# worm-privacy/proof-of-burn

Hardware: AMD Instinct MI355X
Metric: proof_of_burn witnesses/sec (higher is better)
Workload: dtype u64 bit-sliced lanes + BN254 Fr (8x32-bit Montgomery)

## Files before the change

### proof_of_burn_amd/csrc/circuits.hpp

```cpp
#pragma once
#include <string.h>
#include "gadgets.hpp"
#include "poseidon_consts.h"

#define KECCAKF_ROUND_WIRES 102656u
#define KECCAKF_WIRES (43200u + 24u * KECCAKF_ROUND_WIRES)
#define ABSORB_OWN 5888u
#define ABSORB_WIRES (ABSORB_OWN + 17u * 384u + KECCAKF_WIRES)
#define KR_STORED 76u
#define KR_BITS (KR_STORED * 64u)
#define AB_DIRECT (ABSORB_OWN + 17u * 384u + 43200u)
#define ABSORB_BITS (AB_DIRECT + 24u * KR_BITS)
#define ABSORB_ALIAS (ABSORB_WIRES - ABSORB_BITS)

enum UnitKind : uint32_t {
    U_POB_INPUT = 1, U_POB_RANGE, U_POB_LAYER_ASSERT, U_POB_HDR_ASSERT, U_POB_POSEIDONS, U_BAH_PRE, U_BAH_POST,
    U_KB_HEAD, U_KB_RANGE, U_KB_SELROW, U_KB_POST, U_POB_N2B, U_PC_PRE, U_PC_POST, U_POB_LASTLAYER, U_POB_LASTLAYER_RANGE,
    U_POB_LASTLEN, U_POB_LEAF, U_POB_LAYER_POST, U_SC_M, U_SC_RANGE, U_SC_SUMS, U_POB_LASTLEAF,
    U_RL_A, U_RL_SLROW, U_RL_ACC, U_RL_B, U_POW_PRE, U_POW_POST, U_POB_FINAL, U_ABS_RANGE, U_LD_HEAD, U_LD_SELR, U_LD_TAIL, U_POB_INPUT_FR, U_RL_ACC_B, U_RL_ACC_C,
    U_SP_INPUT, U_SP_HEAD,
    U_SC_MI,
    CK_POS_SEG,
    CK_SR_COLS,
    CK_SL_ROWS,
    CK_N2BE,
    CK_CAT,
    CK_RL_B2, CK_RL_B3,
    U_POS_WIDE,
    U_GM, U_GM_INPUT,
    U_PC_COPY,
    U_LD_COPY,
    U_KIND_COUNT
};
enum : uint32_t { UNIT_GEN = 1, UNIT_CHECK = 2, UNIT_EMIT = 4 };
enum Fam : uint32_t { F_MISC = 0, F_RANGE, F_SELROW, F_LD, F_RL, F_SC, F_POS, F_N2B, F_GM, F_COUNT };
#define FAM_BIT(f) (1u << (f))
#define FAM_LIGHT (FAM_BIT(F_MISC) | FAM_BIT(F_RANGE) | FAM_BIT(F_SELROW) | FAM_BIT(F_LD) | FAM_BIT(F_RL))
#define FAM_HEAVY (FAM_BIT(F_POS) | FAM_BIT(F_N2B))
#define FAM_ALL ((1u << F_COUNT) - 1)
HD constexpr uint32_t fam_of(uint32_t k) {
    return (k == U_KB_RANGE || k == U_ABS_RANGE) ? F_RANGE
         : k == U_KB_SELROW ? F_SELROW
         : (k == U_LD_HEAD || k == U_LD_SELR || k == U_LD_TAIL || k == U_LD_COPY || k == U_POB_LASTLAYER_RANGE || k == U_SC_SUMS) ? F_LD
         : (k == U_RL_A || k == U_RL_SLROW || k == U_RL_ACC_B || k == U_RL_ACC_C || k == U_RL_B || k == CK_SR_COLS || k == CK_SL_ROWS || k == CK_RL_B2 || k == CK_RL_B3 || k == CK_CAT) ? F_RL
         : (k == U_POB_LAYER_POST || k == U_SC_M || k == U_SC_RANGE) ? F_SC
         : (k == U_POB_POSEIDONS || k == U_BAH_PRE || k == U_SP_HEAD || k == CK_POS_SEG || k == U_POS_WIDE) ? F_POS
         : (k == U_GM || k == U_GM_INPUT) ? F_GM
         : (k == U_POB_INPUT_FR || k == U_POB_RANGE || k == U_POB_N2B || k == U_PC_POST || k == U_RL_ACC || k == U_POW_PRE || k == U_SP_INPUT || k == CK_N2BE) ? F_N2B
         : F_MISC;
}
HD constexpr uint32_t gen_fam_of(uint32_t k) { return k == U_PC_PRE ? (uint32_t)F_N2B : fam_of(k); }
HD constexpr bool ride_keeps_evaluation(uint32_t kind) { return fam_of(kind) == F_RL; }
#define UCASE(K) case K: if constexpr ((((MASK) >> (P::is_gen ? gen_fam_of(K) : fam_of(K))) & 1u) && !(P::ride && ride_keeps_evaluation(K)))

struct PobParams { int L, NB, HB, minNib, amountBytes, powZero; Fr maxIntended, maxActual; };
struct SpendParams { int maxAmountBytes; };

#define FP_ISEQ_S (Cur{6, 2, 0, 0, 4})
#define FP_ISEQ_F (Cur{6, 2, 0, 0, 4})
#define FP_N2B8 (Cur{9, 0, 0, 0, 9})
#define FP_ISEQ_D (Cur{6, 0, 0, 0, 6})

struct PobMain {
    FrRef commitment, burnKey, actualBalance, intendedBalance, revealAmount, burnExtraCommitment;
    SmRef numLeafAddressNibbles, layers, layerLens, numLayers, blockHeader, blockHeaderLen, byteSecurityRelax;
    FrRef proofExtraCommitment, remainingCoin, nullifier;
    SmRef addressHashNibbles, blockRoot, stateRoot, nullifierBytes, remainingCoinBytes, revealAmountBytes, burnExtraCommitmentBytes,
        extraCommitmentBytes, lastLayer, lastLayerLen;
    BitRef layerExists, substringCheckers;
    SmRef layerKeccaks, reducedLayerKeccaks;
    BitRef isLeaf, isLastLayerLeaf;
    SmRef leaf, leafLen;
};
struct SpendMain {
    FrRef commitment, burnKey, balance, withdrawnBalance, extraCommitment, coin, remainingCoin;
    SmRef coinBytes, withdrawnBalanceBytes, remainingCoinBytes, extraCommitmentBytes;
};
struct KBRefs {
    SmRef out, in, inLen, numBlocks; BitRef inBitsArray, inBits, inBlocks, outBits, outBytes;
    uint32_t padded_w, pad_o_w, pad_in_w;
    SmRef pad_nb, pad_il, pad_dv, pad_rm; BitRef pad_flt, pad_isEq, pad_isLast;
    Cur c_loop;
    Cur c_div;
    BitRef k_out, k_in; SmRef k_blocks; BitRef k_finalState, f_out, f_in; SmRef f_blocks; BitRef f_s;
    uint32_t abs_w, abs_b;
    BitRef sel_out, sel_arrays; SmRef sel_select; BitRef sel_T;
    Cur c_post;
    SmRef dst; uint32_t has_dst;
    uint32_t mb, index;
};
struct ScRefs {
    BitRef out; uint32_t mi_w; SmRef ml, si; FrRef num; uint32_t M_w; BitRef ex, isl, alw; SmRef sums; BitRef dne;
    Cur c_abs_sub, c_abs_main, c_after_abs, c_loop, c_tail;
    SmRef abs_main_in;
};
struct RlRefs {
    SmRef o, ol, in, inl; FrRef bal; SmRef key, keyLen, acc, accLen, pk, pkLen, val, valLen;
    SmRef t_o, t_ol, t_in, t_il, t_dv, t_rm, t_shf, t_on, t_tmp;
    SmRef s_o, s_in, s_cn; BitRef s_isEq; SmRef s_temp;
    Cur c_sl_iseq, c_mux, c_age, c_acc, c_concat;
};
struct LdRefs {
    BitRef isLeaf; SmRef layer, ll;
    BitRef leafPrefixIsF8; SmRef totalLength; BitRef isConsistentWithLayerLen; SmRef keyPrefix; BitRef keyPrefixIsValid, keyIsMultiByte;
    SmRef keyExtraLen, keyLen, valueWrapperPrefix; BitRef valueWrapperPrefixIsB8; SmRef valueWrapperLen, valuePrefix; BitRef valuePrefixIsF8;
    SmRef valueLen; BitRef isValueWrapperLenConsistent, isKeyValueLenEqualWithLayerLen;
    Cur c_sel[4], c_eq[4], c_mand, c_end;
    SmRef src, len_src; BitRef dst;
};
struct RaRefs {
    SmRef ea_o, ea_ol; FrRef ea_ib; SmRef pn, pnl, br, brl, nbl, sc;
    SmRef ri_o, ri_ol; FrRef ri_i; SmRef by, len, be; BitRef isb, isz; SmRef frb;
    Cur c_cb, c_sl, c_lt, c_concat, c_end;
};
struct SpongeDesc { uint32_t n, stage, src_b, kin_b, fin_b, fs_b, abs_b, kin_w, fin_w, fs_w, abs_w, src_w; };
struct UnitDesc { uint32_t kind, stage; Cur cur; uint32_t a[8]; uint32_t cost, flags; };

#define SC_RANGE_POS 32
#define MAX_KB 72
#define MAX_SC 64
struct CircuitLayout {
    int circuit;
    struct { uint32_t tid, nfr_in, nsm_in, nout; } gm;
    uint32_t decl_order;
    PobParams pob; SpendParams spend;
    PobMain pm; SpendMain sm;
    Fr prefix[3];
    struct { SmRef nibbles; FrRef in; SmRef addressBytes, block, hash; uint32_t kb; } bah;
    struct { FrRef out; SmRef in, flat, block, hash, reduced; uint32_t kb; int N, nb; SmRef fl_o, fl_i, fit_o, fit_i; Cur c_abs; } pc;
    struct { FrRef in; SmRef mzb, keyBytes, raBytes, becBytes, eip, hin, block, keccak; BitRef sbz; uint32_t kb; } pw;
    struct { SmRef out; uint32_t arr_w, sel_w, T_w; Cur c_sel0; } ll;
    RlRefs rl;
    RaRefs ra;
    uint32_t kb_hdr, kb_layer0, nkb, nsc;
    Cur fp_n2be32, fp_n2beN;
    KBRefs kbs[MAX_KB];
    ScRefs scs[MAX_SC];
    LdRefs lds[MAX_SC + 1];
};

HD PosOff pos_off(int t) {
    PosOff k;
    if (t == 3) { k.C = POS_OFF_C_3; k.S = POS_OFF_S_3; k.M = POS_OFF_M_3; k.Pm = POS_OFF_P_3; k.rp = POS_RP_3; }
    else if (t == 4) { k.C = POS_OFF_C_4; k.S = POS_OFF_S_4; k.M = POS_OFF_M_4; k.Pm = POS_OFF_P_4; k.rp = POS_RP_4; }
    else { k.C = POS_OFF_C_5; k.S = POS_OFF_S_5; k.M = POS_OFF_M_5; k.Pm = POS_OFF_P_5; k.rp = POS_RP_5; }
    return k;
}

#define NO_RANK 0xFFFFFFFFu
template <class P> HD BitRef dbits(P& p, uint32_t n) { BitRef r = {p.dvs(n), NO_RANK}; return r; }
template <class P> GD void kb_head(P& p, int mb, S inLen, KBRefs& r) {
    const uint32_t m = 136 * mb;
    r.mb = mb;
    r.out = p.sms(32); r.in = p.sms(m); r.inLen = p.sms(1); r.padded_w = p.dvs(m); r.numBlocks = p.sms(1);
    r.inBitsArray = dbits(p, 8 * m); r.inBits = dbits(p, 8 * m); r.inBlocks = p.bits(8 * m); r.outBits = dbits(p, 256); r.outBytes = dbits(p, 256);
    inLen = p.put(r.inLen, inLen);
    gAssertLessThanS(p, 16, inLen, (S)m);
    r.pad_o_w = p.dvs(m); r.pad_nb = p.sms(1); r.pad_in_w = p.dvs(m); r.pad_il = p.sms(1); r.pad_dv = p.sms(1); r.pad_rm = p.sms(1);
    r.pad_flt = p.bits(m + 1); r.pad_isEq = p.bits(m); r.pad_isLast = p.bits(m);
    inLen = p.put(r.pad_il, inLen);
    S q, rem;
    r.c_div = p.cur;
    gDivide(p, 16, inLen, (S)136, q, rem);
    q = p.put(r.pad_dv, q); p.put(r.pad_rm, rem);
    S nb = p.put(r.pad_nb, q + 1);
    gAssertLessEqThanS(p, 16, nb, (S)mb);
    p.put(r.numBlocks, nb);
    p.put(r.pad_flt, ~(B)0);
    r.c_loop = p.cur;
    p.cur = cur_add(cur_add(cur_add(p.cur, FP_ISEQ_D, 2 * m), FP_N2B8, m), Cur{16u * m, 0, 0, 0, 16u * m}, 1);
}
template <class P> HD void iseq_derived(P& p, Cur c, S a, S b) {
    p.derived(c.w + 1, a); p.derived(c.w + 2, b);
    const S x = (S)((uint32_t)b - (uint32_t)a);
    p.derived(c.w + 4, x); p.derived_inv(c.w + 5, x, true);
}
template <class P> GD void kb_range(P& p, const KBRefs& r, SmRef src, uint32_t lo, uint32_t hi, bool assert_src = false, SmRef also = SmRef{0, 0}) {
    const uint32_t m = 136 * r.mb, cnt = hi - lo, ln = p.lane_id();
    const S inLen = p.get(r.inLen), nb = p.get(r.numBlocks);
    const S last = (S)((uint32_t)nb * 136u - 1u);
    const Cur cE = r.c_loop, cL = cur_add(cE, FP_ISEQ_D, m), cN = cur_add(cL, FP_ISEQ_D, m), cF = cur_add(cN, FP_N2B8, m);
    const uint32_t flat_o_w = cF.w, flat_i_w = cF.w + 8 * m;
    bool fl = P::is_gen ? ((uint32_t)inLen >= lo) : p.bit(p.get(r.pad_flt + lo));
    uint32_t wE = 0, wL = 0, wF = 0, wPE = 0, wPL = 0;
    B wb0 = 0, wb1 = 0;
    S vs[16];
    if constexpr (P::is_count) { for (uint32_t t = 0; t < cnt; t++) p.put(r.in + (lo + t), (S)0); for (int q = 0; q < 16; q++) vs[q] = 0; }
    else {
        SmRef rr[16]; S sv[16];
#pragma unroll
        for (int q = 0; q < 16; q++) rr[q] = r.in + (lo + ((uint32_t)q < cnt ? (uint32_t)q : cnt - 1));
        const SmLoaded<16> h = sm_load(p, rr);
#pragma unroll
        for (int q = 0; q < 16; q++) sv[q] = p.get(src + (lo + ((uint32_t)q < cnt ? (uint32_t)q : cnt - 1)));
        sm_commit(p, rr, h, sv);
#pragma unroll
        for (int q = 0; q < 16; q++) vs[q] = P::is_check ? h.s[q] : sv[q];
        if (assert_src) {
#pragma unroll
            for (int q = 0; q < 16; q++) p.require_lane((uint32_t)sv[q] < 256u, FAILCODE(T_NUM2BITS, 38));
        }
        if (also.w) {
            SmRef ar[16];
#pragma unroll
            for (int q = 0; q < 16; q++) ar[q] = also + (lo + ((uint32_t)q < cnt ? (uint32_t)q : cnt - 1));
            const SmLoaded<16> ha = sm_load(p, ar);
            sm_commit(p, ar, ha, sv);
        }
    }
#pragma unroll
    for (uint32_t t = 0; t < 16; t++) if (t < cnt) {
        const uint32_t i = lo + t;
        const Cur ce = cur_add(cE, FP_ISEQ_D, i), cl = cur_add(cL, FP_ISEQ_D, i);
        const S v = vs[t];
        iseq_derived(p, ce, (S)i, inLen); iseq_derived(p, cl, (S)i, last);
        const bool e = (uint32_t)inLen == i, l = (uint32_t)last == i;
        fl = fl && !e;
        const S pv = (fl ? v : 0) + (S)e + (l ? 0x80 : 0);
        p.derived(r.pad_in_w + i, v); p.derived(r.pad_o_w + i, pv); p.derived(r.padded_w + i, pv); p.derived(cN.w + 9 * i + 8, pv);
        p.require_lane((uint32_t)pv < 256u, FAILCODE(T_NUM2BITS, 38));
        wE |= (uint32_t)e << t; wL |= (uint32_t)l << t; wF |= (uint32_t)fl << t;
        wPE |= (e ? 3u : 0u) << (2 * t); wPL |= (l ? 3u : 0u) << (2 * t);
        if (t < 8) wb0 |= (B)((uint32_t)pv & 0xffu) << (8 * t); else wb1 |= (B)((uint32_t)pv & 0xffu) << (8 * (t - 8));
    }
    const B runE = p.xpose64(wE, 0, cnt), runL = p.xpose64(wL, 0, cnt), runF = p.xpose64(wF, 0, cnt);
    const B runPairE = p.xpose64(wPE, 0, 2 * cnt), runPairL = p.xpose64(wPL, 0, 2 * cnt);
    const B bits0 = p.xpose(wb0, 64), bits1 = cnt > 8 ? p.xpose(wb1, 64) : 0;
    p.run_put(cnt, r.pad_isEq.w + lo + ln, r.pad_isEq.i + lo + ln, runE);
    p.run_put(cnt, r.pad_flt.w + lo + 1 + ln, r.pad_flt.i + lo + 1 + ln, runF);
    p.run_put(cnt, r.pad_isLast.w + lo + ln, r.pad_isLast.i + lo + ln, runL);
    {
        const uint32_t i = lo + (ln >> 1), wh = ln & 1;
        p.run_derived(2 * cnt, cE.w + 6 * i + 3 * wh, runPairE);
        p.run_derived(2 * cnt, cL.w + 6 * i + 3 * wh, runPairL);
        if constexpr (P::is_emit) { if (ln < 2 * cnt) { p.site_c(cE.w + 6 * i + 3 * wh, r.pad_isEq.w + i); p.site_c(cL.w + 6 * i + 3 * wh, r.pad_isLast.w + i); } }
    }
    for (uint32_t h2 = 0; h2 < 2 && 8 * h2 < cnt; h2++) {
        const uint32_t n = (cnt - 8 * h2 < 8 ? cnt - 8 * h2 : 8) * 8;
        const B x = h2 ? bits1 : bits0;
        const uint32_t j = 8 * (lo + 8 * h2) + ln, i = lo + 8 * h2 + (ln >> 3);
        p.run_put(n, r.inBlocks.w + j, r.inBlocks.i + j, x);
        p.run_derived(n, cN.w + 9 * i + (ln & 7), x);
        p.run_derived(n, r.inBitsArray.w + j, x);
        p.run_derived(n, flat_i_w + j, x);
        p.run_derived(n, flat_o_w + j, x);
        p.run_derived(n, r.inBits.w + j, x);
    }
}
template <class P> GD void kb_declare_keccak(P& p, KBRefs& r) {
    const uint32_t n = r.mb;
    r.k_out = dbits(p, 256); r.k_in = p.bits(n * 1088); r.k_blocks = p.sms(1); r.k_finalState = dbits(p, 1600);
    r.f_out = dbits(p, 1600); r.f_in = p.bits(n * 1088); r.f_blocks = p.sms(1); r.f_s = p.bits((n + 1) * 1600);
    r.abs_w = p.cur.w; r.abs_b = p.cur.b;
    p.skip_alias(n * ABSORB_WIRES, n * ABSORB_BITS);
    r.sel_out = dbits(p, 1600); r.sel_arrays = dbits(p, (n + 1) * 1600); r.sel_select = p.sms(1); r.sel_T = dbits(p, 1600 * (n + 1));
}
template <class P, int N1> GD void kb_selrow_n(P& p, const KBRefs& r, uint32_t row, uint32_t j0, uint32_t j1) {
    const uint32_t n1 = N1 ? (uint32_t)N1 : r.mb + 1, n = j1 - j0, ln = p.lane_id();
    const uint32_t fw = 9 * n1 + 3, fb = 1, fq = 9 * n1 + 2;
    const Cur c0 = p.cur;
    const uint32_t idx = row * 64 + j0 + ln;
    const S blocks = p.get(r.numBlocks);
    p.require(p.ballot((uint32_t)blocks < n1), FAILCODE(T_SELECTOR, 43));
    const uint32_t bw = c0.w + ln * fw, bb = c0.b + ln * fb;
    B acc = 0;
    p.run_derived(n, bw + 2 * n1 + 2, 0);
#pragma unroll
    for (uint32_t k = 0; k < n1; k++) {
        const B v = p.run_get(n, r.f_s.i + k * 1600 + idx);
        const B e = p.ballot((uint32_t)blocks == k);
        acc |= e & v;
        if constexpr (P::is_emit) {
            p.run_derived(n, r.sel_arrays.w + k * 1600 + idx, v);
            p.run_derived(n, r.sel_T.w + idx * n1 + k, v);
            p.run_derived(n, bw + 1 + k, v);
            p.run_derived(n, bw + n1 + 2 + k, e);
            p.run_derived(n, bw + 2 * n1 + 3 + k, acc);
            const uint32_t cw = bw + 3 * n1 + 3 + 6 * k;
            p.run_derived(n, cw, e);
            p.run_derived(n, cw + 3, e);
        }
    }
    p.run_put(n, bw, bb, acc);
    p.run_derived(n, r.sel_out.w + idx, acc);
    p.run_derived(n, r.f_out.w + idx, acc);
    p.run_derived(n, r.k_finalState.w + idx, acc);
    if (row < 4) {
        const uint32_t pw = r.c_post.w;
        p.run_derived(n, r.k_out.w + idx, acc);
        p.run_derived(n, r.outBits.w + idx, acc);
        p.run_derived(n, pw + 256 + idx, acc);
        p.run_derived(n, pw + idx, acc);
        p.run_derived(n, r.outBytes.w + idx, acc);
        p.run_derived(n, pw + 512 + 9 * (idx >> 3) + 1 + (idx & 7), acc);
        for (uint32_t jj = 0; jj < n; jj += 8) {
            S by = 0;
#pragma unroll
            for (uint32_t b = 0; b < 8; b++) by |= (S)p.bit(p.run_bcast(acc, jj + b)) << b;
            const uint32_t i = (row * 64 + j0 + jj) >> 3;
            const SmRef b2n_o = {pw + 512 + 9 * i, r.c_post.s + i};
            const S o = p.put(r.out + i, p.put(b2n_o, by));
            if (r.has_dst) p.put(r.dst + i, o);
        }
    }
    derived_rows_same(p, c0.w + n1 + 1, fw, n, blocks);
    for (uint32_t k = 0; k < n1; k++) {
        const uint32_t cw = c0.w + 3 * n1 + 3 + 6 * k;
        const S x = (S)(k - (uint32_t)blocks);
        derived_rows_same(p, cw + 1, fw, n, blocks);
        derived_rows_same(p, cw + 2, fw, n, (S)k);
        derived_rows_same(p, cw + 4, fw, n, x);
        derived_rows_same(p, cw + 5, fw, n, x, true);
    }
    p.cur = cur_add(c0, Cur{fw, fb, 0, 0, fq}, n);
}
template <class P> GD void kb_selrow(P& p, const KBRefs& r, uint32_t row, uint32_t j0, uint32_t j1) { kb_selrow_n<P, 0>(p, r, row, j0, j1); }
template <class P> GD void kb_post(P& p, const KBRefs& r) {
    S nb = p.get(r.numBlocks);
    p.put(r.k_blocks, nb); p.put(r.f_blocks, nb); p.put(r.sel_select, nb);
    p.cur = cur_add(r.c_post, Cur{512 + 32 * 9, 0, 32, 0, 512 + 32 * 8}, 1);
}

#include "gadget_mains.hpp"

template <class P> GD void rl_b_prefixes(P& p, const RlRefs& R, const PobParams& prm, S kl, S& pl, S& vl) {
    const int ab = 32, bb = prm.amountBytes, maxAcc = 4 + bb + 66, maxKey = 1 + ab;
    const S al = p.get(R.accLen);
    p.put(R.val, 0xb8); p.put(R.val + 1, al);
    copy_n(p, R.val + 2, R.acc, maxAcc);
    vl = p.put(R.valLen, 2 + al);
    p.put(R.pk, 0xf8); p.put(R.pk + 1, (kl + 1) + vl); p.put(R.pk + 2, 0x80 + kl);
    copy_n(p, R.pk + 3, R.key, maxKey);
    pl = p.put(R.pkLen, 3 + kl);
}
template <class P, class MR> GD void rl_b_concat(P& p, const RlRefs& R, const MR& M, const PobParams& prm, S pl, S vl) {
    const int ab = 32, bb = prm.amountBytes, maxAcc = 4 + bb + 66, maxVal = 2 + maxAcc, maxKey = 1 + ab, maxPK = 2 + 1 + maxKey, maxOut = maxPK + maxVal;
    p.cur = R.c_concat;
    S cl;
    SmRef c;
    if constexpr (P::is_check) c = gConcatHead(p, maxPK, maxVal, R.pk, pl, R.val, vl, cl);
    else c = gConcat(p, maxPK, maxVal, R.pk, pl, R.val, vl, cl, true);
    { copy_n(p, R.o, c, (int)(maxOut)); copy_n(p, M.leaf, c, (int)(maxOut)); }
    p.put(M.leafLen, p.put(R.ol, cl));
}

template <class P> GD void L_pc_declare(P& p, CircuitLayout& L, int N) {
    const Cur c_abs = p.cur;
    for (int j = 0; j < N; j++) { p.dvs(32); p.cur = cur_add(p.cur, FP_ABITS8, 32); }
    const SmRef fl_o = p.sms(32 * N), fl_i = p.sms(32 * N);
    const SmRef fit_o = p.sms(136 * L.pc.nb), fit_i = p.sms(32 * N);
    if (P::is_count) { L.pc.c_abs = c_abs; L.pc.fl_o = fl_o; L.pc.fl_i = fl_i; L.pc.fit_o = fit_o; L.pc.fit_i = fit_i; }
}

HD bool unit_is_heavy(uint32_t k) { return fam_of(k) >= F_SC; }
HD bool unit_gen_is_heavy(uint32_t k) { return gen_fam_of(k) >= F_SC; }

template <class P, uint32_t MASK> GD void unit_run(P& p, const UnitDesc& d, CircuitLayout& L);
#ifdef __HIPCC__
template <uint32_t MASK, bool FAULT> GD void unit_run_ride(GenPT<true, FAULT>& p, const UnitDesc& d, CircuitLayout& L) {
    if constexpr ((MASK >> F_RL) & 1u) { if (ride_keeps_evaluation(d.kind)) { GenPT<false> q = plain_of(p); unit_run<GenPT<false>, FAM_BIT(F_RL)>(q, d, L); p.status = q.status; return; } }
    unit_run<GenPT<true, FAULT>, MASK>(p, d, L);
}
#endif
template <class P, uint32_t MASK> GD void unit_run(P& p, const UnitDesc& d, CircuitLayout& L) {

    const PobMain& M = L.pm;
    const PobParams& prm = L.pob;
    const int LB = 136 * prm.NB, HBy = 136 * prm.HB;
    (void)M; (void)LB; (void)HBy;
    p.cur = d.cur;
    switch (d.kind) {
    UCASE(U_GM) { gm_run(p, d, L); } break;
    UCASE(U_GM_INPUT) { gm_input(p, d); } break;
    UCASE(U_POB_INPUT) {
        for (uint32_t k = d.a[0]; k < d.a[1]; k++) { SmRef r = {M.numLeafAddressNibbles.w + k, M.numLeafAddressNibbles.i + k}; p.put(r, p.input_sm(k)); }
    } break;
    UCASE(U_POB_LAYER_ASSERT) {
        gAssertLessThanS(p, 16, p.get(M.layerLens + d.a[0]), (S)(LB * 8));
    } break;
    UCASE(U_POB_HDR_ASSERT) {
        gAssertLessThanS(p, 16, p.get(M.blockHeaderLen), (S)(HBy * 8));
        for (int i = 0; i < 32; i++) p.put(M.stateRoot + i, p.get(M.blockHeader + 91 + i));
    } break;
    UCASE(U_ABS_RANGE) {
        SmRef src = {d.a[2], d.a[3]};
        abs_range(p, d.cur, d.a[0], src, d.a[4], d.a[5]);
    } break;
    UCASE(U_BAH_POST) {
        SmRef nb = gBytes2Nibbles(p, 32, L.bah.hash);
        { copy_n(p, L.bah.nibbles, nb, (int)(64)); copy_n(p, M.addressHashNibbles, nb, (int)(64)); }
    } break;
    UCASE(U_KB_HEAD) {
        SmRef len = {d.a[1], d.a[2]};
        KBRefs r = L.kbs[d.a[0]];
        const S inLen = (P::is_gen && d.a[3]) ? p.input_sm(d.a[3] - 1) : p.get(len);
        kb_head(p, r.mb, inLen, r);
        if (P::is_count) L.kbs[d.a[0]] = r;
    } break;
    UCASE(U_KB_RANGE) {
        SmRef src = {d.a[1], d.a[2]};
        kb_range(p, L.kbs[d.a[0]], src, d.a[3], d.a[4], d.a[5] != 0, SmRef{d.a[6], d.a[7]});
    } break;
    UCASE(U_KB_SELROW) { kb_selrow(p, L.kbs[d.a[0]], d.a[1], d.a[2], d.a[3]); } break;
    UCASE(U_KB_POST) { kb_post(p, L.kbs[d.a[0]]); } break;
    UCASE(U_PC_PRE) {
        const int N = L.pc.N;
        L_pc_declare(p, L, N);
        KBRefs r = L.kbs[L.pc.kb];
        kb_head(p, L.pc.nb, (S)(32 * N), r);
        if (P::is_count) L.kbs[L.pc.kb] = r;
    } break;
    UCASE(U_PC_COPY) {
        const uint32_t N = (uint32_t)L.pc.N, j = d.a[0], nblk = 136u * (uint32_t)L.pc.nb;
        if (j < N) {
            SmRef src;
            if (L.circuit == 2) src = L.pc.in + 32 * j;
            else if (L.circuit == 0) src = j == 0 ? M.blockRoot : j == 1 ? M.nullifierBytes : j == 2 ? M.remainingCoinBytes : j == 3 ? M.revealAmountBytes : j == 4 ? M.burnExtraCommitmentBytes : M.extraCommitmentBytes;
            else src = j == 0 ? L.sm.coinBytes : j == 1 ? L.sm.withdrawnBalanceBytes : j == 2 ? L.sm.remainingCoinBytes : L.sm.extraCommitmentBytes;
            auto dst_of = [&](uint32_t a) -> SmRef {
                const SmRef b = a == 0 ? L.pc.in : a == 1 ? L.pc.fl_i : a == 2 ? L.pc.fl_o : a == 3 ? L.pc.flat : a == 4 ? L.pc.fit_i : a == 5 ? L.pc.fit_o : L.pc.block;
                return b + 32 * j;
            };
// ... 448 lines not shown
        }
        if (lo == 0) p.derived_fr(sc.M_w, fr_zero());
        for (uint32_t k = lo; k < hi; k++) {
            Fr b1 = {{(uint32_t)p.get(src + k), 0, 0, 0, 0, 0, 0, 0}};
            acc = fr_add(fr_mul(b1, p.k256r(k)), acc);
            p.derived_fr(sc.M_w + k + 1, acc);
            p.site_m(sc.M_w + k + 1, sc.mi_w + k, k);
        }
    } break;
    UCASE(U_SC_RANGE) {
        const ScRefs& sc = L.scs[d.a[0]];
        const uint32_t lo = d.a[1], hi = d.a[2], sl = 31;
        const S mainLen = p.get(sc.ml);
        const F subNum = p.get(sc.num);
        const Fr subC = fr_from_mont(subNum);
        const SmRef src = M.layers + ((d.a[0] - 1) * LB);
        const uint32_t lastIdx = (uint32_t)(mainLen - (S)sl + 1);
        const uint32_t ln = p.lane_id(), cnt = hi - lo;
        bool allowed = P::is_gen ? (lastIdx >= lo) : p.bit(p.get(sc.alw + lo));
        uint32_t wIsl = 0, wAlw = 0, wEx = 0;
        B wC0 = 0, wC1 = 0;
        F ddL = fr_zero();
        Fr win = sc_window(p, src, lo, sl);
        for (uint32_t t = 0; t < cnt; t++) {
            const uint32_t i = lo + t;
            const S nxt = i + sl < (uint32_t)LB ? p.get(src + (i + sl)) : 0;
            const bool e = fr_eq(win, subC), last = i == lastIdx;
            allowed = allowed && !last;
            wIsl |= (uint32_t)last << t; wAlw |= (uint32_t)allowed << t; wEx |= (uint32_t)e << t;
            const B four = (B)((last ? 3u : 0u) | (e ? 12u : 0u)) << (4 * (t & 15));
            if (t < 16) wC0 |= four; else wC1 |= four;
            if constexpr (P::is_emit) {
                const Cur c = cur_add(cur_add(sc.c_loop, FP_ISEQ_S, i), FP_ISEQ_F, i);
                iseq_derived(p, c, (S)i, (S)lastIdx);
                const F t1 = fr_mul(subNum, p.k256(i)), t2 = fr_mul(fr_to_mont(win), p.k256(i)), dd = fr_sub(t2, t1);
                p.derived_fr(c.w + 7, t1); p.derived_fr(c.w + 8, t2); p.derived_fr(c.w + 10, dd);
                const F ds = p.bcast_sel(dd);
                if (ln == t) ddL = ds;
            }
            sc_window_step(win, sl, (uint32_t)nxt);
        }
        if constexpr (P::is_emit) {
            const F inv = fr_is_zero(ddL) ? fr_zero() : fr_inv(ddL);
            if (ln < cnt) p.w32(cur_add(cur_add(sc.c_loop, FP_ISEQ_S, lo + ln), FP_ISEQ_F, lo + ln).w + 11, fr_from_mont(inv), (fr_is_zero(ddL) ? 3 : 2) | 4);
        }
        const B runIsl = p.xpose64(wIsl, 0, cnt), runAlw = p.xpose64(wAlw, 0, cnt), runEx = p.xpose64(wEx, 0, cnt);
        const B runC0 = p.xpose(wC0, 64), runC1 = cnt > 16 ? p.xpose(wC1, 64) : 0;
        p.run_put(cnt, sc.isl.w + lo + ln, sc.isl.i + lo + ln, runIsl);
        p.run_put(cnt, sc.alw.w + lo + 1 + ln, sc.alw.i + lo + 1 + ln, runAlw);
        p.run_put(cnt, sc.ex.w + lo + ln, sc.ex.i + lo + ln, runEx);
        for (uint32_t h2 = 0; h2 < 2 && 16 * h2 < cnt; h2++) {
            const uint32_t n = (cnt - 16 * h2 < 16 ? cnt - 16 * h2 : 16) * 4, i = lo + 16 * h2 + (ln >> 2), wh = ln & 3;
            p.run_put(n, sc.c_loop.w + 12 * i + 3 * wh, sc.c_loop.b + 4 * i + wh, h2 ? runC1 : runC0);
        }
    } break;
    UCASE(CK_POS_SEG) {
        if constexpr (!(P::is_check || P::is_count)) { (void)d; }
        else if (d.a[0] == 3) gPoseidonSegStored<P, 3>(p, pos_off(3), d.cur, d.a[1]);
        else if (d.a[0] == 4) gPoseidonSegStored<P, 4>(p, pos_off(4), d.cur, d.a[1]);
        else gPoseidonSegStored<P, 5>(p, pos_off(5), d.cur, d.a[1]);
    } break;
    UCASE(CK_SL_ROWS) {
        if constexpr (P::is_check || P::is_count) gShiftLeftRows(p, (int)d.a[0], d.cur, Cur{d.a[3], d.a[4], d.a[5], d.cur.f, d.cur.q}, d.a[1], d.a[2]);
    } break;
    UCASE(CK_N2BE) {
        if constexpr (P::is_check || P::is_count || P::is_gen) {
            const FrRef src = P::is_gen ? FrRef{d.a[6], d.a[7]} : FrRef{d.a[1], d.a[2]}; const SmRef also = {d.a[3], d.a[4]};
            gNum2BigEndianBytesFv(p, (int)d.a[0], p.get(src), also, d.a[5] != 0);
        }
    } break;
    default: break;
    }
}
template <class P> GD void unit_run_all(P& p, const UnitDesc& d, CircuitLayout& L) { unit_run<P, FAM_ALL>(p, d, L); }

#include <stdlib.h>
#include <algorithm>
#include <stdexcept>
#include <string>
#include <vector>
struct Plan {
    CircuitLayout L;
    std::vector<UnitDesc> units;
    std::vector<SpongeDesc> sponges;
    Cur total;
    uint32_t nfr_in, nsm_in, max_stage;
    enum { TRACK_STRIDE = 32, MAX_TRACKS = 7 };
    uint32_t ntracks, track_fork[MAX_TRACKS], track_join[MAX_TRACKS];
    uint32_t wide_tracks = 0;
    CountP p;

    static bool same(Cur a, Cur b) { return a.w == b.w && a.b == b.b && a.s == b.s && a.f == b.f && a.q == b.q; }
    void expect_cursor(const char* what, Cur got, Cur want) {
        if (!same(got, want)) throw std::runtime_error(std::string("layout planner: split units disagree with the monolithic template: ") + what);
    }
    void record(uint32_t kind, uint32_t stage, Cur cur, uint32_t a0 = 0, uint32_t a1 = 0, uint32_t a2 = 0, uint32_t a3 = 0, uint32_t a4 = 0, uint32_t a5 = 0, uint32_t a6 = 0, uint32_t a7 = 0) {
        UnitDesc d; d.kind = kind; d.stage = stage; d.cur = cur; d.cost = 0; d.a[0] = a0; d.a[1] = a1; d.a[2] = a2; d.a[3] = a3; d.a[4] = a4; d.a[5] = a5; d.a[6] = a6; d.a[7] = a7;
        d.flags = (kind == CK_POS_SEG || kind == CK_SR_COLS || kind == CK_SL_ROWS || kind == CK_RL_B2 || kind == CK_RL_B3 || kind == CK_CAT) ? UNIT_CHECK
                : kind == CK_N2BE ? (UNIT_GEN | UNIT_CHECK)
                : kind == U_POS_WIDE ? UNIT_GEN
                : kind == U_SC_M ? UNIT_EMIT
                : kind == U_POB_POSEIDONS ? (UNIT_CHECK | UNIT_EMIT)
                : kind == U_GM_INPUT ? (UNIT_GEN | UNIT_CHECK)
                : kind == U_POB_INPUT ? UNIT_EMIT
                : (UNIT_GEN | UNIT_CHECK | UNIT_EMIT);
        units.push_back(d);
        if (stage > max_stage) max_stage = stage;
    }
    void unit(uint32_t kind, uint32_t stage, uint32_t a0 = 0, uint32_t a1 = 0, uint32_t a2 = 0, uint32_t a3 = 0, uint32_t a4 = 0) {
        record(kind, stage, p.cur, a0, a1, a2, a3, a4);
        const UnitDesc d = units.back();
        p.nnotes = 0;
        unit_run_all(p, d, L);
        take_notes(p, stage);
    }
    void take_notes(CountP& q, uint32_t stage) {
        if (q.notes_overflow) throw std::runtime_error("layout planner: a composite unit has more split sub-blocks than PLAN_MAX_NOTES");
        for (uint32_t k = 0; k < q.nnotes; k++) {
            const PlanNote& nt = q.notes[k];
            if (nt.what == NOTE_POSEIDON) {
                const uint32_t ns = pos_nseg(pos_off((int)nt.n).rp);
                for (uint32_t seg = 1; seg < ns; seg++) record(CK_POS_SEG, stage, nt.cur, nt.n, seg);
                if (stage % TRACK_STRIDE == 0) throw std::runtime_error("layout planner: a Poseidon composite needs a stage before it");
                record(U_POS_WIDE, stage - 1, nt.cur, nt.n, nt.a[0], nt.a[1], nt.a[2], nt.a[3], nt.a[4], nt.a[5]);
            } else if (nt.what == NOTE_N2BE) record(CK_N2BE, stage, nt.cur, nt.n, nt.a[0], nt.a[1], nt.a[2], nt.a[3], nt.a[4], nt.a[5], nt.a[6]);
            else if (nt.what == NOTE_SHIFTLEFT) { for (uint32_t i = 0; i < nt.n; i += 2) record(CK_SL_ROWS, stage, nt.cur, nt.n, i, std::min(i + 2, nt.n), nt.a[0], nt.a[1], nt.a[2]); }
        }
        q.nnotes = 0;
    }
    void record_composite(uint32_t kind, uint32_t stage, Cur cur) {
        record(kind, stage, cur);
        const UnitDesc d = units.back();
        CountP q; q.nnotes = 0;
        unit_run_all(q, d, L);
        take_notes(q, stage);
    }
    void cat_units(uint32_t stage, Cur c0, int La, int Lb) {
        Cur cc[3]; concat_cursors(p, c0, La, Lb, cc);
        for (uint32_t part = 0; part < 4; part++) record(CK_CAT, stage, cc[part < 3 ? part : 2], part, (uint32_t)La, (uint32_t)Lb, c0.w, c0.s);
    }
    void abs_units(uint32_t stage, uint32_t N, SmRef src, uint32_t chunk = 32, bool emit_only = false) {
        CountP chk; chk.cur = p.cur; gAssertByteString(chk, (int)N, src);
        const uint32_t own_w = p.dvs(N);
        const Cur c0 = p.cur;
        for (uint32_t lo = 0; lo < N; lo += chunk) { record(U_ABS_RANGE, stage, c0, own_w, 0, src.w, src.i, lo, std::min(lo + chunk, N)); if (emit_only) units.back().flags = UNIT_EMIT; }
        p.cur = cur_add(c0, FP_ABITS8, N);
        expect_cursor("AssertByteString", p.cur, chk.cur);
    }
    void keccak_tail(uint32_t kb, uint32_t range_stage, SmRef dst, bool has_dst) {
        KBRefs& r = L.kbs[kb];
        r.index = kb;
        kb_declare_keccak(p, r);
        SpongeDesc s; s.n = r.mb; s.stage = range_stage + 1; s.src_b = r.inBlocks.i; s.src_w = r.inBlocks.w;
        s.kin_b = r.k_in.i; s.kin_w = r.k_in.w; s.fin_b = r.f_in.i; s.fin_w = r.f_in.w; s.fs_b = r.f_s.i; s.fs_w = r.f_s.w; s.abs_b = r.abs_b; s.abs_w = r.abs_w;
        sponges.push_back(s);
        r.dst = dst; r.has_dst = has_dst ? 1 : 0;
        {
            CountP q; q.cur = p.cur; r.c_post = Cur{0, 0, 0, 0}; r.has_dst = 0; kb_selrow(q, r, 24, 0, 1);
            const Cur fp1 = {q.cur.w - p.cur.w, q.cur.b - p.cur.b, q.cur.s - p.cur.s, 0, q.cur.q - p.cur.q};
            r.c_post = cur_add(p.cur, fp1, 1600); r.has_dst = has_dst ? 1 : 0;
        }
        const uint32_t split = r.mb >= 8 ? 4 : r.mb >= 3 ? 2 : 1;
        for (uint32_t row = 0; row < 25; row++) {
            const Cur c0 = p.cur;
            CountP q; q.cur = c0; kb_selrow(q, r, row, 0, 64);
            const Cur fp = {(q.cur.w - c0.w) / 64, (q.cur.b - c0.b) / 64, (q.cur.s - c0.s) / 64, 0, (q.cur.q - c0.q) / 64};
            for (uint32_t k = 0; k < split; k++) record(U_KB_SELROW, range_stage + 2, cur_add(c0, fp, k * (64 / split)), kb, row, k * (64 / split), (k + 1) * (64 / split));
            p.cur = q.cur;
        }
        if (!same(p.cur, r.c_post)) throw std::runtime_error("layout planner: selector footprint");
        unit(U_KB_POST, range_stage + 2, kb);
        if (range_stage + 1 > max_stage) max_stage = range_stage + 1;
    }
    void keccak_bytes(uint32_t kb, int mb, uint32_t stage, SmRef src, SmRef len, SmRef dst, uint32_t len_input = 0, bool has_dst = true, bool assert_src = false, SmRef also = SmRef{0, 0}) {
        L.kbs[kb].mb = mb;
        const Cur start = p.cur;
        unit(U_KB_HEAD, stage, kb, len.w, len.i, len_input);
        const uint32_t m = 136 * mb;
        for (uint32_t lo = 0; lo < m; lo += 16) record(U_KB_RANGE, stage + 1, start, kb, src.w, src.i, lo, std::min(lo + 16, m), assert_src ? 1u : 0u, also.w, also.i);
        keccak_tail(kb, stage + 1, dst, has_dst);
    }
    void kb_ranges(uint32_t kb, uint32_t stage, SmRef src) {
        const uint32_t m = 136 * L.kbs[kb].mb;
        for (uint32_t lo = 0; lo < m; lo += 16) record(U_KB_RANGE, stage, p.cur, kb, src.w, src.i, lo, std::min(lo + 16, m));
    }
    void leaf_detector(uint32_t inst, uint32_t stage, SmRef src, SmRef len, BitRef dst, bool copy_units = true) {
        const uint32_t N = 136 * L.pob.NB;
        CountP chk; chk.cur = p.cur; gLeafDetector(chk, (int)N, src, 0);
        L.lds[inst].src = src; L.lds[inst].len_src = len; L.lds[inst].dst = dst;
        unit(U_LD_HEAD, stage, inst);
        expect_cursor("LeafDetector", p.cur, chk.cur);
        if (copy_units) for (uint32_t lo = 0; lo < N; lo += 32) record(U_LD_COPY, stage, p.cur, inst, lo, std::min(lo + 32, N));
        for (uint32_t k = 0; k < 4; k++) for (uint32_t lo = 0; lo < N; lo += 34) record(U_LD_SELR, stage + 1, p.cur, inst, k, lo, std::min(lo + 34, N));
        record(U_LD_TAIL, stage + 2, p.cur, inst);
    }
    void burn_address_hash(uint32_t pre_stage) {
        L.bah.nibbles = p.sms(64); L.bah.in = p.frs(3); L.bah.addressBytes = p.sms(20); L.bah.block = p.sms(136); L.bah.hash = p.sms(32);
        L.bah.kb = L.nkb++;
        if (L.circuit == 2) { L.pm.burnKey = L.bah.in; L.pm.revealAmount = L.bah.in + 1; L.pm.burnExtraCommitment = L.bah.in + 2; L.pm.addressHashNibbles = L.bah.nibbles; }
        unit(U_BAH_PRE, pre_stage);
        kb_ranges(L.bah.kb, pre_stage + 1, L.bah.block);
        keccak_tail(L.bah.kb, pre_stage + 1, L.bah.hash, true);
        unit(U_BAH_POST, pre_stage + 4);
    }
    void proof_of_work_checker(uint32_t pre_stage) {
        L.pw.in = p.frs(3); L.pw.mzb = p.sms(1); L.pw.keyBytes = p.sms(32); L.pw.raBytes = p.sms(32); L.pw.becBytes = p.sms(32); L.pw.eip = p.sms(8);
        L.pw.hin = p.sms(104); L.pw.block = p.sms(136); L.pw.keccak = p.sms(32); L.pw.sbz = p.bits(32);
        L.pw.kb = L.nkb++;
        if (L.circuit == 2) { L.pm.burnKey = L.pw.in; L.pm.revealAmount = L.pw.in + 1; L.pm.burnExtraCommitment = L.pw.in + 2; L.pm.byteSecurityRelax = L.pw.mzb; }
        unit(U_POW_PRE, pre_stage);
        kb_ranges(L.pw.kb, pre_stage + 1, L.pw.block);
        keccak_tail(L.pw.kb, pre_stage + 1, L.pw.keccak, true);
        unit(U_POW_POST, pre_stage + 4);
    }
    void public_commitment(int N, uint32_t pre_stage) {
        L.pc.N = N; L.pc.nb = N * 32 / 136 + ((N * 32) % 136 != 0);
        L.pc.out = p.frs(1); L.pc.in = p.sms(32 * N); L.pc.flat = p.sms(32 * N); L.pc.block = p.sms(136 * L.pc.nb); L.pc.hash = p.sms(32); L.pc.reduced = p.sms(31);
        L.pc.kb = L.nkb++; L.kbs[L.pc.kb].mb = L.pc.nb;
        {
            CountP chk; chk.cur = p.cur; chk.decl_order = p.decl_order;
            for (int j = 0; j < N; j++) gAssertByteString(chk, 32, L.pc.in + 32 * j);
            gFlattenS(chk, 32 * N, L.pc.in); gFitS(chk, 32 * N, 136 * L.pc.nb, L.pc.flat);
            unit(U_PC_PRE, pre_stage);
            for (int j = 0; j <= N; j++) record(U_PC_COPY, pre_stage, p.cur, (uint32_t)j);
            KBRefs r2 = L.kbs[L.pc.kb]; kb_head(chk, L.pc.nb, (S)(32 * N), r2);
            expect_cursor("PublicCommitment", p.cur, chk.cur);
        }
        kb_ranges(L.pc.kb, pre_stage + 1, L.pc.block);
        keccak_tail(L.pc.kb, pre_stage + 1, L.pc.hash, true);
        unit(U_PC_POST, pre_stage + 4);
    }

    void estimate_costs() {
        for (UnitDesc& d : units) {
            if (d.kind == U_POS_WIDE) { d.cost = 8 * pos_wires((int)d.a[0], pos_off((int)d.a[0]).rp); continue; }
            CountP q; const UnitDesc dd = d; unit_run_all(q, dd, L); d.cost = q.nput * (unit_is_heavy(d.kind) ? 4 : 1);
        }
    }
    void plan_pob(const PobParams& prm) {
        memset(&L, 0, sizeof L);
        L.circuit = 0; L.pob = prm; L.nkb = 0; max_stage = 0; L.decl_order = p.decl_order;
        L.fp_n2be32 = n2be_footprint(32); L.fp_n2beN = n2be_footprint(prm.amountBytes);
        const uint32_t TB = TRACK_STRIDE, TR = 2 * TRACK_STRIDE, TC = 3 * TRACK_STRIDE, TN = 4 * TRACK_STRIDE;
        ntracks = 6; track_fork[1] = 0; track_join[1] = 5; track_fork[2] = TB + 6; track_join[2] = 10; track_fork[3] = 0; track_join[3] = TR + 2;
        track_fork[4] = TB + 1; track_join[4] = 4;
        const uint32_t TP = 5 * TRACK_STRIDE;
        track_fork[5] = 0; track_join[5] = 5; wide_tracks = 1u << 5;
        const uint32_t TQ = 6 * TRACK_STRIDE;
        ntracks = 7; track_fork[6] = 4; track_join[6] = 10;
        PobMain& M = L.pm;
        const int Ln = prm.L, LB = 136 * prm.NB, HBy = 136 * prm.HB;
        p.cur = Cur{1, 0, 0, 0};
        M.commitment = p.frs(1);
        M.burnKey = p.frs(1); M.actualBalance = p.frs(1); M.intendedBalance = p.frs(1); M.revealAmount = p.frs(1); M.burnExtraCommitment = p.frs(1);
        M.numLeafAddressNibbles = p.sms(1); M.layers = p.sms(Ln * LB); M.layerLens = p.sms(Ln); M.numLayers = p.sms(1);
        M.blockHeader = p.sms(HBy); M.blockHeaderLen = p.sms(1); M.byteSecurityRelax = p.sms(1); M.proofExtraCommitment = p.frs(1);
        M.remainingCoin = p.frs(1); M.nullifier = p.frs(1); M.addressHashNibbles = p.sms(64); M.blockRoot = p.sms(32); M.stateRoot = p.sms(32);
        M.nullifierBytes = p.sms(32); M.remainingCoinBytes = p.sms(32); M.revealAmountBytes = p.sms(32); M.burnExtraCommitmentBytes = p.sms(32);
        M.extraCommitmentBytes = p.sms(32); M.lastLayer = p.sms(LB); M.lastLayerLen = p.sms(1); M.layerExists = p.bits(Ln);
        M.substringCheckers = p.bits(Ln - 1); M.layerKeccaks = p.sms(32 * Ln); M.reducedLayerKeccaks = p.sms(31 * Ln); M.isLeaf = p.bits(Ln);
        M.isLastLayerLeaf = p.bits(1); M.leaf = p.sms(139); M.leafLen = p.sms(1);
        nfr_in = 6; nsm_in = 1 + Ln * LB + Ln + 1 + HBy + 2;

        unit(U_POB_INPUT_FR, 0);
        for (uint32_t k = 0; k < nsm_in; k += 256) unit(U_POB_INPUT, 0, k, std::min(k + 256, nsm_in));
        for (int k = 0; k < 5; k++) unit(U_POB_RANGE, TB + 1, k);
        for (int i = 0; i < Ln; i++) { unit(U_POB_LAYER_ASSERT, TP + 1, i); abs_units(TP + 1, LB, M.layers + i * LB, 32, true); }
        unit(U_POB_HDR_ASSERT, TP + 1); abs_units(TP + 1, HBy, M.blockHeader, 32, true);
        unit(U_POB_POSEIDONS, TB + 2, 0);
        unit(U_POB_POSEIDONS, TB + 2, 1);
        burn_address_hash(TB + 2);
        L.kb_hdr = L.nkb++;
        keccak_bytes(L.kb_hdr, prm.HB, 0, M.blockHeader, M.blockHeaderLen, M.blockRoot, 0, true, true);
        for (int j = 0; j < 5; j++) unit(U_POB_N2B, TN + 1, j);
        public_commitment(6, TQ + 1);
        {
            CountP chk; chk.cur = p.cur; gSelectorArray1D(chk, Ln, LB, M.layers, 0);
            L.ll.out = p.sms(LB); L.ll.arr_w = p.dvs(Ln * LB); L.ll.sel_w = p.dvs(1); L.ll.T_w = p.dvs(LB * Ln);
            unit(U_POB_LASTLAYER, TP + 1);
            L.ll.c_sel0 = p.cur;
            const Cur fp = sel_fp((uint32_t)Ln);
            for (uint32_t j = 0; j < (uint32_t)LB; j += 4) record(U_POB_LASTLAYER_RANGE, TP + 1, p.cur, j, std::min<uint32_t>(j + 4, LB));
            p.cur = cur_add(p.cur, fp, LB);
            expect_cursor("SelectorArray1D", p.cur, chk.cur);
        }
        unit(U_POB_LASTLEN, TP + 1);
        L.kb_layer0 = L.nkb; L.nkb += Ln;
        L.nsc = Ln;
        for (int i = 0; i < Ln; i++) {
            leaf_detector(i, TP + 1, M.layers + i * LB, M.layerLens + i, M.isLeaf + i, false);
            keccak_bytes(L.kb_layer0 + i, prm.NB, 0, M.layers + i * LB, M.layerLens + i, M.layerKeccaks + 32 * i, 0, true, true, L.lds[i].layer);
            const Cur start = p.cur;
            unit(U_POB_LAYER_POST, 5, i);
            if (i > 0) {
                const ScRefs sc = L.scs[i];
                CountP chk; chk.cur = start; { gFitS(chk, 32, 31, M.layerKeccaks); gSubstringCheck(chk, LB, 31, M.layers, 0, M.reducedLayerKeccaks); }
                expect_cursor("SubstringCheck", p.cur, chk.cur);
                const SmRef src = M.layers + (i - 1) * LB;
                for (uint32_t lo = 0; lo < (uint32_t)LB; lo += 32) {
                    record(U_ABS_RANGE, TP + 1, sc.c_abs_main, sc.abs_main_in.w, sc.abs_main_in.i, src.w, src.i, lo, std::min<uint32_t>(lo + 32, LB));
                    units.back().flags = UNIT_EMIT;
                }
                for (uint32_t lo = 0; lo < (uint32_t)LB; lo += 32) record(U_SC_M, TP + 1, start, i, lo, std::min<uint32_t>(lo + 32, LB));
                const uint32_t kk = LB - 31 + 1;
                record(U_SC_MI, TP + 1, start, i);
                for (uint32_t lo = 0; lo < kk; lo += SC_RANGE_POS) record(U_SC_RANGE, 6, sc.c_loop, i, lo, std::min<uint32_t>(lo + SC_RANGE_POS, kk));
                const uint32_t sums_step = 64;
// ... 129 lines not shown
```

### proof_of_burn_amd/csrc/k_keccak.hip

```cpp
#include <stdlib.h>
#define POB_KECCAK_TU
#include "keccak_kernels.hpp"
void launch_k_chain(const KArgs& K, bool check, uint32_t nsponges, uint32_t ngroups, hipStream_t st) {
    if (check) hipLaunchKernelGGL(k_chain_check, dim3(nsponges, ngroups), dim3(64), 0, st, K);
    else hipLaunchKernelGGL(k_chain, dim3(nsponges, ngroups), dim3(64), 0, st, K);
}
int pob_kchk_rounds() { return POB_KCHK_ROUNDS; }
void launch_k_rounds(const KArgs& K, bool check, uint32_t nperms, uint32_t ngroups, hipStream_t st) {
    if (check) hipLaunchKernelGGL((k_rounds_check<true, POB_KCHK_ROUNDS, 4, 12>), dim3(nperms * (24 / POB_KCHK_ROUNDS), ngroups), dim3(64), 0, st, K);
    else hipLaunchKernelGGL(k_rounds_gen<POB_KGEN_ROUNDS>, dim3(nperms * (24 / POB_KGEN_ROUNDS), ngroups), dim3(64), 0, st, K);
}
#ifndef POB_KGC_ROUNDS
#define POB_KGC_ROUNDS 8
#endif
#ifndef POB_KGC_WAVES
#define POB_KGC_WAVES 4
#endif
#ifndef POB_KGC_DP
#define POB_KGC_DP 4
#endif
#ifndef POB_KGC_NTM
#define POB_KGC_NTM false
#endif
int pob_kgc_rounds() { return POB_KGC_ROUNDS; }
void launch_k_rounds_gc(const KArgs& K, uint32_t nperms, uint32_t ngroups, bool fault, hipStream_t st) {
    if (fault) hipLaunchKernelGGL((k_rounds_gc<POB_KGC_ROUNDS, POB_KGC_DP, POB_KGC_WAVES, true, POB_KGC_NTM>), dim3(nperms * (24 / POB_KGC_ROUNDS), ngroups), dim3(64), 0, st, K);
    else hipLaunchKernelGGL((k_rounds_gc<POB_KGC_ROUNDS, POB_KGC_DP, POB_KGC_WAVES, false, POB_KGC_NTM>), dim3(nperms * (24 / POB_KGC_ROUNDS), ngroups), dim3(64), 0, st, K);
}
void launch_k_emit_bits(const u64* G, uint8_t* out, uint32_t wire_base, uint32_t bit_base, uint32_t count, uint32_t sel, hipStream_t st) {
    uint32_t blocks = (count + 255) / 256; if (blocks > 8192) blocks = 8192;
    hipLaunchKernelGGL(k_emit_bits, dim3(blocks), dim3(256), 0, st, G, out, wire_base, bit_base, count, sel);
}
void launch_k_emit_bits_red(const u64* G, uint8_t* out, uint32_t wire0, uint32_t bit_base, uint32_t count, uint32_t sel, const unsigned long long* rbits, const uint32_t* rpre,
                            uint32_t k0, uint32_t kn, hipStream_t st) {
    uint32_t blocks = (count + 255) / 256; if (blocks > 16384) blocks = 16384;
    hipLaunchKernelGGL(k_emit_bits_red, dim3(blocks), dim3(256), 0, st, G, out, wire0, bit_base, count, sel, rbits, rpre, k0, kn);
}
void launch_k_emit_absorb(const u64* G, uint8_t* out, uint32_t ab, uint32_t o0, uint32_t count, uint32_t sel, const uint16_t* tab, hipStream_t st) {
    uint32_t blocks = (count + 255) / 256; if (blocks > 8192) blocks = 8192;
    hipLaunchKernelGGL(k_emit_absorb, dim3(blocks), dim3(256), 0, st, G, out, ab, o0, count, sel, tab);
}
void launch_k_emit_absorb_red(const u64* G, uint8_t* out, uint32_t wire0, uint32_t ab, uint32_t o0, uint32_t count, uint32_t sel, const uint16_t* tab, const unsigned long long* rbits,
                              const uint32_t* rpre, uint32_t k0, uint32_t kn, hipStream_t st) {
    uint32_t blocks = (count + 255) / 256; if (blocks > 16384) blocks = 16384;
    hipLaunchKernelGGL(k_emit_absorb_red, dim3(blocks), dim3(256), 0, st, G, out, wire0, ab, o0, count, sel, tab, rbits, rpre, k0, kn);
}
bool keccak_alias_table_host(uint16_t* tab) { return keccak_round_alias_table(tab); }
```

### proof_of_burn_amd/csrc/keccak_kernels.hpp

```cpp
#pragma once
#include <hip/hip_runtime.h>
#include <stdint.h>
#include "kernels_common.hpp"
#ifdef POB_HOSTSIM
#define POB_WAVES_PER_SIMD(n)
#else
#define POB_WAVES_PER_SIMD(n) __attribute__((amdgpu_waves_per_eu(n, n)))
#endif

static __device__ __constant__ u64 KECCAK_RC_DEV[24] = {
    0x0000000000000001ULL, 0x0000000000008082ULL, 0x800000000000808AULL, 0x8000000080008000ULL, 0x000000000000808BULL,
    0x0000000080000001ULL, 0x8000000080008081ULL, 0x8000000000008009ULL, 0x000000000000008AULL, 0x0000000000000088ULL,
    0x0000000080008009ULL, 0x000000008000000AULL, 0x000000008000808BULL, 0x800000000000008BULL, 0x8000000000008089ULL,
    0x8000000000008003ULL, 0x8000000000008002ULL, 0x8000000000000080ULL, 0x000000000000800AULL, 0x800000008000000AULL,
    0x8000000080008081ULL, 0x8000000000008080ULL, 0x0000000080000001ULL, 0x8000000080008008ULL};

__host__ __device__ constexpr int krot_(int i) {
    constexpr int t[25] = {1, 10, 7, 11, 17, 18, 3, 5, 16, 8, 21, 24, 4, 15, 23, 19, 13, 12, 2, 20, 14, 22, 9, 6, 1};
    return t[i];
}
#define KROT(i) krot_(i)

enum : uint32_t { KS_IN = 0, KS_ST = 25, KS_OUT = 101, KS_ZERO = 126, KS_RC = 127 };
#define KSL_X5(x, k) (4u * (x) + (k))
// ... 107 lines not shown
    void arr(uint32_t off, const V& v) { for (uint32_t k = 0; k < 64; k++) set(off + k, v.e[k]); }
    void gate(uint32_t off, const V& o, const V& a, const V& b) { for (uint32_t k = 0; k < 64; k++) { set(off + 3 * k, o.e[k]); set(off + 3 * k + 1, a.e[k]); set(off + 3 * k + 2, b.e[k]); } }
    void out(int, const V&) {}
    void set(uint32_t w, uint16_t e) { if (w >= KECCAKF_ROUND_WIRES || tab[w] != 0xFFFFu) ok = false; else tab[w] = e; }
};

template <class IO> HD void garr(IO& io, uint32_t off, const typename IO::V& o, const typename IO::V& a, const typename IO::V& b) {
    io.arr(off, o); io.arr(off + 64, a); io.arr(off + 128, b); io.gate(off + 192, o, a, b);
}

template <class W> __device__ __forceinline__ void round_native(W* a, int r, uint32_t lane) {
    W c[5], d[5], b[25];
#pragma unroll
    for (int x = 0; x < 5; x++) c[x] = a[x] ^ a[x + 5] ^ a[x + 10] ^ a[x + 15] ^ a[x + 20];
#pragma unroll
    for (int x = 0; x < 5; x++) d[x] = c[(x + 4) % 5] ^ lane_rotl(c[(x + 1) % 5], 1, lane);
#pragma unroll
    for (int i = 0; i < 25; i++) a[i] ^= d[i % 5];
    b[0] = a[0];
#pragma unroll
    for (int i = 0; i < 24; i++) b[KROT(i + 1)] = lane_rotl(a[KROT(i)], ((i + 1) * (i + 2) / 2) % 64, lane);
#pragma unroll
    for (int i = 0; i < 25; i++) { const int y = i / 5 * 5; a[i] = b[i] ^ (~b[y + (i + 1) % 5] & b[y + (i + 2) % 5]); }
    a[0] ^= ((KECCAK_RC_DEV[r] >> lane) & 1) ? ~(W)0 : (W)0;
}

template <class IO> HD void round_walk(IO& io, int r) {
    typedef typename IO::V V;
    V in[25], th[25], rp[25], ch[25], out[25];
#pragma unroll
    for (int i = 0; i < 25; i++) in[i] = io.in(i);
#pragma unroll
    for (int i = 0; i < 25; i++) io.arr(1600 + 64 * i, in[i]);
    {
        const uint32_t T = 8000;
        V C[5], Dv[5];
#pragma unroll
        for (int i = 0; i < 25; i++) io.arr(T + 1600 + 64 * i, in[i]);
#pragma unroll
        for (int x = 0; x < 5; x++) {
            const uint32_t X = T + 3840 + 2112 * x;
            const V a = in[x], b = in[5 + x], c = in[10 + x], d = in[15 + x], e = in[20 + x];
            const V ab = io.gx(KSL_X5(x, 0), a, b), abc = io.gx(KSL_X5(x, 1), ab, c), abcd = io.gx(KSL_X5(x, 2), abc, d), o = io.gx(KSL_X5(x, 3), abcd, e);
            io.arr(X, o); io.arr(X + 64, a); io.arr(X + 128, b); io.arr(X + 192, c); io.arr(X + 256, d); io.arr(X + 320, e);
            io.arr(X + 384, ab); io.arr(X + 448, abc); io.arr(X + 512, abcd);
            garr(io, X + 576, ab, a, b); garr(io, X + 960, abc, ab, c); garr(io, X + 1344, abcd, abc, d); garr(io, X + 1728, o, abcd, e);
            C[x] = o; io.arr(T + 3200 + 64 * x, o);
        }
#pragma unroll
        for (int x = 0; x < 5; x++) {
            const uint32_t Dd = T + 14400 + 1408 * x;
            const V a = C[(x + 1) % 5], b = C[(x + 4) % 5];
            const V rot = io.rotl(a, 1);
            const V aux0 = io.keep_ge(rot, 1), aux1 = io.keep_lt(rot, 1), aux2 = io.or_disjoint(aux0, aux1, rot);
            const V o = io.gx(KSL_D(x), b, aux2);
            io.arr(Dd, o); io.arr(Dd + 64, a); io.arr(Dd + 128, b); io.arr(Dd + 192, aux0); io.arr(Dd + 256, aux1); io.arr(Dd + 320, aux2);
            io.arr(Dd + 384, aux0); io.arr(Dd + 448, a);
            io.arr(Dd + 512, aux1); io.arr(Dd + 576, a);
            garr(io, Dd + 640, aux2, aux0, aux1); garr(io, Dd + 1024, o, b, aux2);
            Dv[x] = o; io.arr(T + 3520 + 64 * x, o);
        }
#pragma unroll
        for (int i = 0; i < 5; i++) {
#pragma unroll
            for (int j = 0; j < 5; j++) {
                const int idx = i + 5 * j;
                const V o = io.gx(KSL_TH(idx), in[idx], Dv[i]);
                garr(io, T + 21440 + 384 * (i * 5 + j), o, in[idx], Dv[i]);
                th[idx] = o; io.arr(T + 64 * idx, o);
            }
        }
    }
#pragma unroll
    for (int i = 0; i < 25; i++) io.arr(3200 + 64 * i, th[i]);
    {
        const uint32_t Rb = 39040;
#pragma unroll
        for (int i = 0; i < 25; i++) io.arr(Rb + 1600 + 64 * i, th[i]);
        rp[0] = th[0]; io.arr(Rb, th[0]);
#pragma unroll
        for (int i = 0; i < 24; i++) {
            const uint32_t S_ = Rb + 3200 + 896 * i;
            const int shl = ((i + 1) * (i + 2) / 2) % 64;
            const V a = th[KROT(i)];
            const V rot = io.rotl(a, shl);
            const V aux0 = io.keep_lt(rot, shl);
            const V aux1 = io.keep_ge(rot, shl);
            const V o = io.or_disjoint(aux0, aux1, rot);
            io.arr(S_, o); io.arr(S_ + 64, a); io.arr(S_ + 128, aux0); io.arr(S_ + 192, aux1);
            io.arr(S_ + 256, aux0); io.arr(S_ + 320, a);
            io.arr(S_ + 384, aux1); io.arr(S_ + 448, a);
            garr(io, S_ + 512, o, aux0, aux1);
            rp[KROT(i + 1)] = o; io.arr(Rb + 64 * KROT(i + 1), o);
        }
    }
#pragma unroll
    for (int i = 0; i < 25; i++) io.arr(4800 + 64 * i, rp[i]);
    {
        const uint32_t Cb = 63744;
#pragma unroll
        for (int i = 0; i < 25; i++) io.arr(Cb + 1600 + 64 * i, rp[i]);
#pragma unroll
        for (int i = 0; i < 25; i++) {
            const uint32_t C_ = Cb + 3200 + 1280 * i;
            const int y = i / 5 * 5;
            const V a = rp[i], b = rp[y + (i + 1) % 5], c = rp[y + (i + 2) % 5];
            const V bx = io.not_(b), bc = io.ga(KSL_AND(i), bx, c);
            const V o = i == 0 ? io.gx(KSL_CHI0, a, bc) : io.gxo(i, a, bc);
            io.arr(C_, o); io.arr(C_ + 64, a); io.arr(C_ + 128, b); io.arr(C_ + 192, c); io.arr(C_ + 256, bx); io.arr(C_ + 320, bc);
            io.arr(C_ + 384, bx); io.arr(C_ + 448, b);
            garr(io, C_ + 512, bc, bx, c); garr(io, C_ + 896, o, a, bc);
            ch[i] = o; io.arr(Cb + 64 * i, o);
        }
    }
#pragma unroll
    for (int i = 0; i < 25; i++) io.arr(6400 + 64 * i, ch[i]);
    {
        const uint32_t Ib = 98944;
        const V rc = io.rc(r);
#pragma unroll
        for (int i = 0; i < 25; i++) io.arr(Ib + 1600 + 64 * i, ch[i]);
        io.arr(Ib + 3200, rc); io.arr(Ib + 3264, rc);
        const V o = io.gxo(0, ch[0], rc);
        garr(io, Ib + 3328, o, ch[0], rc);
        out[0] = o;
#pragma unroll
        for (int i = 1; i < 25; i++) out[i] = ch[i];
#pragma unroll
        for (int i = 0; i < 25; i++) io.arr(Ib + 64 * i, out[i]);
    }
#pragma unroll
    for (int i = 0; i < 25; i++) { io.arr(64 * i, out[i]); io.out(i, out[i]); }
}
static inline bool keccak_round_alias_table(uint16_t* tab) {
    for (uint32_t i = 0; i < KECCAKF_ROUND_WIRES; i++) tab[i] = 0xFFFFu;
    SymIO io; io.tab = tab; io.ok = true;
    round_walk(io, 0);
    for (uint32_t i = 0; i < KECCAKF_ROUND_WIRES; i++) if (tab[i] == 0xFFFFu) io.ok = false;
    return io.ok;
}

#define KF_MID 3200u
#define KF_ROUNDS 43200u
#define AB_KECCAKF (ABSORB_OWN + 17u * 384u)


__device__ __forceinline__ void chain_body(const KArgs A, uint32_t bx, uint32_t by) {
    const uint32_t lane = threadIdx.x & 63u;
    const SpongeDesc sp = A.sponges[A.first + bx];
    u64* G = A.bits + (uint64_t)by * A.group_stride;
    u64 st[25];
#pragma unroll
    for (int i = 0; i < 25; i++) st[i] = 0;
    auto put = [&](uint32_t idx, u64 v) { G[idx + lane] = v; };
    for (uint32_t b = 0; b < sp.n; b++) {
        const uint32_t Ab = sp.abs_b + b * ABSORB_BITS;
        u64 blk[17], aux[25];
#pragma unroll
        for (int i = 0; i < 17; i++) blk[i] = G[sp.src_b + b * 1088 + 64 * i + lane];
#pragma unroll
        for (int i = 0; i < 25; i++) { put(sp.fs_b + b * 1600 + 64 * i, st[i]); put(Ab + 1600 + 64 * i, st[i]); }
#pragma unroll
        for (int i = 0; i < 17; i++) {
            put(sp.kin_b + b * 1088 + 64 * i, blk[i]); put(sp.fin_b + b * 1088 + 64 * i, blk[i]); put(Ab + 3200 + 64 * i, blk[i]);
            const u64 o = st[i] ^ blk[i];
            const uint32_t X = Ab + ABSORB_OWN + 384 * i;
            put(X, o); put(X + 64, st[i]); put(X + 128, blk[i]);
            { u64* q = G + X + 192 + 3 * lane; q[0] = o; q[1] = st[i]; q[2] = blk[i]; }
            aux[i] = o;
        }
#pragma unroll
        for (int i = 17; i < 25; i++) aux[i] = st[i];
        const uint32_t Kf = Ab + AB_KECCAKF;
#pragma unroll
        for (int i = 0; i < 25; i++) { put(Ab + 4288 + 64 * i, aux[i]); put(Kf + 1600 + 64 * i, aux[i]); put(Kf + KF_MID + 64 * i, aux[i]); st[i] = aux[i]; }
        for (int r = 0; r < 24; r++) {
            round_native(st, r, lane);
#pragma unroll
            for (int i = 0; i < 25; i++) put(Kf + KF_MID + 1600 * (r + 1) + 64 * i, st[i]);
        }
#pragma unroll
        for (int i = 0; i < 25; i++) { put(Kf + 64 * i, st[i]); put(Ab + 64 * i, st[i]); }
    }
#pragma unroll
    for (int i = 0; i < 25; i++) put(sp.fs_b + sp.n * 1600 + 64 * i, st[i]);
}
#ifdef POB_KECCAK_TU
__global__ void __launch_bounds__(64, 3) k_chain(KArgs A) { chain_body(A, blockIdx.x, blockIdx.y); }
#endif

__device__ __forceinline__ void chain_check_body(const KArgs A, uint32_t bx, uint32_t by) {
    const uint32_t lane = threadIdx.x;
    const uint32_t pi = A.first + bx;
    const SpongeDesc sp = A.sponges[A.perm_sponge[pi]];
    const uint32_t b = A.perm_block[pi];
    const u64* G = A.bits + (uint64_t)by * A.group_stride;
    const uint32_t Ab = sp.abs_b + b * ABSORB_BITS, Kf = Ab + AB_KECCAKF;
    u64 bad = 0;
#pragma unroll 1
    for (int i = 0; i < 25; i++) {
        const u64 st = G[sp.fs_b + b * 1600 + 64 * i + lane];
        if (b == 0) bad |= st;
        bad |= G[Ab + 1600 + 64 * i + lane] ^ st;
        u64 aux = st;
        if (i < 17) {
            const u64 blk = G[sp.src_b + b * 1088 + 64 * i + lane];
            bad |= (G[sp.kin_b + b * 1088 + 64 * i + lane] ^ blk) | (G[sp.fin_b + b * 1088 + 64 * i + lane] ^ blk) | (G[Ab + 3200 + 64 * i + lane] ^ blk);
            const u64 o = st ^ blk;
            const uint32_t X = Ab + ABSORB_OWN + 384 * i;
            const u64* q = G + X + 192 + 3 * lane;
            bad |= (G[X + lane] ^ o) | (G[X + 64 + lane] ^ st) | (G[X + 128 + lane] ^ blk) | (q[0] ^ o) | (q[1] ^ st) | (q[2] ^ blk);
            aux = o;
        }
        bad |= (G[Ab + 4288 + 64 * i + lane] ^ aux) | (G[Kf + 1600 + 64 * i + lane] ^ aux) | (G[Kf + KF_MID + 64 * i + lane] ^ aux);
        const u64 last = G[Kf + KF_MID + 1600 * 24 + 64 * i + lane];
        bad |= (G[Kf + 64 * i + lane] ^ last) | (G[Ab + 64 * i + lane] ^ last) | (G[sp.fs_b + (b + 1) * 1600 + 64 * i + lane] ^ last);
    }
#pragma unroll
    for (int o = 32; o > 0; o >>= 1) { bad |= ((u64)__shfl_xor((uint32_t)(bad >> 32), o, 64) << 32) | __shfl_xor((uint32_t)bad, o, 64); }
    if ((bad >> lane) & 1) atomicMin(&A.bad_wire[by * 64 + lane], sp.abs_w + b * ABSORB_WIRES);
}
#ifdef POB_KECCAK_TU
__global__ void __launch_bounds__(64) POB_WAVES_PER_SIMD(4) k_chain_check(KArgs A) { chain_check_body(A, blockIdx.x, blockIdx.y); }
#endif

template <int KR> __device__ __forceinline__ void rounds_gen_body(const KArgs A, uint32_t x, uint32_t y) {
    static_assert(24 % KR == 0, "a chunk does not straddle two permutations");
    const uint32_t lane = threadIdx.x;
    const uint32_t pi = A.first + x / (24 / KR), r0 = x % (24 / KR) * KR;
    const SpongeDesc sp = A.sponges[A.perm_sponge[pi]];
    const uint32_t Ab = sp.abs_b + A.perm_block[pi] * ABSORB_BITS;
    u64* G = A.bits + (uint64_t)y * A.group_stride;
    GenIO io; io.lane = lane;
    const u64* mid = G + Ab + AB_KECCAKF + KF_MID + 1600 * r0;
#pragma unroll
    for (int i = 0; i < 25; i++) io.s[i] = mid[64 * i + lane];
    io.st = G + Ab + AB_DIRECT + r0 * KR_BITS;
#pragma unroll 1
    for (uint32_t r = r0; r < r0 + KR; r++) {
        io.refresh();
        round_walk(io, (int)r);
        io.st += KR_BITS;
    }
}
template <int KR> __global__ void __launch_bounds__(64) k_rounds_gen(KArgs A) { rounds_gen_body<KR>(A, blockIdx.x, blockIdx.y); }

#define KR_CHECK_ARRAYS(kr) (101u * (kr) + 25u)
#define POB_KCHK_ROUNDS 4
#define POB_KGEN_ROUNDS 8
#define POB_ROUNDS_CHECK_BODY(A, X_, Y_, NT, KR, DP) do { \
    static_assert(24 % (KR) == 0, "a chunk does not straddle two permutations"); \
    __builtin_amdgcn_s_setprio(3);        \
    const uint32_t lane = threadIdx.x; \
    const uint32_t pi = (A).first + (X_) / (24 / (KR)), r0 = (X_) % (24 / (KR)) * (KR); \
    const SpongeDesc sp = (A).sponges[(A).perm_sponge[pi]]; \
    const uint32_t Ab = sp.abs_b + (A).perm_block[pi] * ABSORB_BITS; \
    const u64* G = (A).bits + (uint64_t)(Y_) * (A).group_stride; \
    CheckIOT<NT, DP> io; io.lane = lane; io.bad = 0; \
    const u64* mid = G + Ab + AB_KECCAKF + KF_MID + 1600 * r0; \
    _Pragma("unroll") \
    for (int i = 0; i < 25; i++) io.s[i] = io.ldw(mid + 64 * i + lane); \
    io.st = G + Ab + AB_DIRECT + r0 * KR_BITS; \
    _Pragma("unroll 1") \
    for (uint32_t r = r0; r < r0 + (KR); r++) { \
        mid += 1600; io.out_ = mid; \
        io.begin_round(); \
        round_walk(io, (int)r); \
        io.st += KR_BITS; \
        if (__any(io.bad != 0)) {        \
            u64 bad = io.bad; \
            _Pragma("unroll") \
            for (int o = 32; o > 0; o >>= 1) { bad |= ((u64)__shfl_xor((uint32_t)(bad >> 32), o, 64) << 32) | __shfl_xor((uint32_t)bad, o, 64); } \
            if ((bad >> lane) & 1) atomicMin(&(A).bad_wire[(Y_) * 64 + lane], sp.abs_w + (A).perm_block[pi] * ABSORB_WIRES + AB_KECCAKF + KF_ROUNDS + r * KECCAKF_ROUND_WIRES); \
            io.bad = 0; \
        } \
    } } while (0)
template <bool NT, int KR, int WAVES, int DP> __global__ void __launch_bounds__(64) POB_WAVES_PER_SIMD(WAVES) k_rounds_check(KArgs A) { POB_ROUNDS_CHECK_BODY(A, blockIdx.x, blockIdx.y, NT, KR, DP); }

template <int DP, bool FAULT, bool NTM> struct GcIOT : DevIOBase {
    u64* st; const u64* ld; const u64* out_; u64 bad; V s[25];
    V ring[DP], pend[DP];
    const u64* fault; u64 fault_mask;
    __device__ __forceinline__ V in(int i) const { return s[i]; }
    template <bool STORE> __device__ __forceinline__ V twin(int want, V v) {
        const int q = kchk_pos(want), k = q % DP;
        if (q >= DP) bad |= ring[k] ^ pend[k];
        if constexpr (STORE) {
            u64* p = st + want + lane;
            V w = v;
            if constexpr (FAULT) { if (p == fault) w ^= fault_mask; }
            *p = w;
            ring[k] = ld[want + lane];
        } else ring[k] = NTM ? __builtin_nontemporal_load(out_ + (-want - 1) + lane) : out_[(-want - 1) + lane];
        pend[k] = v;
        __builtin_amdgcn_sched_barrier(0);
        return v;
    }
    __device__ __forceinline__ V gx(uint32_t sl, V a, V b) { return twin<true>(64 * (int)sl, a ^ b); }
    __device__ __forceinline__ V ga(uint32_t sl, V a, V b) { return twin<true>(64 * (int)sl, a & b); }
    __device__ __forceinline__ V gxo(int i, V a, V b) { return twin<false>(-(64 * i) - 1, a ^ b); }
    __device__ __forceinline__ void out(int i, V v) { s[i] = v; }
    __device__ __forceinline__ void end_round() {
#pragma unroll
        for (int k = 0; k < DP; k++) bad |= ring[k] ^ pend[k];
    }
};
template <int KR, int DP, int WAVES, bool FAULT, bool NTM> __global__ void __launch_bounds__(64) POB_WAVES_PER_SIMD(WAVES) k_rounds_gc(KArgs A) {
    static_assert(24 % KR == 0, "a chunk does not straddle two permutations");
    static_assert(DP >= 1 && DP <= KCHK_LOADS, "loads in flight");
    const uint32_t lane = threadIdx.x;
    const uint32_t pi = A.first + blockIdx.x / (24 / KR), r0 = blockIdx.x % (24 / KR) * KR;
    const SpongeDesc sp = A.sponges[A.perm_sponge[pi]];
    const uint32_t Ab = sp.abs_b + A.perm_block[pi] * ABSORB_BITS;
    u64* G = A.bits + (uint64_t)blockIdx.y * A.group_stride;
    const u64* mid = G + Ab + AB_KECCAKF + KF_MID + 1600 * r0;
    GcIOT<DP, FAULT, NTM> io; io.lane = lane; io.bad = 0;
    if constexpr (FAULT) { io.fault = blockIdx.y == A.fault_group ? G + A.fault_word : nullptr; io.fault_mask = A.fault_mask; }
#pragma unroll
    for (int i = 0; i < 25; i++) io.s[i] = mid[64 * i + lane];
    io.st = G + Ab + AB_DIRECT + r0 * KR_BITS;
#pragma unroll 1
    for (uint32_t r = r0; r < r0 + KR; r++) {
        uint32_t zero = 0;
        POB_OPAQUE_S(zero);
        io.ld = io.st + zero; mid += 1600; io.out_ = mid;
        io.refresh();
        round_walk(io, (int)r);
        io.end_round();
        io.st += KR_BITS;
        if (__any(io.bad != 0)) {
            u64 bad = io.bad;
#pragma unroll
            for (int o = 32; o > 0; o >>= 1) { bad |= ((u64)__shfl_xor((uint32_t)(bad >> 32), o, 64) << 32) | __shfl_xor((uint32_t)bad, o, 64); }
            if ((bad >> lane) & 1) atomicMin(&A.bad_wire[blockIdx.y * 64 + lane], sp.abs_w + A.perm_block[pi] * ABSORB_WIRES + AB_KECCAKF + KF_ROUNDS + r * KECCAKF_ROUND_WIRES);
            io.bad = 0;
        }
    }
}

__device__ __forceinline__ u64 absorb_wire_word(const u64* A, uint32_t ab, uint32_t o, const uint16_t* tab, uint32_t* neg) {
    *neg = 0;
    if (o < AB_DIRECT) return A[ab + o];
    const uint32_t q = o - AB_DIRECT, r = q / KECCAKF_ROUND_WIRES, e = tab[q - r * KECCAKF_ROUND_WIRES];
    const uint32_t slot = e >> 7, k = (e >> 1) & 63u;
    *neg = e & 1u;
    if (slot < KS_ST) return A[ab + AB_KECCAKF + KF_MID + 1600 * r + 64 * slot + k];
    if (slot < KS_OUT) return A[ab + AB_DIRECT + r * KR_BITS + 64 * (slot - KS_ST) + k];
    if (slot < KS_ZERO) return A[ab + AB_KECCAKF + KF_MID + 1600 * (r + 1) + 64 * (slot - KS_OUT) + k];
    if (slot == KS_ZERO) return 0;
    return ((KECCAK_RC_DEV[r] >> k) & 1) ? ~0ULL : 0ULL;
}
#ifdef POB_KECCAK_TU
__global__ void __launch_bounds__(256) k_emit_absorb(const u64* G, uint8_t* out, uint32_t ab, uint32_t o0, uint32_t count, uint32_t sel, const uint16_t* tab) {
    for (uint32_t t = blockIdx.x * blockDim.x + threadIdx.x; t < count; t += gridDim.x * blockDim.x) {
        uint32_t neg;
        const u64 word = absorb_wire_word(G, ab, o0 + t, tab, &neg);
        const uint32_t v = (uint32_t)((word >> sel) & 1) ^ neg;
        uint4* q = (uint4*)(out + (uint64_t)t * 32);
        q[0] = make_uint4(v, 0, 0, 0); q[1] = make_uint4(0, 0, 0, 0);
    }
}
__global__ void __launch_bounds__(256) k_emit_absorb_red(const u64* G, uint8_t* out, uint32_t wire0, uint32_t ab, uint32_t o0, uint32_t count, uint32_t sel, const uint16_t* tab,
                                                         const unsigned long long* rbits, const uint32_t* rpre, uint32_t k0, uint32_t kn) {
    for (uint32_t t = blockIdx.x * blockDim.x + threadIdx.x; t < count; t += gridDim.x * blockDim.x) {
        const uint32_t w = wire0 + t;
        const unsigned long long word_k = rbits[w >> 6];
        if (!((word_k >> (w & 63)) & 1)) continue;
        const uint32_t p = rpre[w >> 6] + (uint32_t)__popcll(word_k & ((1ull << (w & 63)) - 1)) - k0;
        if (p >= kn) continue;
        uint32_t neg;
        const u64 word = absorb_wire_word(G, ab, o0 + t, tab, &neg);
        const uint32_t v = (uint32_t)((word >> sel) & 1) ^ neg;
        uint4* q = (uint4*)(out + (uint64_t)p * 32);
        q[0] = make_uint4(v, 0, 0, 0); q[1] = make_uint4(0, 0, 0, 0);
    }
}

__global__ void __launch_bounds__(256) k_emit_bits(const u64* G, uint8_t* out, uint32_t wire_base, uint32_t bit_base, uint32_t count, uint32_t sel) {
    for (uint32_t t = blockIdx.x * blockDim.x + threadIdx.x; t < count; t += gridDim.x * blockDim.x) {
        const uint32_t v = (uint32_t)((G[bit_base + t] >> sel) & 1);
        uint4* q = (uint4*)(out + (uint64_t)(wire_base + t) * 32);
        q[0] = make_uint4(v, 0, 0, 0); q[1] = make_uint4(0, 0, 0, 0);
    }
}
__global__ void __launch_bounds__(256) k_emit_bits_red(const u64* G, uint8_t* out, uint32_t wire0, uint32_t bit_base, uint32_t count, uint32_t sel,
                                                       const unsigned long long* rbits, const uint32_t* rpre, uint32_t k0, uint32_t kn) {
    for (uint32_t t = blockIdx.x * blockDim.x + threadIdx.x; t < count; t += gridDim.x * blockDim.x) {
        const uint32_t w = wire0 + t;
        const unsigned long long word = rbits[w >> 6];
        if (!((word >> (w & 63)) & 1)) continue;
        const uint32_t p = rpre[w >> 6] + (uint32_t)__popcll(word & ((1ull << (w & 63)) - 1)) - k0;
        if (p >= kn) continue;
        const uint32_t v = (uint32_t)((G[bit_base + t] >> sel) & 1);
        uint4* q = (uint4*)(out + (uint64_t)p * 32);
        q[0] = make_uint4(v, 0, 0, 0); q[1] = make_uint4(0, 0, 0, 0);
    }
}
#endif
```

### proof_of_burn_amd/csrc/kernels_common.hpp

```cpp
#pragma once
#include <hip/hip_runtime.h>
#include <stdint.h>
#include "circuits.hpp"

typedef unsigned long long u64;

struct GArgs {
    const UnitDesc* units; const uint32_t* order; uint32_t first;
    CircuitLayout* L;
    uint64_t* bits; int32_t* sm; uint32_t* fr;
    uint64_t bits_stride, sm_stride, fr_stride;
    const uint32_t* pos_tab; const uint32_t* inv_lut; const uint32_t* pow256; uint32_t npow256;
    const uint8_t* in_fr; const int32_t* in_sm; uint32_t nfr_in, nsm_in;
    uint32_t* status; uint32_t* chk_status; uint32_t* bad_wire;
    uint8_t* emit_out; uint32_t emit_sel, emit_group;
    uint32_t emit_w0, emit_wn;
    unsigned long long* emit_probe;
    const unsigned long long* emit_rbits; const uint32_t* emit_rpre;
    uint32_t* emit_sites; uint32_t emit_sites_cap;
    uint32_t* emit_counters;
    uint32_t fault_cls, fault_group, fault_idx; uint64_t fault_lanes;
};
struct KArgs {
    u64* bits;
    uint64_t group_stride;
    const SpongeDesc* sponges;
    const uint32_t* perm_sponge;
    const uint32_t* perm_block;
    uint32_t* bad_wire;
    uint32_t first, count;
    uint32_t fault_group; uint64_t fault_word, fault_mask;
};

void launch_g_gen_light(const GArgs& A, uint32_t nunits, uint32_t ngroups, hipStream_t st);
void launch_g_gen_sc(const GArgs& A, uint32_t nunits, uint32_t ngroups, hipStream_t st);
void launch_pos_wide(const GArgs& A, uint32_t nunits, uint32_t ngroups, hipStream_t st, bool ride = false, bool fault = false);
void launch_g_gen_n2b(const GArgs& A, uint32_t nunits, uint32_t ngroups, hipStream_t st);
void launch_g_gen_all(const GArgs& A, uint32_t nunits, uint32_t ngroups, hipStream_t st);
void launch_g_gen_all_ride(const GArgs& A, uint32_t nunits, uint32_t ngroups, hipStream_t st);
void launch_g_gen_all_ride_fault(const GArgs& A, uint32_t nunits, uint32_t ngroups, hipStream_t st);
void launch_g_check_narrow(const GArgs& A, uint32_t nunits, uint32_t ngroups, hipStream_t st);
void launch_g_check_misc(const GArgs& A, uint32_t nunits, uint32_t ngroups, hipStream_t st);
void launch_g_check_range(const GArgs& A, uint32_t nunits, uint32_t ngroups, hipStream_t st);
void launch_g_check_selrow(const GArgs& A, uint32_t nunits, uint32_t ngroups, hipStream_t st);
void launch_g_check_ld(const GArgs& A, uint32_t nunits, uint32_t ngroups, hipStream_t st);
void launch_g_check_rl(const GArgs& A, uint32_t nunits, uint32_t ngroups, hipStream_t st);
void launch_g_check_sc(const GArgs& A, uint32_t nunits, uint32_t ngroups, hipStream_t st);
void launch_g_check_pos(const GArgs& A, uint32_t nunits, uint32_t ngroups, hipStream_t st);
void launch_g_check_n2b(const GArgs& A, uint32_t nunits, uint32_t ngroups, hipStream_t st);
void launch_g_emit_light(const GArgs& A, uint32_t nunits, uint32_t ngroups, hipStream_t st);
void launch_g_emit_heavy(const GArgs& A, uint32_t nunits, uint32_t ngroups, hipStream_t st);
void launch_g_emit_sc(const GArgs& A, uint32_t nunits, uint32_t ngroups, hipStream_t st);
void launch_g_gen_gm(const GArgs& A, uint32_t nunits, uint32_t ngroups, hipStream_t st);
void launch_g_check_gm(const GArgs& A, uint32_t nunits, uint32_t ngroups, hipStream_t st);
void launch_g_emit_gm(const GArgs& A, uint32_t nunits, uint32_t ngroups, hipStream_t st);
void launch_pos_chain(const GArgs& A, const KArgs& K, uint32_t npos, uint32_t nsponges, uint32_t ngroups, hipStream_t st, bool ride = false, bool fault = false);
void launch_k_chain(const KArgs& K, bool check, uint32_t nsponges, uint32_t ngroups, hipStream_t st);
void launch_k_rounds(const KArgs& K, bool check, uint32_t nperms, uint32_t ngroups, hipStream_t st);
void launch_k_rounds_gc(const KArgs& K, uint32_t nperms, uint32_t ngroups, bool fault, hipStream_t st);
int pob_kchk_rounds();
int pob_kgc_rounds();
void launch_k_emit_bits(const u64* G, uint8_t* out, uint32_t wire_base, uint32_t bit_base, uint32_t count, uint32_t sel, hipStream_t st);
void launch_k_emit_bits_red(const u64* G, uint8_t* out, uint32_t wire0, uint32_t bit_base, uint32_t count, uint32_t sel, const unsigned long long* rbits, const uint32_t* rpre, uint32_t k0, uint32_t kn, hipStream_t st);
void launch_k_emit_absorb(const u64* G, uint8_t* out, uint32_t ab, uint32_t o0, uint32_t count, uint32_t sel, const uint16_t* tab, hipStream_t st);
void launch_k_emit_absorb_red(const u64* G, uint8_t* out, uint32_t wire0, uint32_t ab, uint32_t o0, uint32_t count, uint32_t sel, const uint16_t* tab, const unsigned long long* rbits,
                              const uint32_t* rpre, uint32_t k0, uint32_t kn, hipStream_t st);
bool keccak_alias_table_host(uint16_t* tab);
```

### proof_of_burn_amd/csrc/pob_host.hip

```cpp
#include <hip/hip_runtime.h>
#include <stdint.h>
#include <stdio.h>
#include <stdlib.h>
#include <string.h>
#include <time.h>
#include <algorithm>
#include <array>
#include <functional>
#include <string>
#include <mutex>
#include <vector>

#include "../../include/pob_hip.h"
#include "kernels_common.hpp"
#include "pack_window.hpp"


__global__ void k_init_invlut(uint32_t* lut) {
    int t = blockIdx.x * blockDim.x + threadIdx.x;
    if (t > 8192) return;
    Fr c = fr_from_mont(fr_inv(fr_from_i64((int64_t)t - 4096)));
    for (int j = 0; j < 8; j++) lut[t * 8 + j] = c.l[j];
}
__global__ void k_collect(const uint32_t* fr, uint64_t fr_stride, uint32_t out_idx, uint32_t* status_raw, uint32_t* status, uint8_t* outputs, uint32_t* records,
// ... 124 lines not shown
    if (!((word >> (w & 63)) & 1)) return false;
    *pos = W.rpre[w >> 6] + (uint32_t)__popcll(word & ((1ull << (w & 63)) - 1)) - W.w0;
    return *pos < W.wn;
}
__device__ __forceinline__ Fr sc_load(const ScWin& W, uint32_t pos) {
    const uint32_t* q = (const uint32_t*)(W.win + (size_t)pos * 32);
    Fr c; for (int j = 0; j < 8; j++) c.l[j] = q[j];
    return fr_to_mont(c);
}
__global__ void __launch_bounds__(64) k_selfcheck_z(ScWin W, const uint32_t* sites, uint32_t n, uint32_t* res) {
    const uint32_t t = blockIdx.x * blockDim.x + threadIdx.x;
    if (t >= n) return;
    const uint32_t s = sites[t], w = s & 0x7FFFFFFFu;
    uint32_t po, pi, pv, pe = 0, pa = 0, pb = 0;
    bool have = sc_pos(W, w, &po) && sc_pos(W, w + 1, &pi) && sc_pos(W, w + 2, &pv);
    if (have && (s >> 31)) have = sc_pos(W, w - 3, &pe) && sc_pos(W, w - 2, &pa) && sc_pos(W, w - 1, &pb);
    if (!have) { atomicAdd(res + 1, 1u); return; }
    const Fr out = sc_load(W, po), in = sc_load(W, pi), inv = sc_load(W, pv);
    bool ok = fr_eq(fr_mul(in, inv), fr_sub(fr_one_mont(), out)) && fr_is_zero(fr_mul(in, out));
    if (s >> 31) {
        const Fr eo = sc_load(W, pe), a = sc_load(W, pa), b = sc_load(W, pb);
        ok = ok && fr_eq(in, fr_sub(b, a)) && fr_eq(eo, out);
    }
    if (!ok) atomicMin(res, w);
}
__global__ void __launch_bounds__(64) k_selfcheck_c(ScWin W, const uint32_t* sites, uint32_t n, uint32_t* res) {
    const uint32_t t = blockIdx.x * blockDim.x + threadIdx.x;
    if (t >= n) return;
    const uint32_t a = sites[2 * t], b = sites[2 * t + 1];
    uint32_t pa, pb;
    if (!sc_pos(W, a, &pa) || !sc_pos(W, b, &pb)) { atomicAdd(res + 1, 1u); return; }
    const uint4* p = (const uint4*)(W.win + (size_t)pa * 32); const uint4* q = (const uint4*)(W.win + (size_t)pb * 32);
    const uint4 x0 = p[0], x1 = p[1], y0 = q[0], y1 = q[1];
    if (x0.x != y0.x || x0.y != y0.y || x0.z != y0.z || x0.w != y0.w || x1.x != y1.x || x1.y != y1.y || x1.z != y1.z || x1.w != y1.w) atomicMin(res, a);
}
__global__ void __launch_bounds__(64) k_selfcheck_m(ScWin W, const uint32_t* sites, uint32_t n, const uint32_t* pow256, uint32_t* res) {
    const uint32_t t = blockIdx.x * blockDim.x + threadIdx.x;
    if (t >= n) return;
    const uint32_t wn1 = sites[3 * t], wb = sites[3 * t + 1], k = sites[3 * t + 2];
    uint32_t pn, pp, pby;
    if (!sc_pos(W, wn1, &pn) || !sc_pos(W, wn1 - 1, &pp) || !sc_pos(W, wb, &pby)) { atomicAdd(res + 1, 1u); return; }
    Fr pw; for (int j = 0; j < 8; j++) pw.l[j] = pow256[(size_t)k * 8 + j];
    const Fr next = sc_load(W, pn), prev = sc_load(W, pp), by = sc_load(W, pby);
    if (!fr_eq(next, fr_add(prev, fr_mul(by, pw)))) atomicMin(res, wn1);
}
__global__ void __launch_bounds__(64) k_selfcheck_zr(ScWin W, const uint32_t* zw, uint32_t n, uint32_t* res) {
    const uint32_t t = blockIdx.x * blockDim.x + threadIdx.x;
    if (t >= n) return;
    const uint32_t* w6 = zw + 6 * (size_t)t;
    uint32_t p[6];
    if (!sc_pos(W, w6[0], &p[0])) return;
    const bool iseq = w6[3] != 0xFFFFFFFFu;
    auto pos = [&](int j) { if (w6[j] >> 31) { p[j] = w6[j]; return true; } return sc_pos(W, w6[j], &p[j]); };
    bool have = pos(1) && pos(2);
    if (have && iseq) have = pos(3) && pos(4) && pos(5);
    if (!have) { atomicAdd(res + 1, 1u); return; }
    atomicAdd(res + 2, 1u);
    auto val = [&](int j) { if (p[j] >> 31) { Fr c = fr_zero(); c.l[0] = p[j] & 0x7FFFFFFFu; return fr_to_mont(c); } return sc_load(W, p[j]); };
    const Fr out = val(0), in = val(1), inv = val(2);
    bool ok = fr_eq(fr_mul(in, inv), fr_sub(fr_one_mont(), out)) && fr_is_zero(fr_mul(in, out));
    if (iseq) { const Fr eo = val(3), a = val(4), b = val(5); ok = ok && fr_eq(in, fr_sub(b, a)) && fr_eq(eo, out); }
    if (!ok) atomicMin(res, w6[0]);
}
__global__ void __launch_bounds__(64) k_selfcheck_mr(ScWin W, const uint32_t* mw, uint32_t n, const uint32_t* pow256, uint32_t* res) {
    const uint32_t t = blockIdx.x * blockDim.x + threadIdx.x;
    if (t >= n) return;
    const uint32_t* w4 = mw + 4 * (size_t)t;
    uint32_t pn, pp, pby;
    if (!sc_pos(W, w4[0], &pn)) return;
    if (!sc_pos(W, w4[1], &pp) || !sc_pos(W, w4[2], &pby)) { atomicAdd(res + 1, 1u); return; }
    atomicAdd(res + 2, 1u);
    Fr pw; for (int j = 0; j < 8; j++) pw.l[j] = pow256[(size_t)w4[3] * 8 + j];
    const Fr next = sc_load(W, pn), prev = sc_load(W, pp), by = sc_load(W, pby);
    if (!fr_eq(next, fr_add(prev, fr_mul(by, pw)))) atomicMin(res, w4[0]);
}
__global__ void k_xor_word(uint64_t* p, uint64_t mask) { *p ^= mask; }
__global__ void k_xor_u32(uint32_t* p, uint32_t mask) { *p ^= mask; }
__global__ void __launch_bounds__(256) k_fill_ee(uint4* p, uint64_t n16) {
    const uint4 v = make_uint4(0xEEEEEEEEu, 0xEEEEEEEEu, 0xEEEEEEEEu, 0xEEEEEEEEu);
    for (uint64_t i = (uint64_t)blockIdx.x * blockDim.x + threadIdx.x; i < n16; i += (uint64_t)gridDim.x * blockDim.x) p[i] = v;
}

__device__ __forceinline__ uint64_t pow_rotl(uint64_t x, int n) { return n ? (x << n) | (x >> (64 - n)) : x; }
__global__ void __launch_bounds__(256) k_pow_search(uint64_t k0, uint64_t k1, uint64_t k2, uint64_t k3,
                                                     const uint64_t* __restrict__ tail,
                                                     uint64_t base, uint64_t count, uint64_t mask, unsigned long long* found) {
    const uint64_t t = (uint64_t)blockIdx.x * blockDim.x + threadIdx.x;
    if (t >= count) return;
    const uint64_t off = base + t;
    uint64_t w3 = k3 + off, c = w3 < k3, w2 = k2 + c; c = w2 < c; uint64_t w1 = k1 + c; c = w1 < c; const uint64_t w0 = k0 + c;
    uint64_t a[25];
    a[0] = __builtin_bswap64(w0); a[1] = __builtin_bswap64(w1); a[2] = __builtin_bswap64(w2); a[3] = __builtin_bswap64(w3);
#pragma unroll
    for (int i = 4; i < 17; i++) a[i] = tail[i - 4];
#pragma unroll
    for (int i = 17; i < 25; i++) a[i] = 0;
    const uint64_t RC[24] = {0x0000000000000001ULL, 0x0000000000008082ULL, 0x800000000000808AULL, 0x8000000080008000ULL, 0x000000000000808BULL,
                             0x0000000080000001ULL, 0x8000000080008081ULL, 0x8000000000008009ULL, 0x000000000000008AULL, 0x0000000000000088ULL,
                             0x0000000080008009ULL, 0x000000008000000AULL, 0x000000008000808BULL, 0x800000000000008BULL, 0x8000000000008089ULL,
                             0x8000000000008003ULL, 0x8000000000008002ULL, 0x8000000000000080ULL, 0x000000000000800AULL, 0x800000008000000AULL,
                             0x8000000080008081ULL, 0x8000000000008080ULL, 0x0000000080000001ULL, 0x8000000080008008ULL};
    const int ROT[25] = {0, 1, 62, 28, 27, 36, 44, 6, 55, 20, 3, 10, 43, 25, 39, 41, 45, 15, 21, 8, 18, 2, 61, 56, 14};
#pragma unroll 1
    for (int r = 0; r < 24; r++) {
        uint64_t cc[5], b[25];
#pragma unroll
        for (int x = 0; x < 5; x++) cc[x] = a[x] ^ a[x + 5] ^ a[x + 10] ^ a[x + 15] ^ a[x + 20];
#pragma unroll
        for (int x = 0; x < 5; x++) {
            const uint64_t d = cc[(x + 4) % 5] ^ pow_rotl(cc[(x + 1) % 5], 1);
#pragma unroll
            for (int y = 0; y < 25; y += 5) a[y + x] ^= d;
        }
#pragma unroll
        for (int x = 0; x < 5; x++)
#pragma unroll
            for (int y = 0; y < 5; y++) b[y + 5 * ((2 * x + 3 * y) % 5)] = pow_rotl(a[x + 5 * y], ROT[x + 5 * y]);
#pragma unroll
        for (int y = 0; y < 25; y += 5)
#pragma unroll
            for (int x = 0; x < 5; x++) a[y + x] = b[y + x] ^ (~b[y + (x + 1) % 5] & b[y + (x + 2) % 5]);
        a[0] ^= RC[r];
    }
    if ((a[0] & mask) == 0) atomicMin(found, (unsigned long long)off);
}

struct pob_ctx {
    int device = 0, circuit = 0;
    Plan plan;
    uint32_t max_batch = 0, groups = 0, n = 0;
    std::string err;
    hipStream_t stream = nullptr;
    uint64_t* d_bits = nullptr; int32_t* d_sm = nullptr; uint32_t* d_fr = nullptr;
    UnitDesc* d_units = nullptr; uint32_t* d_order = nullptr; CircuitLayout* d_L = nullptr;
    SpongeDesc* d_sponges = nullptr; uint32_t *d_perm_sponge = nullptr, *d_perm_block = nullptr;
    uint32_t *d_pos = nullptr, *d_inv = nullptr, *d_pow256 = nullptr; uint32_t npow256 = 0;
    uint32_t* d_emit_ctr = nullptr;
    uint16_t* d_ktab = nullptr;
    uint8_t* d_in_fr[2] = {nullptr, nullptr}; int32_t* d_in_sm[2] = {nullptr, nullptr}; int in_cur = 0, in_next = 0; uint32_t n_next = 0;
    hipEvent_t ev_in_done[2] = {nullptr, nullptr}; bool in_done_rec[2] = {false, false};
    uint8_t* d_in_sm8[2] = {nullptr, nullptr}; pob_sm_exc_t* d_in_exc[2] = {nullptr, nullptr};
    bool in_bytes[2] = {false, false};
    uint32_t *d_status_raw = nullptr, *d_status = nullptr, *d_chk = nullptr, *d_bad = nullptr, *d_records = nullptr; uint8_t* d_outputs = nullptr;
    struct Emit {
        enum { NSLOT = 3 };
        uint8_t* d_win[NSLOT] = {nullptr, nullptr, nullptr}; uint8_t* h_pin[NSLOT] = {nullptr, nullptr, nullptr};
        hipStream_t s_copy = nullptr; hipEvent_t ev_made[NSLOT] = {nullptr, nullptr, nullptr}, ev_copied[NSLOT] = {nullptr, nullptr, nullptr}, ev_free[NSLOT] = {nullptr, nullptr, nullptr};
        uint64_t win_wires = 0, alloc_wires = 0, next_make = 0, next_take = 0, nwin = 0; uint32_t idx = 0; bool active = false;
        uint32_t first_slot = 0;
        int64_t queued_idx = -1; bool pre_made = false;
        uint64_t pre_made_gen = 0;
        std::vector<uint32_t> status_host; uint64_t status_gen = 0;
        const uint32_t* pin_ptr = nullptr; uint64_t pin_n = 0, pin_id = 0;
        struct Run { uint32_t w, b, n, absorb; };
        std::vector<Run> runs;
        uint64_t probe_win = 0, probe_map = 0; uint32_t* d_order = nullptr; unsigned long long* d_probe = nullptr;
        struct WSeg { uint32_t cls, first, count; };
        std::vector<std::vector<WSeg>> wsegs;
        bool sc_on = false, sc_built = false; std::vector<uint32_t> sc_z, sc_m_next, sc_c_hi; uint32_t *d_sc_z = nullptr, *d_sc_m = nullptr, *d_sc_c = nullptr, *d_sc_res = nullptr;
        uint64_t sc_checked = 0, sc_skipped = 0;
        std::vector<std::array<uint32_t, 3>> sc_ms; std::vector<std::array<uint32_t, 2>> sc_cs;
        const int32_t* sc_alias = nullptr; uint64_t sc_alias_n = 0, sc_red_map = 0, sc_red_host_skipped = 0; uint32_t sc_red_nz = 0, sc_red_nm = 0;
        uint32_t *d_sc_zr = nullptr, *d_sc_mr = nullptr;
        bool red = false; uint64_t map_id = 0, total = 0; std::vector<uint32_t> keep; unsigned long long* d_rbits = nullptr; uint32_t* d_rpre = nullptr;
        bool packed = false, pre_made_packed = false; uint8_t* d_pk[NSLOT] = {nullptr, nullptr, nullptr}; uint32_t *d_pk_blk = nullptr, *d_pk_tot = nullptr; uint64_t pk_alloc_wires = 0, pk_d2h = 0;
        hipStream_t s_val = nullptr;
    } em;
    std::vector<uint32_t> order;
    struct Seg { uint32_t stage, lds, first, count; };
    std::vector<Seg> segs, emit_segs, chk_segs;
    hipStream_t stream2 = nullptr, stream3 = nullptr; hipEvent_t ev_fork = nullptr, ev_join = nullptr, ev_join3 = nullptr;
    struct KSeg { uint32_t stage, sp_first, sp_count, perm_first, perm_count; hipEvent_t ev_done; };
    std::vector<KSeg> ksegs;
    hipStream_t stream_k = nullptr;
    hipEvent_t ev_rounds_fork = nullptr, ev_g_done = nullptr, ev_k_done = nullptr;
    struct Track { hipStream_t s_main = nullptr, s_heavy = nullptr; hipEvent_t ev_fork = nullptr, ev_join = nullptr, ev_start = nullptr, ev_end = nullptr; };
    Track tracks[Plan::MAX_TRACKS];
    uint32_t nperms = 0;
    bool inorder = false;
    bool fused = false;
    bool gc = false, rode = false;
    bool rode_g = false;
    bool fault_armed = false, fault_g = false; int fault_cls = 0; uint32_t fault_group = 0; uint64_t fault_word = 0, fault_mask = 0;
    struct GenLaunch { uint32_t kind, cls, first, count, k_first, k_count; };
    enum { GL_UNITS = 0, GL_CHAIN = 1, GL_POS_CHAIN = 2, GL_ROUNDS = 4 };
    std::vector<GenLaunch> gen_plan[2];
    Seg chk_narrow{0, 0, 0, 0};
    Seg chk_ride_kept{0, F_RL, 0, 0};
    uint32_t nlevels = 0;
    bool generated = false; uint64_t gen_count = 0;
    pob_ctx* partner = nullptr; struct StreamPool* pool = nullptr;
    hipEvent_t ev_gen_done = nullptr, ev_check_done = nullptr; bool gen_done_rec = false, check_done_rec = false, evaluated = false;
    hipStream_t gen_stream = nullptr, chk_stream = nullptr; bool gen_ordered = false, chk_ordered = false;
    hipStream_t s_upload = nullptr;
    hipEvent_t ev_upload = nullptr, ev_rec[2] = {nullptr, nullptr};
    bool kchk_rec[2] = {false, false}; hipEvent_t ev_kchk[2][2] = {{nullptr, nullptr}, {nullptr, nullptr}};
    uint8_t* h_records[2] = {nullptr, nullptr}; int rec_slot = 0, fetch_slot = 0; uint32_t rec_n[2] = {0, 0}; bool upload_pending = false, have_next = false, fetch_pending = false;
};

static hipStream_t own_stream(pob_ctx* h) {
    if (!h->stream) {
        int lo = 0, hi = 0;
        hipSetDevice(h->device);
        if (hipDeviceGetStreamPriorityRange(&lo, &hi) != hipSuccess) hi = 0;
        if (hipStreamCreateWithPriority(&h->stream, hipStreamNonBlocking, hi) != hipSuccess) h->stream = nullptr;
    }
    return h->stream;
}

struct StreamPool { int device = 0, refs = 0; hipStream_t stream2 = nullptr, stream_k = nullptr, track1 = nullptr, track2 = nullptr, chk1 = nullptr, chk2 = nullptr, s_in = nullptr; };
static std::mutex g_pool_mu;
static std::vector<StreamPool*> g_pools;

#define POB_PIPELINE_HW_QUEUES 12
static int hw_queues_env() { const char* e = getenv("GPU_MAX_HW_QUEUES"); return e ? atoi(e) : 4; }
__attribute__((constructor)) static void pob_default_hw_queues() { setenv("GPU_MAX_HW_QUEUES", "16", 0); }

struct pob_ctx;
static hipStream_t own_stream(pob_ctx* h);

#define HIPC(call) do { hipError_t e_ = (call); if (e_ != hipSuccess) { h->err = std::string(#call) + ": " + hipGetErrorString(e_); return POB_E_HIP; } } while (0)

#define N_GEN_CLASSES 6
#define CLS_ALL 6
static uint32_t unit_class(uint32_t kind, bool gen = false) { return fam_of(kind) == F_GM ? 5 : kind == U_POS_WIDE ? 4 : fam_of(kind) == F_SC ? 3 : (gen ? unit_gen_is_heavy(kind) : unit_is_heavy(kind)) ? 1 : 0; }
static void launch_g_gen(const GArgs& A, uint32_t cls, uint32_t nunits, uint32_t ngroups, hipStream_t st, bool ride = false, bool fault = false) {
    if (cls == 5) launch_g_gen_gm(A, nunits, ngroups, st);
    else if (cls == 4) launch_pos_wide(A, nunits, ngroups, st, ride, fault);
    else if (cls == CLS_ALL && ride && fault) launch_g_gen_all_ride_fault(A, nunits, ngroups, st);
    else if (cls == CLS_ALL && ride) launch_g_gen_all_ride(A, nunits, ngroups, st);
    else if (cls == 3) launch_g_gen_sc(A, nunits, ngroups, st);
    else if (cls == 1) launch_g_gen_n2b(A, nunits, ngroups, st);
    else if (cls == CLS_ALL) launch_g_gen_all(A, nunits, ngroups, st);
    else launch_g_gen_light(A, nunits, ngroups, st);
}
static void launch_g_check(const GArgs& A, uint32_t fam, uint32_t nunits, uint32_t ngroups, hipStream_t st) {
    switch (fam) {
    case F_MISC: launch_g_check_misc(A, nunits, ngroups, st); break;
    case F_RANGE: launch_g_check_range(A, nunits, ngroups, st); break;
    case F_SELROW: launch_g_check_selrow(A, nunits, ngroups, st); break;
    case F_LD: launch_g_check_ld(A, nunits, ngroups, st); break;
    case F_RL: launch_g_check_rl(A, nunits, ngroups, st); break;
    case F_SC: launch_g_check_sc(A, nunits, ngroups, st); break;
    case F_POS: launch_g_check_pos(A, nunits, ngroups, st); break;
    case F_GM: launch_g_check_gm(A, nunits, ngroups, st); break;
    default: launch_g_check_n2b(A, nunits, ngroups, st); break;
    }
}
static void launch_g_emit(const GArgs& A, uint32_t cls, uint32_t nunits, hipStream_t st) {
    if (cls == 5) launch_g_emit_gm(A, nunits, 1, st); else if (cls == 3) launch_g_emit_sc(A, nunits, 1, st); else if (cls) launch_g_emit_heavy(A, nunits, 1, st); else launch_g_emit_light(A, nunits, 1, st);
}

static void launch_inputs(pob_ctx* h, int mode, uint32_t G, hipStream_t st) {
    if (h->circuit != POB_CIRCUIT_PROOF_OF_BURN || !h->plan.nsm_in) return;
    const SmRef r0 = h->plan.L.pm.numLeafAddressNibbles;
    const uint32_t fk = (mode == 2 && h->fault_armed && !h->fault_g && h->fault_cls == POB_CLASS_SM) ? (uint32_t)h->fault_word - r0.i : 0xFFFFFFFFu;
    if (h->in_bytes[h->in_cur]) {
        const dim3 grid8((h->plan.nsm_in + IN8_K - 1) / IN8_K, G);
        const size_t lds = 64 * (IN8_K + 1) * 4;
        auto go = [&](auto kern) { hipLaunchKernelGGL(kern, grid8, dim3(256), lds, st, h->d_in_sm8[h->in_cur], h->d_in_exc[h->in_cur], h->plan.nsm_in, h->n, h->d_sm, (uint64_t)h->plan.total.s * 64, r0.i, r0.w, h->d_bad, fk, h->fault_group, h->fault_mask); };
        if (mode == 1) go(k_inputs8<1>); else if (mode == 2) go(k_inputs8<2>); else go(k_inputs8<0>);
        return;
    }
    const dim3 grid((h->plan.nsm_in + 63) / 64, G);
    auto go = [&](auto kern) { hipLaunchKernelGGL(kern, grid, dim3(64), 64 * 65 * 4, st, h->d_in_sm[h->in_cur], h->plan.nsm_in, h->d_sm, (uint64_t)h->plan.total.s * 64, r0.i, r0.w, h->d_bad, fk, h->fault_group, h->fault_mask); };
    if (mode == 1) go(k_inputs<1>); else if (mode == 2) go(k_inputs<2>); else go(k_inputs<0>);
}
static Fr limbs_to_mont(const uint64_t* l) {
    Fr c; for (int i = 0; i < 4; i++) { c.l[2 * i] = (uint32_t)l[i]; c.l[2 * i + 1] = (uint32_t)(l[i] >> 32); }
    return fr_to_mont(c);
}

static GArgs gargs(pob_ctx* h) {
    GArgs A; memset(&A, 0, sizeof A);
    A.units = h->d_units; A.order = h->d_order; A.L = h->d_L;
    A.bits = h->d_bits; A.sm = h->d_sm; A.fr = h->d_fr;
    A.bits_stride = h->plan.total.b; A.sm_stride = (uint64_t)h->plan.total.s * 64; A.fr_stride = (uint64_t)h->plan.total.f * 512;
    A.pos_tab = h->d_pos; A.inv_lut = h->d_inv; A.pow256 = h->d_pow256; A.npow256 = h->npow256; A.in_fr = h->d_in_fr[h->in_cur]; A.in_sm = h->d_in_sm[h->in_cur];
    A.nfr_in = h->plan.nfr_in; A.nsm_in = h->plan.nsm_in;
    A.status = h->d_status_raw; A.chk_status = h->d_chk; A.bad_wire = h->d_bad; A.emit_counters = h->d_emit_ctr;
    A.fault_cls = 0xFFFFFFFFu;
    return A;
}
static KArgs kargs(pob_ctx* h) {
    KArgs K; memset(&K, 0, sizeof K);
    K.bits = (u64*)h->d_bits; K.group_stride = h->plan.total.b; K.sponges = h->d_sponges;
    K.perm_sponge = h->d_perm_sponge; K.perm_block = h->d_perm_block; K.bad_wire = h->d_bad;
    return K;
}

static bool small_param(const uint64_t* l, uint64_t lo, uint64_t hi, int* out) {
    if (l[1] | l[2] | l[3]) return false;
    if (l[0] < lo || l[0] > hi) return false;
    *out = (int)l[0];
    return true;
}
static Fr field_param(const uint64_t* l) {
    Fr c; for (int i = 0; i < 4; i++) { c.l[2 * i] = (uint32_t)l[i]; c.l[2 * i + 1] = (uint32_t)(l[i] >> 32); }
    for (int k = 0; k < 6 && fr_geq_p(c); k++) c = fr_sub_p(c);
    return fr_to_mont(c);
}
static int make_plan(Plan& plan, std::string& err, int circuit, const uint64_t* params, int nparams) {
    if (circuit == POB_CIRCUIT_PROOF_OF_BURN) {
        if (nparams != 8) { err = "ProofOfBurn takes 8 template parameters"; return POB_E_ARG; }
        PobParams prm;
        if (!small_param(params + 0, 2, 64, &prm.L) || !small_param(params + 4, 1, 16, &prm.NB) || !small_param(params + 8, 1, 32, &prm.HB) ||
            !small_param(params + 12, 0, 64, &prm.minNib) || !small_param(params + 16, 1, 31, &prm.amountBytes) || !small_param(params + 20, 0, 32, &prm.powZero) ||
// ... 566 lines not shown
        return POB_OK;
    }
    static const uint32_t side_plan[2][5] = {{F_N2B, F_SC, F_LD, F_RANGE, F_GM}, {F_RL, F_POS, F_MISC, F_SELROW, F_COUNT}};
    hipStream_t side[2] = {h->partner ? h->pool->chk1 : h->stream2, h->partner ? h->pool->chk2 : h->stream3};
    HIPC(hipEventRecord(h->ev_fork, st));
    for (int k = 0; k < 2; k++) {
        HIPC(hipStreamWaitEvent(side[k], h->ev_fork, 0));
        if (k == 1) launch_inputs(h, 1, G, side[k]);
        for (uint32_t fam : side_plan[k])
            for (const pob_ctx::Seg& sg : h->chk_segs) if (sg.lds == fam) { A.first = sg.first; launch_g_check(A, fam, sg.count, G, side[k]); }
    }
    if (!h->plan.sponges.empty()) {
        KArgs K = kargs(h);
        K.first = 0;
        hipStream_t sk = h->partner ? h->stream_k : st;
        if (sk != st) HIPC(hipStreamWaitEvent(sk, h->ev_g_done, 0));
        if (h->ev_kchk[h->rec_slot][0]) { HIPC(hipEventRecord(h->ev_kchk[h->rec_slot][0], sk)); h->kchk_rec[h->rec_slot] = true; }
        launch_k_rounds(K, true, h->nperms, G, sk);
        if (h->ev_kchk[h->rec_slot][1]) HIPC(hipEventRecord(h->ev_kchk[h->rec_slot][1], sk));
        launch_k_chain(K, true, h->nperms, G, h->partner ? side[1] : sk);
        if (sk != st) { HIPC(hipEventRecord(h->ev_k_done, sk)); HIPC(hipStreamWaitEvent(st, h->ev_k_done, 0)); }
    }
    HIPC(hipEventRecord(h->ev_join, side[0])); HIPC(hipEventRecord(h->ev_join3, side[1]));
    HIPC(hipStreamWaitEvent(st, h->ev_join, 0)); HIPC(hipStreamWaitEvent(st, h->ev_join3, 0));
    { int rc = enqueue_collect(h, st, true); if (rc) return rc; }
    HIPC(hipEventRecord(h->ev_check_done, st)); h->check_done_rec = true; h->evaluated = true; h->chk_stream = st; h->chk_ordered = true;
    HIPC(hipEventRecord(h->ev_in_done[h->in_cur], st));
    HIPC(hipGetLastError());
    return POB_OK;
}

int pob_set_partner(pob_handle h, pob_handle partner) {
    if (!h || h == partner || (partner && partner->device != h->device)) return POB_E_ARG;
    if (partner && (h->inorder || partner->inorder)) { h->err = "the two-calculator pipeline links calculators with the track schedule, not in-order ones"; return POB_E_STATE; }
    if (partner && hw_queues_env() < POB_PIPELINE_HW_QUEUES) {
        h->err = "the two-calculator pipeline needs GPU_MAX_HW_QUEUES >= " + std::to_string(POB_PIPELINE_HW_QUEUES) + " in the environment BEFORE the HIP runtime "
                 "initialises (it is " + std::to_string(hw_queues_env()) + "); libpob_hip.so sets it when it is loaded first and the variable is unset";
        return POB_E_STATE;
    }
    for (pob_handle q : {h, partner}) if (q && q->partner) { q->partner->partner = nullptr; q->partner = nullptr; }
    h->partner = partner; h->gen_done_rec = h->check_done_rec = false;
    if (partner) { partner->partner = h; partner->gen_done_rec = partner->check_done_rec = false; }
    return POB_OK;
}

int pob_set_inorder(pob_handle h, int on) {
    if (!h) return POB_E_ARG;
    if (on && h->partner) { h->err = "an in-order calculator has no partner: unlink first (pob_set_partner(h, NULL))"; return POB_E_STATE; }
    h->inorder = on != 0; h->fused = (on & 2) != 0; h->gc = (on & 4) != 0;
    return POB_OK;
}

int pob_sync(pob_handle h) {
    if (!h) return POB_E_ARG;
    HIPC(hipSetDevice(h->device));
    if (h->gen_done_rec) HIPC(hipEventSynchronize(h->ev_gen_done));
    if (h->check_done_rec && h->evaluated) HIPC(hipEventSynchronize(h->ev_check_done));
    HIPC(hipStreamSynchronize(own_stream(h)));
    return POB_OK;
}

int pob_results_fetch(pob_handle h) {
    if (!h || !h->generated) return POB_E_STATE;
    h->fetch_slot = h->rec_slot; h->fetch_pending = true;
    return POB_OK;
}

int pob_results_wait(pob_handle h, const uint8_t** records, uint32_t* n) {
    if (!h || !records) return POB_E_ARG;
    if (!h->fetch_pending) { h->err = "pob_results_wait without pob_results_fetch"; return POB_E_STATE; }
    HIPC(hipSetDevice(h->device));
    HIPC(hipEventSynchronize(h->ev_rec[h->fetch_slot]));
    *records = h->h_records[h->fetch_slot];
    if (n) *n = h->rec_n[h->fetch_slot];
    return POB_OK;
}

int pob_results(pob_handle h, uint32_t* status, uint8_t* outputs, uint32_t* check_status, uint32_t* bad_wire) {
    if (!h || !h->generated) return POB_E_STATE;
    int rc = pob_results_fetch(h); if (rc) return rc;
    const uint8_t* rec = nullptr; uint32_t n = 0;
    rc = pob_results_wait(h, &rec, &n); if (rc) return rc;
    for (uint32_t i = 0; i < n; i++) {
        const uint32_t* r = (const uint32_t*)(rec + (uint64_t)i * POB_RECORD_BYTES);
        if (status) status[i] = r[0];
        if (check_status) check_status[i] = r[1];
        if (bad_wire) bad_wire[i] = r[2];
        if (outputs) memcpy(outputs + (uint64_t)i * 32, r + 3, 32);
    }
    return POB_OK;
}

int pob_results_device(pob_handle h, void** d_status, void** d_outputs) {
    if (!h) return POB_E_ARG;
    if (d_status) *d_status = h->d_status;
    if (d_outputs) *d_outputs = h->d_outputs;
    return POB_OK;
}

#include <dlfcn.h>
typedef int (*pob_nccl_allgather_t)(const void*, void*, size_t, int, void*, hipStream_t);
typedef const char* (*pob_nccl_errstr_t)(int);
static pob_nccl_allgather_t g_nccl_allgather = nullptr; static pob_nccl_errstr_t g_nccl_errstr = nullptr; static bool g_nccl_tried = false;
int pob_gather_records(pob_handle h, void* comm, void* stream_, void* d_out, uint32_t n_per_rank) {
    if (!h || !comm || !d_out || n_per_rank == 0 || n_per_rank > h->groups * 64) return POB_E_ARG;
    if (!h->generated) return POB_E_STATE;
    {
        std::lock_guard<std::mutex> lk(g_pool_mu);
        if (!g_nccl_tried) {
            g_nccl_tried = true;
            void* lib = dlopen("librccl.so.1", RTLD_NOW | RTLD_GLOBAL);
            if (!lib) lib = dlopen("librccl.so", RTLD_NOW | RTLD_GLOBAL);
            if (lib) { g_nccl_allgather = (pob_nccl_allgather_t)dlsym(lib, "ncclAllGather"); g_nccl_errstr = (pob_nccl_errstr_t)dlsym(lib, "ncclGetErrorString"); }
        }
    }
    if (!g_nccl_allgather) { h->err = "librccl.so could not be loaded (pob_gather_records)"; return POB_E_STATE; }
    HIPC(hipSetDevice(h->device));
    hipStream_t st = stream_ ? (hipStream_t)stream_ : own_stream(h);
    if (h->evaluated && h->check_done_rec) { if (h->chk_stream != st) HIPC(hipStreamWaitEvent(st, h->ev_check_done, 0)); }
    else if (h->gen_done_rec && h->gen_stream != st) HIPC(hipStreamWaitEvent(st, h->ev_gen_done, 0));
    const int rc = g_nccl_allgather(h->d_records, d_out, (size_t)n_per_rank * POB_RECORD_BYTES,  1, comm, st);
    if (rc != 0) { h->err = std::string("ncclAllGather: ") + (g_nccl_errstr ? g_nccl_errstr(rc) : "error"); return POB_E_HIP; }
    return POB_OK;
}

int pob_results_records_device(pob_handle h, void** d_records) {
    if (!h || !d_records) return POB_E_ARG;
    *d_records = h->d_records;
    return POB_OK;
}

static int emit_make_window(pob_ctx* h, uint32_t idx, uint64_t k, int slot) {
    pob_ctx::Emit& E = h->em;
    const uint64_t w0 = k * E.win_wires, wn = std::min(E.win_wires, E.total - w0);
    hipStream_t st = own_stream(h);
    HIPC(hipStreamWaitEvent(st, E.ev_free[slot], 0));
    hipLaunchKernelGGL(k_fill_ee, dim3(2048), dim3(256), 0, st, (uint4*)E.d_win[slot], wn * 2);
    if (w0 == 0) { const uint32_t one[8] = {1, 0, 0, 0, 0, 0, 0, 0}; HIPC(hipMemcpyAsync(E.d_win[slot], one, 32, hipMemcpyHostToDevice, st)); }
    GArgs A = gargs(h);
    A.emit_out = E.d_win[slot]; A.emit_sel = idx % 64; A.emit_group = idx / 64; A.emit_w0 = (uint32_t)w0; A.emit_wn = (uint32_t)wn;
    if (E.red) { A.emit_rbits = E.d_rbits; A.emit_rpre = E.d_rpre; }
    if (E.probe_win == E.win_wires && E.probe_map == E.map_id && k < E.wsegs.size()) {
        A.order = E.d_order;
        for (const pob_ctx::Emit::WSeg& sg : E.wsegs[k]) { A.first = sg.first; launch_g_emit(A, sg.cls, sg.count, st); }
    } else {
        for (const pob_ctx::Seg& sg : h->emit_segs) { A.first = sg.first; launch_g_emit(A, sg.lds, sg.count, st); }
    }
    const u64* Gp = (const u64*)h->d_bits + (uint64_t)(idx / 64) * h->plan.total.b;
    const uint64_t wire_lo = E.red ? E.keep[w0] : w0, wire_hi = E.red ? (uint64_t)E.keep[w0 + wn - 1] + 1 : w0 + wn;
    for (const pob_ctx::Emit::Run& r : E.runs) {
        const uint64_t lo = std::max<uint64_t>(r.w, wire_lo), hi = std::min<uint64_t>((uint64_t)r.w + r.n, wire_hi);
        if (lo >= hi) continue;
        if (!E.red) {
            if (r.absorb) launch_k_emit_absorb(Gp, E.d_win[slot] + (lo - w0) * 32, r.b, (uint32_t)(lo - r.w), (uint32_t)(hi - lo), idx % 64, h->d_ktab, st);
            else launch_k_emit_bits(Gp, E.d_win[slot] + (lo - w0) * 32, 0, (uint32_t)(r.b + (lo - r.w)), (uint32_t)(hi - lo), idx % 64, st);
        } else {
            const auto a = std::lower_bound(E.keep.begin() + w0, E.keep.begin() + w0 + wn, (uint32_t)lo), b = std::lower_bound(a, E.keep.begin() + w0 + wn, (uint32_t)hi);
            if (a == b) continue;
            const uint64_t lo2 = *a, hi2 = (uint64_t)*(b - 1) + 1;
            if (r.absorb) launch_k_emit_absorb_red(Gp, E.d_win[slot], (uint32_t)lo2, r.b, (uint32_t)(lo2 - r.w), (uint32_t)(hi2 - lo2), idx % 64, h->d_ktab, E.d_rbits, E.d_rpre, (uint32_t)w0, (uint32_t)wn, st);
            else launch_k_emit_bits_red(Gp, E.d_win[slot], (uint32_t)lo2, (uint32_t)(r.b + (lo2 - r.w)), (uint32_t)(hi2 - lo2), idx % 64, E.d_rbits, E.d_rpre, (uint32_t)w0, (uint32_t)wn, st);
        }
    }
    if (E.sc_on && E.red) {
        const ScWin W{E.d_win[slot], (uint32_t)w0, (uint32_t)wn, E.d_rbits, E.d_rpre};
        uint32_t* res = E.d_sc_res; const uint32_t* zr = E.d_sc_zr; const uint32_t* mr = E.d_sc_mr; const uint32_t* pw = h->d_pow256; const uint32_t nz = E.sc_red_nz, nm = E.sc_red_nm;
        if (nz) hipLaunchKernelGGL(k_selfcheck_zr, dim3((nz + 63) / 64), dim3(64), 0, st, W, zr, nz, res);
        if (nm) hipLaunchKernelGGL(k_selfcheck_mr, dim3((nm + 63) / 64), dim3(64), 0, st, W, mr, nm, pw, res);
    }
    if (E.sc_on && !E.red) {
        const ScWin W{E.d_win[slot], (uint32_t)w0, (uint32_t)wn, nullptr, nullptr};
        uint32_t* res = E.d_sc_res;
        const auto za = std::lower_bound(E.sc_z.begin(), E.sc_z.end(), (uint32_t)wire_lo, [](uint32_t s, uint32_t v) { return (s & 0x7FFFFFFFu) < v; });
        const auto zb = std::lower_bound(za, E.sc_z.end(), (uint32_t)wire_hi, [](uint32_t s, uint32_t v) { return (s & 0x7FFFFFFFu) < v; });
        const uint32_t nz = (uint32_t)(zb - za);
        const uint32_t* zs = E.d_sc_z + (za - E.sc_z.begin());
        if (nz) hipLaunchKernelGGL(k_selfcheck_z, dim3((nz + 63) / 64), dim3(64), 0, st, W, zs, nz, res);
        E.sc_checked += nz;
        const auto ma = std::lower_bound(E.sc_m_next.begin(), E.sc_m_next.end(), (uint32_t)wire_lo), mb = std::lower_bound(ma, E.sc_m_next.end(), (uint32_t)wire_hi);
        const uint32_t nm = (uint32_t)(mb - ma);
        const uint32_t* msites = E.d_sc_m + 3 * (ma - E.sc_m_next.begin()); const uint32_t* pw = h->d_pow256;
        if (nm) hipLaunchKernelGGL(k_selfcheck_m, dim3((nm + 63) / 64), dim3(64), 0, st, W, msites, nm, pw, res);
        E.sc_checked += nm;
        const auto ca = std::lower_bound(E.sc_c_hi.begin(), E.sc_c_hi.end(), (uint32_t)wire_lo), cb = std::lower_bound(ca, E.sc_c_hi.end(), (uint32_t)wire_hi);
        const uint32_t ncs = (uint32_t)(cb - ca);
        const uint32_t* csites = E.d_sc_c + 2 * (ca - E.sc_c_hi.begin());
        if (ncs) hipLaunchKernelGGL(k_selfcheck_c, dim3((ncs + 63) / 64), dim3(64), 0, st, W, csites, ncs, res);
        E.sc_checked += ncs;
    }
    HIPC(hipGetLastError());
    if (E.packed) {
        launch_pack_window(E.d_win[slot], w0, (uint32_t)wn, E.d_pk[slot], E.d_pk_blk, E.d_pk_tot, st);
        HIPC(hipGetLastError());
    }
    HIPC(hipEventRecord(E.ev_made[slot], st));
    HIPC(hipStreamWaitEvent(E.s_copy, E.ev_made[slot], 0));
    if (E.packed) { HIPC(hipMemcpyAsync(E.h_pin[slot], E.d_pk[slot], pack_fixed_bytes(wn), hipMemcpyDeviceToHost, E.s_copy)); E.pk_d2h += pack_fixed_bytes(wn); }
    else HIPC(hipMemcpyAsync(E.h_pin[slot], E.d_win[slot], wn * 32, hipMemcpyDeviceToHost, E.s_copy));
    HIPC(hipEventRecord(E.ev_copied[slot], E.s_copy));
    HIPC(hipEventRecord(E.ev_free[slot], E.s_copy));
    return POB_OK;
}

static uint64_t fnv64(const void* p, size_t n) {
    const uint8_t* q = (const uint8_t*)p; uint64_t hsh = 1469598103934665603ull;
    size_t i = 0;
    for (; i + 8 <= n; i += 8) { uint64_t v; memcpy(&v, q + i, 8); hsh = (hsh ^ v) * 1099511628211ull; }
    for (; i < n; i++) hsh = (hsh ^ q[i]) * 1099511628211ull;
    return hsh ? hsh : 1;
}

static int emit_statuses(pob_ctx* h) {
    pob_ctx::Emit& E = h->em;
    if (E.status_gen == h->gen_count && E.status_host.size() == h->n) return POB_OK;
    HIPC(hipEventSynchronize(h->ev_gen_done));
    E.status_host.resize(h->n);
    HIPC(hipMemcpyAsync(E.status_host.data(), h->d_status, (size_t)h->n * 4, hipMemcpyDeviceToHost, own_stream(h)));
    HIPC(hipStreamSynchronize(own_stream(h)));
    E.status_gen = h->gen_count;
    return POB_OK;
}

static int emit_start(pob_ctx* h, uint32_t idx, uint64_t window_wires) {
    pob_ctx::Emit& E = h->em;
    const int NS = pob_ctx::Emit::NSLOT;
    HIPC(hipEventSynchronize(h->ev_gen_done));
    if (h->evaluated) HIPC(hipEventSynchronize(h->ev_check_done));
    {
        int rc = emit_statuses(h); if (rc) return rc;
        const uint32_t st_w = E.status_host[idx];
        if (st_w != 0) { h->err = "witness " + std::to_string(idx) + " failed an assert (status " + std::to_string(st_w) + "): nothing to emit"; E.queued_idx = -1; E.pre_made = false; return POB_E_STATE; }
    }
    if (window_wires == 0) window_wires = 8ull << 20;
    window_wires = std::min<uint64_t>(window_wires, E.total);
    const uint64_t nwin_ = (E.total + window_wires - 1) / window_wires;
    if (E.pre_made && E.pre_made_gen == h->gen_count && E.queued_idx == (int64_t)idx && E.win_wires == window_wires && E.nwin == nwin_ && E.probe_map == E.map_id && E.pre_made_packed == E.packed) {
        E.first_slot = (E.first_slot + (uint32_t)E.nwin) % NS;
        E.idx = idx; E.next_make = 1; E.next_take = 0; E.active = true; E.queued_idx = -1; E.pre_made = false;
        return POB_OK;
    }
    if (E.pre_made || E.queued_idx == (int64_t)idx) E.queued_idx = -1;
    E.pre_made = false;
    if (E.s_copy) HIPC(hipStreamSynchronize(E.s_copy));
    if (!E.s_copy) {
        HIPC(hipStreamCreateWithPriority(&E.s_copy, hipStreamNonBlocking, 0));
        for (int k = 0; k < NS; k++) {
            HIPC(hipEventCreateWithFlags(&E.ev_made[k], hipEventDisableTiming)); HIPC(hipEventCreateWithFlags(&E.ev_copied[k], hipEventDisableTiming));
            HIPC(hipEventCreateWithFlags(&E.ev_free[k], hipEventDisableTiming));
        }
        for (const SpongeDesc& sp : h->plan.sponges) {
            E.runs.push_back({sp.kin_w, sp.kin_b, sp.n * 1088, 0}); E.runs.push_back({sp.fin_w, sp.fin_b, sp.n * 1088, 0});
            E.runs.push_back({sp.fs_w, sp.fs_b, (sp.n + 1) * 1600, 0});
            for (uint32_t b = 0; b < sp.n; b++) E.runs.push_back({sp.abs_w + b * ABSORB_WIRES, sp.abs_b + b * ABSORB_BITS, ABSORB_WIRES, 1});
        }
        std::sort(E.runs.begin(), E.runs.end(), [](const pob_ctx::Emit::Run& a, const pob_ctx::Emit::Run& b) { return a.w < b.w; });
    }
    if (E.alloc_wires < window_wires) {
        for (int k = 0; k < NS; k++) {
            if (E.d_win[k]) { HIPC(hipFree(E.d_win[k])); E.d_win[k] = nullptr; }
            if (E.h_pin[k]) { HIPC(hipHostFree(E.h_pin[k])); E.h_pin[k] = nullptr; }
            HIPC(hipMalloc(&E.d_win[k], window_wires * 32));
            HIPC(hipHostMalloc((void**)&E.h_pin[k], window_wires * 32 + pack_fixed_bytes(window_wires) + 32, hipHostMallocDefault));
        }
        E.alloc_wires = window_wires;
    }
    if (E.packed && E.pk_alloc_wires < E.alloc_wires) {
        for (int k = 0; k < NS; k++) {
            if (E.d_pk[k]) { HIPC(hipFree(E.d_pk[k])); E.d_pk[k] = nullptr; }
            HIPC(hipMalloc(&E.d_pk[k], E.alloc_wires * 32 + pack_fixed_bytes(E.alloc_wires) + 32));
        }
        if (E.d_pk_blk) { HIPC(hipFree(E.d_pk_blk)); E.d_pk_blk = nullptr; }
        if (E.d_pk_tot) { HIPC(hipFree(E.d_pk_tot)); E.d_pk_tot = nullptr; }
        HIPC(hipMalloc(&E.d_pk_blk, ((E.alloc_wires + 63) / 64) * 4)); HIPC(hipMalloc(&E.d_pk_tot, ((E.alloc_wires + 4095) / 4096) * 4));
        if (!E.s_val) HIPC(hipStreamCreateWithPriority(&E.s_val, hipStreamNonBlocking, 0));
        E.pk_alloc_wires = E.alloc_wires;
    }
    if ((E.probe_win != window_wires || E.probe_map != E.map_id) && nwin_ <= 64) {
        const size_t nu = h->plan.units.size();
        if (!E.d_probe) HIPC(hipMalloc(&E.d_probe, nu * 8));
        HIPC(hipMemsetAsync(E.d_probe, 0, nu * 8, own_stream(h)));
        GArgs A = gargs(h);
        A.emit_sel = 0; A.emit_group = idx / 64; A.emit_w0 = 0; A.emit_wn = (uint32_t)window_wires; A.emit_probe = E.d_probe; A.emit_out = nullptr;
        if (E.red) { A.emit_rbits = E.d_rbits; A.emit_rpre = E.d_rpre; }
        for (const pob_ctx::Seg& sg : h->emit_segs) { A.first = sg.first; launch_g_emit(A, sg.lds, sg.count, own_stream(h)); }
        HIPC(hipGetLastError());
        std::vector<unsigned long long> mask(nu);
        HIPC(hipMemcpyAsync(mask.data(), E.d_probe, nu * 8, hipMemcpyDeviceToHost, own_stream(h)));
        HIPC(hipStreamSynchronize(own_stream(h)));
        std::vector<uint32_t> order;
        E.wsegs.assign(nwin_, {});
        for (uint64_t wi = 0; wi < nwin_; wi++)
            for (const pob_ctx::Seg& sg : h->emit_segs) {
                pob_ctx::Emit::WSeg ws{sg.lds, (uint32_t)order.size(), 0};
                for (uint32_t j = 0; j < sg.count; j++) { const uint32_t u = h->order[sg.first + j]; if ((mask[u] >> wi) & 1) order.push_back(u); }
                ws.count = (uint32_t)order.size() - ws.first;
                if (ws.count) E.wsegs[wi].push_back(ws);
            }
        if (E.d_order) { HIPC(hipFree(E.d_order)); E.d_order = nullptr; }
        HIPC(hipMalloc(&E.d_order, std::max<size_t>(order.size(), 1) * 4));
        if (!order.empty()) HIPC(hipMemcpy(E.d_order, order.data(), order.size() * 4, hipMemcpyHostToDevice));
        E.probe_win = window_wires; E.probe_map = E.map_id;
    } else if (nwin_ > 64) { E.probe_win = 0; E.probe_map = E.map_id; }
    if (E.sc_on && !E.sc_built) {
        const uint32_t cap = std::max(h->plan.total.q, 1u);
        uint32_t* d_rec = nullptr;
        const size_t words = 4 + (size_t)cap + 3 * (size_t)cap + 2 * (size_t)cap;
        HIPC(hipMalloc(&d_rec, words * 4));
        HIPC(hipMemsetAsync(d_rec, 0, 16, own_stream(h)));
        GArgs A = gargs(h);
        A.emit_sel = idx % 64; A.emit_group = idx / 64; A.emit_w0 = 0; A.emit_wn = (uint32_t)E.total; A.emit_out = nullptr; A.emit_sites = d_rec; A.emit_sites_cap = cap;
        for (const pob_ctx::Seg& sg : h->emit_segs) { A.first = sg.first; launch_g_emit(A, sg.lds, sg.count, own_stream(h)); }
        HIPC(hipGetLastError());
        std::vector<uint32_t> rec(words);
        HIPC(hipMemcpyAsync(rec.data(), d_rec, words * 4, hipMemcpyDeviceToHost, own_stream(h)));
        HIPC(hipStreamSynchronize(own_stream(h)));
        HIPC(hipFree(d_rec));
        if (rec[0] > cap || rec[1] > cap || rec[2] > cap) { h->err = "internal: more self-check sites than derived wires"; return POB_E_STATE; }
        E.sc_z.assign(rec.begin() + 4, rec.begin() + 4 + rec[0]);
        std::sort(E.sc_z.begin(), E.sc_z.end(), [](uint32_t a, uint32_t b) { return (a & 0x7FFFFFFFu) < (b & 0x7FFFFFFFu); });
        std::vector<std::array<uint32_t, 3>> ms(rec[1]);
        for (uint32_t i = 0; i < rec[1]; i++) for (int j = 0; j < 3; j++) ms[i][j] = rec[4 + (size_t)cap + 3 * (size_t)i + j];
        std::sort(ms.begin(), ms.end());
        E.sc_ms = ms;
        E.sc_m_next.resize(ms.size());
        for (size_t i = 0; i < ms.size(); i++) E.sc_m_next[i] = ms[i][0];
        std::vector<std::array<uint32_t, 2>> cs(rec[2]);
        for (uint32_t i = 0; i < rec[2]; i++) for (int j = 0; j < 2; j++) cs[i][j] = rec[4 + 4 * (size_t)cap + 2 * (size_t)i + j];
        std::sort(cs.begin(), cs.end());
        E.sc_cs = cs;
        E.sc_c_hi.resize(cs.size());
        for (size_t i = 0; i < cs.size(); i++) E.sc_c_hi[i] = cs[i][0];
        HIPC(hipMalloc(&E.d_sc_c, std::max<size_t>(cs.size(), 1) * 8));
        if (!cs.empty()) HIPC(hipMemcpy(E.d_sc_c, cs.data(), cs.size() * 8, hipMemcpyHostToDevice));
        HIPC(hipMalloc(&E.d_sc_z, std::max<size_t>(E.sc_z.size(), 1) * 4)); HIPC(hipMalloc(&E.d_sc_m, std::max<size_t>(ms.size(), 1) * 12)); HIPC(hipMalloc(&E.d_sc_res, 16));
        if (!E.sc_z.empty()) HIPC(hipMemcpy(E.d_sc_z, E.sc_z.data(), E.sc_z.size() * 4, hipMemcpyHostToDevice));
        if (!ms.empty()) HIPC(hipMemcpy(E.d_sc_m, ms.data(), ms.size() * 12, hipMemcpyHostToDevice));
        E.sc_built = true;
    }
    if (E.sc_on) {
        const uint32_t init[3] = {0xFFFFFFFFu, 0, 0};
        HIPC(hipMemcpyAsync(E.d_sc_res, init, 12, hipMemcpyHostToDevice, own_stream(h)));
        HIPC(hipStreamSynchronize(own_stream(h)));
        E.sc_checked = 0; E.sc_skipped = 0;
    }
    if (E.sc_on && E.red && E.sc_red_map != E.map_id) {
        const bool have_alias = E.sc_alias && E.sc_alias_n == h->plan.total.w;
        auto rep = [&](uint32_t w, uint32_t* out, bool may_be_const = true) -> bool {
            int64_t r = w;
            if (have_alias) {
                r = E.sc_alias[w];
                if (r < 0) {
                    if (!may_be_const || r == INT32_MIN) return false;
                    *out = 0x80000000u | (uint32_t)(-1 - r); return true;
                }
            }
            if (!std::binary_search(E.keep.begin(), E.keep.end(), (uint32_t)r)) return false;
            *out = (uint32_t)r; return true;
        };
        std::vector<uint32_t> zr, mr; uint64_t left_out = E.sc_cs.size();
        for (uint32_t s0 : E.sc_z) {
            const uint32_t w = s0 & 0x7FFFFFFFu; uint32_t q[6] = {0, 0, 0, 0xFFFFFFFFu, 0xFFFFFFFFu, 0xFFFFFFFFu};
            bool ok = rep(w, &q[0], false) && rep(w + 1, &q[1]) && rep(w + 2, &q[2]);
            if (ok && (s0 >> 31)) ok = rep(w - 3, &q[3]) && rep(w - 2, &q[4]) && rep(w - 1, &q[5]);
            if (!ok) { left_out++; continue; }
            zr.insert(zr.end(), q, q + 6);
        }
        for (const std::array<uint32_t, 3>& m3 : E.sc_ms) {
            uint32_t q[4] = {0, 0, 0, m3[2]};
            if (!(rep(m3[0], &q[0], false) && rep(m3[0] - 1, &q[1], false) && rep(m3[1], &q[2], false))) { left_out++; continue; }
            mr.insert(mr.end(), q, q + 4);
        }
        if (E.d_sc_zr) { HIPC(hipFree(E.d_sc_zr)); E.d_sc_zr = nullptr; }
        if (E.d_sc_mr) { HIPC(hipFree(E.d_sc_mr)); E.d_sc_mr = nullptr; }
        HIPC(hipMalloc(&E.d_sc_zr, std::max<size_t>(zr.size(), 1) * 4)); HIPC(hipMalloc(&E.d_sc_mr, std::max<size_t>(mr.size(), 1) * 4));
        if (!zr.empty()) HIPC(hipMemcpy(E.d_sc_zr, zr.data(), zr.size() * 4, hipMemcpyHostToDevice));
        if (!mr.empty()) HIPC(hipMemcpy(E.d_sc_mr, mr.data(), mr.size() * 4, hipMemcpyHostToDevice));
        E.sc_red_nz = (uint32_t)(zr.size() / 6); E.sc_red_nm = (uint32_t)(mr.size() / 4); E.sc_red_host_skipped = left_out; E.sc_red_map = E.map_id;
    }
    for (int k = 0; k < NS; k++) HIPC(hipEventRecord(E.ev_free[k], E.s_copy));
    E.win_wires = window_wires; E.nwin = nwin_; E.idx = idx; E.next_make = 0; E.next_take = 0; E.first_slot = 0; E.active = true;
    for (; E.next_make < std::min<uint64_t>(1, E.nwin); E.next_make++) { int rc = emit_make_window(h, idx, E.next_make, (int)((E.first_slot + E.next_make) % NS)); if (rc) return rc; }
    return POB_OK;
}

int pob_emit_begin(pob_handle h, uint32_t idx, uint64_t window_wires) {
    if (!h) return POB_E_ARG;
    if (!h->generated || idx >= h->n) { h->err = "nothing generated / witness index out of range"; return POB_E_STATE; }
    HIPC(hipSetDevice(h->device));
    h->em.red = false; h->em.map_id = 0; h->em.total = h->plan.total.w; h->em.packed = false;
    return emit_start(h, idx, window_wires);
}

static int emit_begin_reduced(pob_handle h, uint32_t idx, const uint32_t* keep, uint64_t n_keep, uint64_t window_wires, bool packed);
int pob_emit_begin_reduced(pob_handle h, uint32_t idx, const uint32_t* keep, uint64_t n_keep, uint64_t window_wires) { return emit_begin_reduced(h, idx, keep, n_keep, window_wires, false); }
int pob_emit_begin_packed(pob_handle h, uint32_t idx, const uint32_t* keep, uint64_t n_keep, uint64_t window_wires) {
    if (keep) return emit_begin_reduced(h, idx, keep, n_keep, window_wires, true);
    if (!h || n_keep) return POB_E_ARG;
    if (!h->generated || idx >= h->n) { h->err = "nothing generated / witness index out of range"; return POB_E_STATE; }
    HIPC(hipSetDevice(h->device));
    h->em.red = false; h->em.map_id = 0; h->em.total = h->plan.total.w; h->em.packed = true;
    return emit_start(h, idx, window_wires);
}

static int emit_begin_reduced(pob_handle h, uint32_t idx, const uint32_t* keep, uint64_t n_keep, uint64_t window_wires, bool packed) {
    if (!h || !keep || n_keep == 0) return POB_E_ARG;
    if (!h->generated || idx >= h->n) { h->err = "nothing generated / witness index out of range"; return POB_E_STATE; }
// ... 158 lines not shown
    free(canon);
    fclose(f);
    if (!ok) { remove(path); h->err = "write failed"; return POB_E_IO; }
    return POB_OK;
}
int pob_write_wtns(pob_handle h, uint32_t idx, const char* path) {
    if (!h || !path) return POB_E_ARG;
    int rc = pob_emit_begin(h, idx, 0);
    return rc ? rc : write_wtns_stream(h, path);
}
int pob_write_wtns_reduced(pob_handle h, uint32_t idx, const uint32_t* keep, uint64_t n_keep, const char* path) {
    if (!h || !path) return POB_E_ARG;
    int rc = pob_emit_begin_reduced(h, idx, keep, n_keep, 0);
    return rc ? rc : write_wtns_stream(h, path);
}
int pob_write_wtns_packed(pob_handle h, uint32_t idx, const uint32_t* keep, uint64_t n_keep, const char* path) {
    if (!h || !path) return POB_E_ARG;
    int rc = pob_emit_begin_packed(h, idx, keep, n_keep, 0);
    return rc ? rc : write_wtns_stream(h, path);
}

int pob_emit_measure_ex(pob_handle h, uint32_t first_idx, uint32_t count, uint64_t window_wires, const uint32_t* keep, uint64_t n_keep, double* seconds, uint64_t* bytes) {
    if (!h || !seconds || !bytes || count == 0) return POB_E_ARG;
    HIPC(hipSetDevice(h->device));
    uint64_t total = 0; volatile uint8_t sink = 0;
    timespec t0, t1; clock_gettime(CLOCK_MONOTONIC, &t0);
    for (uint32_t i = 0; i < count; i++) {
        int rc = keep ? pob_emit_begin_reduced(h, first_idx + i, keep, n_keep, window_wires) : pob_emit_begin(h, first_idx + i, window_wires);
        if (rc) return rc;
        if (i + 1 < count) { rc = pob_emit_queue(h, first_idx + i + 1); if (rc) return rc; }
        for (;;) {
            const uint8_t* p; uint64_t w0, wn;
            rc = pob_emit_next(h, &p, &w0, &wn);
            if (rc) return rc;
            if (!wn) break;
            sink = sink ^ p[0] ^ p[wn * 32 - 1]; total += wn * 32;
        }
    }
    clock_gettime(CLOCK_MONOTONIC, &t1);
    *seconds = (double)(t1.tv_sec - t0.tv_sec) + 1e-9 * (double)(t1.tv_nsec - t0.tv_nsec); *bytes = total;
    return POB_OK;
}
int pob_emit_measure_packed(pob_handle h, uint32_t first_idx, uint32_t count, uint64_t window_wires, const uint32_t* keep, uint64_t n_keep, uint8_t* dst, uint64_t dst_cap, int threads,
                            double* seconds_pinned, double* seconds_expanded, uint64_t* d2h_bytes) {
    if (!h || !seconds_pinned || !d2h_bytes || count == 0 || threads < 0 || (dst && !seconds_expanded)) return POB_E_ARG;
    HIPC(hipSetDevice(h->device));
    for (int pass = 0; pass < (dst ? 2 : 1); pass++) {
        const uint64_t d0 = h->em.pk_d2h; volatile uint8_t sink = 0;
        timespec t0, t1; clock_gettime(CLOCK_MONOTONIC, &t0);
        for (uint32_t i = 0; i < count; i++) {
            int rc = pob_emit_begin_packed(h, first_idx + i, keep, n_keep, window_wires);
            if (rc) return rc;
            const bool whole = dst_cap >= h->em.total * 32;
            if (pass && !whole && dst_cap < h->em.win_wires * 32) { h->em.active = false; h->err = "destination smaller than a window"; return POB_E_ARG; }
            if (i + 1 < count) { rc = pob_emit_queue(h, first_idx + i + 1); if (rc) return rc; }
            for (;;) {
                const uint8_t* p; uint64_t pb, w0, wn;
                rc = pob_emit_next_packed(h, &p, &pb, &w0, &wn);
                if (rc) return rc;
                if (!wn) break;
                sink = sink ^ p[0] ^ p[pb - 1];
                if (pass) { rc = pob_unpack_window(p, pb, whole ? dst + w0 * 32 : dst, wn * 32, threads); if (rc) { h->em.active = false; h->err = "internal: a packed window does not validate"; return rc; } }
            }
        }
        clock_gettime(CLOCK_MONOTONIC, &t1);
        const double sec = (double)(t1.tv_sec - t0.tv_sec) + 1e-9 * (double)(t1.tv_nsec - t0.tv_nsec);
        if (pass) *seconds_expanded = sec; else { *seconds_pinned = sec; *d2h_bytes = h->em.pk_d2h - d0; }
    }
    return POB_OK;
}
int pob_emit_measure(pob_handle h, uint32_t first_idx, uint32_t count, uint64_t window_wires, double* seconds, uint64_t* bytes) {
    return pob_emit_measure_ex(h, first_idx, count, window_wires, nullptr, 0, seconds, bytes);
}

int pob_probe_check_kernel(pob_handle h, int enable, float* ms) {
    if (!h) return POB_E_ARG;
    HIPC(hipSetDevice(h->device));
    if (ms) {
        uint32_t sl = h->rec_slot;
        if (!h->kchk_rec[sl] || hipEventQuery(h->ev_kchk[sl][1]) != hipSuccess) sl ^= 1;
        if (!h->ev_kchk[sl][0] || !h->kchk_rec[sl]) { h->err = "no timed evaluation yet"; return POB_E_STATE; }
        HIPC(hipEventSynchronize(h->ev_kchk[sl][1]));
        HIPC(hipEventElapsedTime(ms, h->ev_kchk[sl][0], h->ev_kchk[sl][1]));
    }
    if (enable && !h->ev_kchk[0][0]) for (auto& pr : h->ev_kchk) for (hipEvent_t& e : pr) HIPC(hipEventCreate(&e));
    if (!enable) { for (auto& pr : h->ev_kchk) for (hipEvent_t& e : pr) if (e) { hipEventDestroy(e); e = nullptr; } h->kchk_rec[0] = h->kchk_rec[1] = false; }
    return POB_OK;
}

int pob_time_kernel(pob_handle h, int which, int iters, void* stream_, float* avg_ms) {
    if (!h || !h->generated || iters < 1 || !avg_ms) return POB_E_STATE;
    HIPC(hipSetDevice(h->device));
    hipStream_t st = stream_ ? (hipStream_t)stream_ : own_stream(h);
    const uint32_t G = (h->n + 63) / 64;
    hipEvent_t e0, e1;
    HIPC(hipEventCreate(&e0)); HIPC(hipEventCreate(&e1));
    KArgs K = kargs(h); K.first = 0;
    GArgs A = gargs(h);
    uint32_t* d_sel = nullptr; uint32_t nsel = 0, sel_cls = 0, sel_fam = 0;
    if (which >= 100 && which < 300) {
        const uint32_t kind = (uint32_t)which % 100, need = which >= 200 ? UNIT_GEN : UNIT_CHECK;
        std::vector<uint32_t> sel;
        for (uint32_t u = 0; u < h->plan.units.size(); u++) if (h->plan.units[u].kind == kind && (h->plan.units[u].flags & need)) sel.push_back(u);
        if (sel.empty()) { *avg_ms = 0; hipEventDestroy(e0); hipEventDestroy(e1); return POB_OK; }
        nsel = (uint32_t)sel.size(); sel_cls = unit_class(kind, which >= 200); sel_fam = fam_of(kind);
        HIPC(hipMalloc(&d_sel, nsel * 4)); HIPC(hipMemcpy(d_sel, sel.data(), nsel * 4, hipMemcpyHostToDevice));
        A.order = d_sel; A.first = 0;
    }
    HIPC(hipEventRecord(e0, st));
    for (int it = 0; it < iters; it++) {
        if (which >= 300) {
            for (const pob_ctx::Seg& sg : h->chk_segs) if (sg.lds == (uint32_t)which - 300) { A.first = sg.first; launch_g_check(A, sg.lds, sg.count, G, st); }
        } else if (which >= 200) launch_g_gen(A, sel_cls, nsel, G, st);
        else if (which >= 100) launch_g_check(A, sel_fam, nsel, G, st);
        else if (which == 0) launch_k_rounds(K, false, h->nperms, G, st);
        else if (which == 1) launch_k_rounds(K, true, h->nperms, G, st);
        else if (which == 6) launch_k_rounds_gc(K, h->nperms, G, false, st);
        else if (which == 2) {
            for (const pob_ctx::Seg& sg : h->chk_segs) {
                A.first = sg.first;
                launch_g_check(A, sg.lds, sg.count, G, st);
            }
        } else launch_k_chain(K, false, (uint32_t)h->plan.sponges.size(), G, st);
    }
    HIPC(hipEventRecord(e1, st));
    HIPC(hipEventSynchronize(e1));
    float ms = 0; HIPC(hipEventElapsedTime(&ms, e0, e1));
    *avg_ms = ms / iters;
    hipEventDestroy(e0); hipEventDestroy(e1);
    if (d_sel) hipFree(d_sel);
    return POB_OK;
}

int pob_debug_stream_create(int device, const uint32_t* cu_mask, uint32_t words, void** stream) {
    if (!cu_mask || !words || !stream) return POB_E_ARG;
    if (hipSetDevice(device) != hipSuccess) return POB_E_HIP;
    hipStream_t st = nullptr;
    if (hipExtStreamCreateWithCUMask(&st, words, cu_mask) != hipSuccess) return POB_E_HIP;
    *stream = (void*)st;
    return POB_OK;
}
void pob_debug_stream_destroy(int device, void* stream) { if (stream && hipSetDevice(device) == hipSuccess) hipStreamDestroy((hipStream_t)stream); }

int pob_debug_store_fault(pob_handle h, int cls, uint32_t group, uint64_t index, uint64_t mask, uint32_t* wire) {
    if (!h || group >= h->groups) return POB_E_ARG;
    if (!h->inorder || !h->gc) { h->err = "pob_debug_store_fault: the calculator's generation carries no evaluation (pob_set_inorder bit 2)"; return POB_E_STATE; }
    bool found = false;
    if (cls == POB_CLASS_BIT) {
        if (index >= h->plan.total.b) return POB_E_ARG;
        for (const SpongeDesc& sp : h->plan.sponges) {
            if (index < sp.abs_b || index >= sp.abs_b + (uint64_t)sp.n * ABSORB_BITS) continue;
            const uint32_t b = (uint32_t)((index - sp.abs_b) / ABSORB_BITS), o = (uint32_t)((index - sp.abs_b) % ABSORB_BITS);
            if (o < AB_DIRECT) break;
            if (wire) *wire = sp.abs_w + b * ABSORB_WIRES + AB_DIRECT + (o - AB_DIRECT) / KR_BITS * KECCAKF_ROUND_WIRES;
            found = true; break;
        }
    } else if (cls == POB_CLASS_SM && h->circuit == POB_CIRCUIT_PROOF_OF_BURN) {
        const SmRef r0 = h->plan.L.pm.numLeafAddressNibbles;
        if (index >= r0.i && index < r0.i + h->plan.nsm_in) { found = true; if (wire) *wire = r0.w + (uint32_t)(index - r0.i); }
    }
    h->fault_g = !found;
    if (!found) {
        const Cur t = h->plan.total;
        if (!(h->circuit == POB_CIRCUIT_PROOF_OF_BURN || h->circuit == POB_CIRCUIT_SPEND) || (cls == POB_CLASS_BIT ? index >= t.b : cls == POB_CLASS_SM ? index >= t.s : cls == POB_CLASS_FR ? index >= t.f : true)) {
            h->err = "pob_debug_store_fault: not a stored word whose evaluation rides with its generation"; return POB_E_ARG;
        }
        if (wire) *wire = 0xFFFFFFFFu;
    }
    h->fault_armed = true; h->fault_cls = cls; h->fault_group = group; h->fault_word = index; h->fault_mask = mask;
    return POB_OK;
}

int pob_debug_xor_bits(pob_handle h, uint32_t group, uint64_t bit_index, uint64_t mask) {
    if (!h || group >= h->groups || bit_index >= h->plan.total.b) return POB_E_ARG;
    HIPC(hipSetDevice(h->device));
    h->rode = false;
    hipLaunchKernelGGL(k_xor_word, dim3(1), dim3(1), 0, own_stream(h), h->d_bits + (uint64_t)group * h->plan.total.b + bit_index, mask);
    HIPC(hipStreamSynchronize(own_stream(h)));
    return POB_OK;
}

int pob_debug_poke(pob_handle h, int cls, uint32_t group, uint64_t index, uint32_t sub, uint32_t lane, uint32_t xor_mask) {
    if (!h || group >= h->groups || lane >= 64) return POB_E_ARG;
    HIPC(hipSetDevice(h->device));
    h->rode = false;
    const Cur t = h->plan.total;
    if (cls == POB_CLASS_BIT) {
        if (index >= t.b) return POB_E_ARG;
        hipLaunchKernelGGL(k_xor_word, dim3(1), dim3(1), 0, own_stream(h), h->d_bits + (uint64_t)group * t.b + index, (uint64_t)(xor_mask & 1u) << lane);
    } else if (cls == POB_CLASS_SM) {
        if (index >= t.s) return POB_E_ARG;
        hipLaunchKernelGGL(k_xor_u32, dim3(1), dim3(1), 0, own_stream(h), (uint32_t*)h->d_sm + ((uint64_t)group * t.s + index) * 64 + lane, xor_mask);
    } else if (cls == POB_CLASS_FR) {
        if (index >= t.f || sub >= 8) return POB_E_ARG;
        hipLaunchKernelGGL(k_xor_u32, dim3(1), dim3(1), 0, own_stream(h), h->d_fr + ((uint64_t)group * t.f + index) * 512 + sub * 64 + lane, xor_mask);
    } else return POB_E_ARG;
    HIPC(hipStreamSynchronize(own_stream(h)));
    return POB_OK;
}

int pob_debug_fr_inv(int device, const uint8_t* in, uint32_t n, uint8_t* out_kaliski, uint8_t* out_fermat) {
    if (!in || !out_kaliski || !out_fermat || n == 0) return POB_E_ARG;
    if (hipSetDevice(device) != hipSuccess) return POB_E_HIP;
    uint32_t *d_in = nullptr, *d_a = nullptr, *d_b = nullptr;
    const size_t bytes = (size_t)n * 32;
    int rc = POB_E_HIP;
    if (hipMalloc(&d_in, bytes) == hipSuccess && hipMalloc(&d_a, bytes) == hipSuccess && hipMalloc(&d_b, bytes) == hipSuccess &&
        hipMemcpy(d_in, in, bytes, hipMemcpyHostToDevice) == hipSuccess) {
        hipLaunchKernelGGL(k_fr_inv_test, dim3((n + 63) / 64), dim3(64), 0, 0, d_in, d_a, d_b, n);
        if (hipMemcpy(out_kaliski, d_a, bytes, hipMemcpyDeviceToHost) == hipSuccess && hipMemcpy(out_fermat, d_b, bytes, hipMemcpyDeviceToHost) == hipSuccess) rc = POB_OK;
    }
    if (d_in) hipFree(d_in); if (d_a) hipFree(d_a); if (d_b) hipFree(d_b);
    return rc;
}

int pob_debug_fr_sqr(int device, const uint8_t* in, uint32_t n, uint8_t* out_sqr, uint8_t* out_mul) {
    if (!in || !out_sqr || !out_mul || n == 0) return POB_E_ARG;
    if (hipSetDevice(device) != hipSuccess) return POB_E_HIP;
    uint32_t *d_in = nullptr, *d_a = nullptr, *d_b = nullptr;
    const size_t bytes = (size_t)n * 32;
    int rc = POB_E_HIP;
    if (hipMalloc(&d_in, bytes) == hipSuccess && hipMalloc(&d_a, bytes) == hipSuccess && hipMalloc(&d_b, bytes) == hipSuccess &&
        hipMemcpy(d_in, in, bytes, hipMemcpyHostToDevice) == hipSuccess) {
        hipLaunchKernelGGL(k_fr_sqr_test, dim3((n + 63) / 64), dim3(64), 0, 0, d_in, d_a, d_b, n);
        if (hipMemcpy(out_sqr, d_a, bytes, hipMemcpyDeviceToHost) == hipSuccess && hipMemcpy(out_mul, d_b, bytes, hipMemcpyDeviceToHost) == hipSuccess) rc = POB_OK;
    }
    if (d_in) hipFree(d_in); if (d_a) hipFree(d_a); if (d_b) hipFree(d_b);
    return rc;
}

int pob_debug_emit_counters(pob_handle h, uint64_t out[4], int reset) {
    if (!h || !out) return POB_E_ARG;
    HIPC(hipSetDevice(h->device));
    uint32_t c[4];
    HIPC(hipStreamSynchronize(own_stream(h)));
    HIPC(hipMemcpy(c, h->d_emit_ctr, sizeof c, hipMemcpyDeviceToHost));
    for (int k = 0; k < 4; k++) out[k] = c[k];
    if (reset) HIPC(hipMemset(h->d_emit_ctr, 0, sizeof c));
    return POB_OK;
}

int pob_debug_ref(pob_handle h, const char* name, uint32_t k, int* cls, uint64_t* index, uint64_t* wire) {
    if (!h || !name || !cls || !index || !wire) return POB_E_ARG;
    const Plan& pl = h->plan; const CircuitLayout& L = pl.L;
    const std::string n = name;
    auto set = [&](int c, uint64_t i, uint64_t w) { *cls = c; *index = i; *wire = w; return POB_OK; };
    if (n == "poseidon" || n == "poseidon.t3" || n == "poseidon.t4" || n == "poseidon.t5") {
        const uint32_t want_t = n.size() > 8 ? (uint32_t)(n[10] - '0') : 0;
        for (const UnitDesc& u : pl.units) if (u.kind == CK_POS_SEG && (want_t == 0 || u.a[0] == want_t)) {
            if (k >= pos_wires((int)u.a[0], pos_off((int)u.a[0]).rp)) return POB_E_ARG;
            return set(POB_CLASS_FR, u.cur.f + k, u.cur.w + k);
        }
        return POB_E_ARG;
    }
    if (n == "commitment") { const FrRef r = h->circuit == POB_CIRCUIT_PROOF_OF_BURN ? L.pm.commitment : L.sm.commitment; return set(POB_CLASS_FR, r.i, r.w); }
    if (n == "kb.inLen") { if (k >= L.nkb) return POB_E_ARG; return set(POB_CLASS_SM, L.kbs[k].inLen.i, L.kbs[k].inLen.w); }
    if (n == "pad.div.out" || n == "pad.div.rem") {
        if (k >= L.nkb) return POB_E_ARG;
        const KBRefs& r = L.kbs[k];
        const uint32_t o = n == "pad.div.rem" ? 1 : 0;
        return set(POB_CLASS_SM, r.c_div.s + o, r.c_div.w + o);
    }
    if (h->circuit == POB_CIRCUIT_PROOF_OF_BURN && L.nsc > 1) {
        const ScRefs& sc = L.scs[1];
        const uint32_t mm = 136u * (uint32_t)L.pob.NB, kk = mm - 31 + 1;
        if (n == "sc.exists" && k < kk) return set(POB_CLASS_BIT, sc.ex.i + k, sc.ex.w + k);
    }
    return POB_E_ARG;
}

static const int KROT_H[25] = {1, 10, 7, 11, 17, 18, 3, 5, 16, 8, 21, 24, 4, 15, 23, 19, 13, 12, 2, 20, 14, 22, 9, 6, 1};
static uint64_t rotl64h(uint64_t v, int n) { return n ? (v << n) | (v >> (64 - n)) : v; }
static void keccak_f_host(uint64_t a[25]) {
    static const uint64_t RC[24] = {
        0x0000000000000001ULL, 0x0000000000008082ULL, 0x800000000000808AULL, 0x8000000080008000ULL, 0x000000000000808BULL,
        0x0000000080000001ULL, 0x8000000080008081ULL, 0x8000000000008009ULL, 0x000000000000008AULL, 0x0000000000000088ULL,
        0x0000000080008009ULL, 0x000000008000000AULL, 0x000000008000808BULL, 0x800000000000008BULL, 0x8000000000008089ULL,
        0x8000000000008003ULL, 0x8000000000008002ULL, 0x8000000000000080ULL, 0x000000000000800AULL, 0x800000008000000AULL,
        0x8000000080008081ULL, 0x8000000000008080ULL, 0x0000000080000001ULL, 0x8000000080008008ULL};
    for (int r = 0; r < 24; r++) {
        uint64_t c[5], b[25];
        for (int x = 0; x < 5; x++) c[x] = a[x] ^ a[x + 5] ^ a[x + 10] ^ a[x + 15] ^ a[x + 20];
        for (int x = 0; x < 5; x++) { uint64_t d = c[(x + 4) % 5] ^ rotl64h(c[(x + 1) % 5], 1); for (int y = 0; y < 25; y += 5) a[x + y] ^= d; }
        b[0] = a[0];
        for (int i = 0; i < 24; i++) b[KROT_H[i + 1]] = rotl64h(a[KROT_H[i]], ((i + 1) * (i + 2) / 2) % 64);
        for (int i = 0; i < 25; i++) { int y = i / 5 * 5; a[i] = b[i] ^ (~b[y + (i + 1) % 5] & b[y + (i + 2) % 5]); }
        a[0] ^= RC[r];
    }
}
void pob_keccak256(const uint8_t* msg, uint64_t len, uint8_t out[32]) {
    uint64_t st[25]; memset(st, 0, sizeof st);
    uint8_t blk[136];
    for (uint64_t off = 0;; off += 136) {
        uint64_t n = len - off < 136 ? len - off : 136;
        memset(blk, 0, 136); if (n) memcpy(blk, msg + off, n);
        const bool last = n < 136;
        if (last) { blk[n] ^= 0x01; blk[135] ^= 0x80; }
        for (int i = 0; i < 17; i++) { uint64_t v; memcpy(&v, blk + 8 * i, 8); st[i] ^= v; }
        keccak_f_host(st);
        if (last) break;
    }
    memcpy(out, st, 32);
}

int64_t pob_pow_search(const uint8_t start_key[32], const uint8_t* postfix, uint32_t postfix_len, uint32_t zero_bytes, uint64_t max_tries, uint8_t out_key[32]) {
    if (postfix_len > 100 || zero_bytes > 8) return -1;
    uint8_t msg[136];
    memcpy(msg, start_key, 32); memcpy(msg + 32, postfix, postfix_len);
    const uint32_t len = 32 + postfix_len;
    for (uint64_t t = 0; t < max_tries; t++) {
        uint8_t blk[136]; memset(blk, 0, 136); memcpy(blk, msg, len); blk[len] ^= 0x01; blk[135] ^= 0x80;
        uint64_t st[25]; memset(st, 0, sizeof st);
        for (int i = 0; i < 17; i++) { uint64_t v; memcpy(&v, blk + 8 * i, 8); st[i] = v; }
        keccak_f_host(st);
        const uint64_t mask = zero_bytes == 8 ? ~0ULL : ((1ULL << (8 * zero_bytes)) - 1);
        if ((st[0] & mask) == 0) { memcpy(out_key, msg, 32); return (int64_t)t; }
        for (int i = 31; i >= 0; i--) if (++msg[i]) break;
    }
    return -1;
}

int64_t pob_pow_search_gpu(int device, const uint8_t start_key[32], const uint8_t* postfix, uint32_t postfix_len, uint32_t zero_bytes,
                           uint64_t max_tries, uint8_t out_key[32]) {
    if (postfix_len > 100 || zero_bytes > 8 || zero_bytes == 0) return -1;
    if (hipSetDevice(device) != hipSuccess) return -2;
    uint8_t blk[136]; memset(blk, 0, 136);
    memcpy(blk + 32, postfix, postfix_len);
    const uint32_t len = 32 + postfix_len;
    blk[len] ^= 0x01; blk[135] ^= 0x80;
    uint64_t tail[13];
    for (int i = 0; i < 13; i++) memcpy(&tail[i], blk + 32 + 8 * i, 8);
    uint64_t kw[4];
    for (int i = 0; i < 4; i++) { uint64_t v = 0; for (int j = 0; j < 8; j++) v = (v << 8) | start_key[8 * i + j]; kw[i] = v; }
    uint64_t* d_tail = nullptr; unsigned long long* d_found = nullptr;
    if (hipMalloc(&d_tail, sizeof tail) != hipSuccess || hipMalloc(&d_found, 8) != hipSuccess) return -2;
    hipMemcpy(d_tail, tail, sizeof tail, hipMemcpyHostToDevice);
    const uint64_t mask = zero_bytes == 8 ? ~0ULL : ((1ULL << (8 * zero_bytes)) - 1);
    const uint64_t WIN = 1ULL << 24;
    int64_t result = -1;
    for (uint64_t base = 0; base < max_tries; base += WIN) {
        const uint64_t cnt = max_tries - base < WIN ? max_tries - base : WIN;
        unsigned long long init = ~0ULL;
        hipMemcpy(d_found, &init, 8, hipMemcpyHostToDevice);
        hipLaunchKernelGGL(k_pow_search, dim3((uint32_t)((cnt + 255) / 256)), dim3(256), 0, 0, kw[0], kw[1], kw[2], kw[3], d_tail, base, cnt, mask, d_found);
        unsigned long long got = ~0ULL;
        if (hipMemcpy(&got, d_found, 8, hipMemcpyDeviceToHost) != hipSuccess) { result = -2; break; }
        if (got != ~0ULL) { result = (int64_t)got; break; }
    }
    hipFree(d_tail); hipFree(d_found);
    if (result >= 0) {
        uint64_t w[4] = {kw[0], kw[1], kw[2], kw[3]};
        uint64_t add = (uint64_t)result;
        for (int i = 3; i >= 0 && add; i--) { const uint64_t o = w[i]; w[i] += add; add = w[i] < o; }
        for (int i = 0; i < 4; i++) for (int j = 0; j < 8; j++) out_key[8 * i + j] = (uint8_t)(w[i] >> (56 - 8 * j));
    }
    return result;
}

}
```

Before: 1.143 million.

## Store keccak sponge states once and derive duplicated wires at emit time

The sponge chain kernel stops writing many redundant copies of each absorb block's state, input block and XOR output (k_in, f_in, f_s, absorb-own slots, keccak-f input copies). It now stores only the 25 round-state snapshots per block. The emit kernels get an AbsorbRef (previous block's final state and source block) and remap the old wire offsets onto those snapshots, while the check kernel verifies against the compact layout. This cuts global-memory write traffic and footprint per witness, at the cost of more index arithmetic and branching when wire words are emitted.

```diff
diff --git a/proof_of_burn_amd/csrc/circuits.hpp b/proof_of_burn_amd/csrc/circuits.hpp
--- a/proof_of_burn_amd/csrc/circuits.hpp
+++ b/proof_of_burn_amd/csrc/circuits.hpp
@@ -9,7 +9,9 @@
 #define ABSORB_WIRES (ABSORB_OWN + 17u * 384u + KECCAKF_WIRES)
 #define KR_STORED 76u
 #define KR_BITS (KR_STORED * 64u)
-#define AB_DIRECT (ABSORB_OWN + 17u * 384u + 43200u)
+#define AB_ROUNDS_W (ABSORB_OWN + 17u * 384u + 43200u)
+#define AB_MID 0u
+#define AB_DIRECT (25u * 1600u)
 #define ABSORB_BITS (AB_DIRECT + 24u * KR_BITS)
 #define ABSORB_ALIAS (ABSORB_WIRES - ABSORB_BITS)
 
@@ -113,7 +115,7 @@
     SmRef ri_o, ri_ol; FrRef ri_i; SmRef by, len, be; BitRef isb, isz; SmRef frb;
     Cur c_cb, c_sl, c_lt, c_concat, c_end;
 };
-struct SpongeDesc { uint32_t n, stage, src_b, kin_b, fin_b, fs_b, abs_b, kin_w, fin_w, fs_w, abs_w, src_w; };
+struct SpongeDesc { uint32_t n, stage, src_b, abs_b, kin_w, fin_w, fs_w, abs_w, src_w; };
 struct UnitDesc { uint32_t kind, stage; Cur cur; uint32_t a[8]; uint32_t cost, flags; };
 
 #define SC_RANGE_POS 32
@@ -249,8 +251,8 @@
 }
 template <class P> GD void kb_declare_keccak(P& p, KBRefs& r) {
     const uint32_t n = r.mb;
-    r.k_out = dbits(p, 256); r.k_in = p.bits(n * 1088); r.k_blocks = p.sms(1); r.k_finalState = dbits(p, 1600);
-    r.f_out = dbits(p, 1600); r.f_in = p.bits(n * 1088); r.f_blocks = p.sms(1); r.f_s = p.bits((n + 1) * 1600);
+    r.k_out = dbits(p, 256); r.k_in = dbits(p, n * 1088); r.k_blocks = p.sms(1); r.k_finalState = dbits(p, 1600);
+    r.f_out = dbits(p, 1600); r.f_in = dbits(p, n * 1088); r.f_blocks = p.sms(1); r.f_s = dbits(p, (n + 1) * 1600);
     r.abs_w = p.cur.w; r.abs_b = p.cur.b;
     p.skip_alias(n * ABSORB_WIRES, n * ABSORB_BITS);
     r.sel_out = dbits(p, 1600); r.sel_arrays = dbits(p, (n + 1) * 1600); r.sel_select = p.sms(1); r.sel_T = dbits(p, 1600 * (n + 1));
@@ -267,7 +269,7 @@
     p.run_derived(n, bw + 2 * n1 + 2, 0);
 #pragma unroll
     for (uint32_t k = 0; k < n1; k++) {
-        const B v = p.run_get(n, r.f_s.i + k * 1600 + idx);
+        const B v = k == 0 ? (B)0 : p.run_get(n, r.abs_b + (k - 1) * ABSORB_BITS + AB_MID + 24u * 1600u + idx);
         const B e = p.ballot((uint32_t)blocks == k);
         acc |= e & v;
         if constexpr (P::is_emit) {
@@ -1022,7 +1024,7 @@
         r.index = kb;
         kb_declare_keccak(p, r);
         SpongeDesc s; s.n = r.mb; s.stage = range_stage + 1; s.src_b = r.inBlocks.i; s.src_w = r.inBlocks.w;
-        s.kin_b = r.k_in.i; s.kin_w = r.k_in.w; s.fin_b = r.f_in.i; s.fin_w = r.f_in.w; s.fs_b = r.f_s.i; s.fs_w = r.f_s.w; s.abs_b = r.abs_b; s.abs_w = r.abs_w;
+        s.kin_w = r.k_in.w; s.fin_w = r.f_in.w; s.fs_w = r.f_s.w; s.abs_b = r.abs_b; s.abs_w = r.abs_w;
         sponges.push_back(s);
         r.dst = dst; r.has_dst = has_dst ? 1 : 0;
         {
diff --git a/proof_of_burn_amd/csrc/k_keccak.hip b/proof_of_burn_amd/csrc/k_keccak.hip
--- a/proof_of_burn_amd/csrc/k_keccak.hip
+++ b/proof_of_burn_amd/csrc/k_keccak.hip
@@ -36,11 +36,11 @@
     uint32_t blocks = (count + 255) / 256; if (blocks > 16384) blocks = 16384;
     hipLaunchKernelGGL(k_emit_bits_red, dim3(blocks), dim3(256), 0, st, G, out, wire0, bit_base, count, sel, rbits, rpre, k0, kn);
 }
-void launch_k_emit_absorb(const u64* G, uint8_t* out, uint32_t ab, uint32_t o0, uint32_t count, uint32_t sel, const uint16_t* tab, hipStream_t st) {
+void launch_k_emit_absorb(const u64* G, uint8_t* out, AbsorbRef ab, uint32_t o0, uint32_t count, uint32_t sel, const uint16_t* tab, hipStream_t st) {
     uint32_t blocks = (count + 255) / 256; if (blocks > 8192) blocks = 8192;
     hipLaunchKernelGGL(k_emit_absorb, dim3(blocks), dim3(256), 0, st, G, out, ab, o0, count, sel, tab);
 }
-void launch_k_emit_absorb_red(const u64* G, uint8_t* out, uint32_t wire0, uint32_t ab, uint32_t o0, uint32_t count, uint32_t sel, const uint16_t* tab, const unsigned long long* rbits,
+void launch_k_emit_absorb_red(const u64* G, uint8_t* out, uint32_t wire0, AbsorbRef ab, uint32_t o0, uint32_t count, uint32_t sel, const uint16_t* tab, const unsigned long long* rbits,
                               const uint32_t* rpre, uint32_t k0, uint32_t kn, hipStream_t st) {
     uint32_t blocks = (count + 255) / 256; if (blocks > 16384) blocks = 16384;
     hipLaunchKernelGGL(k_emit_absorb_red, dim3(blocks), dim3(256), 0, st, G, out, wire0, ab, o0, count, sel, tab, rbits, rpre, k0, kn);
diff --git a/proof_of_burn_amd/csrc/keccak_kernels.hpp b/proof_of_burn_amd/csrc/keccak_kernels.hpp
--- a/proof_of_burn_amd/csrc/keccak_kernels.hpp
+++ b/proof_of_burn_amd/csrc/keccak_kernels.hpp
@@ -283,38 +283,20 @@
     u64 st[25];
 #pragma unroll
     for (int i = 0; i < 25; i++) st[i] = 0;
-    auto put = [&](uint32_t idx, u64 v) { G[idx + lane] = v; };
     for (uint32_t b = 0; b < sp.n; b++) {
-        const uint32_t Ab = sp.abs_b + b * ABSORB_BITS;
-        u64 blk[17], aux[25];
-#pragma unroll
-        for (int i = 0; i < 17; i++) blk[i] = G[sp.src_b + b * 1088 + 64 * i + lane];
-#pragma unroll
-        for (int i = 0; i < 25; i++) { put(sp.fs_b + b * 1600 + 64 * i, st[i]); put(Ab + 1600 + 64 * i, st[i]); }
-#pragma unroll
-        for (int i = 0; i < 17; i++) {
-            put(sp.kin_b + b * 1088 + 64 * i, blk[i]); put(sp.fin_b + b * 1088 + 64 * i, blk[i]); put(Ab + 3200 + 64 * i, blk[i]);
-            const u64 o = st[i] ^ blk[i];
-            const uint32_t X = Ab + ABSORB_OWN + 384 * i;
-            put(X, o); put(X + 64, st[i]); put(X + 128, blk[i]);
-            { u64* q = G + X + 192 + 3 * lane; q[0] = o; q[1] = st[i]; q[2] = blk[i]; }
-            aux[i] = o;
-        }
-#pragma unroll
-        for (int i = 17; i < 25; i++) aux[i] = st[i];
-        const uint32_t Kf = Ab + AB_KECCAKF;
-#pragma unroll
-        for (int i = 0; i < 25; i++) { put(Ab + 4288 + 64 * i, aux[i]); put(Kf + 1600 + 64 * i, aux[i]); put(Kf + KF_MID + 64 * i, aux[i]); st[i] = aux[i]; }
+        u64* mid = G + sp.abs_b + b * ABSORB_BITS + AB_MID + lane;
+        const u64* blk = G + sp.src_b + b * 1088 + lane;
+#pragma unroll
+        for (int i = 0; i < 17; i++) st[i] ^= blk[64 * i];
+#pragma unroll
+        for (int i = 0; i < 25; i++) mid[64 * i] = st[i];
         for (int r = 0; r < 24; r++) {
             round_native(st, r, lane);
-#pragma unroll
-            for (int i = 0; i < 25; i++) put(Kf + KF_MID + 1600 * (r + 1) + 64 * i, st[i]);
-        }
-#pragma unroll
-        for (int i = 0; i < 25; i++) { put(Kf + 64 * i, st[i]); put(Ab + 64 * i, st[i]); }
-    }
-#pragma unroll
-    for (int i = 0; i < 25; i++) put(sp.fs_b + sp.n * 1600 + 64 * i, st[i]);
+            mid += 1600;
+#pragma unroll
+            for (int i = 0; i < 25; i++) mid[64 * i] = st[i];
+        }
+    }
 }
 #ifdef POB_KECCAK_TU
 __global__ void __launch_bounds__(64, 3) k_chain(KArgs A) { chain_body(A, blockIdx.x, blockIdx.y); }
@@ -326,26 +308,22 @@
     const SpongeDesc sp = A.sponges[A.perm_sponge[pi]];
     const uint32_t b = A.perm_block[pi];
     const u64* G = A.bits + (uint64_t)by * A.group_stride;
-    const uint32_t Ab = sp.abs_b + b * ABSORB_BITS, Kf = Ab + AB_KECCAKF;
+    const u64* mid = G + sp.abs_b + b * ABSORB_BITS + AB_MID + lane;
+    const u64* prev = G + sp.abs_b + (b ? b - 1 : 0) * ABSORB_BITS + AB_MID + 1600 * 24 + lane;
+    const u64* blk = G + sp.src_b + b * 1088 + lane;
     u64 bad = 0;
 #pragma unroll 1
-    for (int i = 0; i < 25; i++) {
-        const u64 st = G[sp.fs_b + b * 1600 + 64 * i + lane];
-        if (b == 0) bad |= st;
-        bad |= G[Ab + 1600 + 64 * i + lane] ^ st;
-        u64 aux = st;
-        if (i < 17) {
-            const u64 blk = G[sp.src_b + b * 1088 + 64 * i + lane];
-            bad |= (G[sp.kin_b + b * 1088 + 64 * i + lane] ^ blk) | (G[sp.fin_b + b * 1088 + 64 * i + lane] ^ blk) | (G[Ab + 3200 + 64 * i + lane] ^ blk);
-            const u64 o = st ^ blk;
-            const uint32_t X = Ab + ABSORB_OWN + 384 * i;
-            const u64* q = G + X + 192 + 3 * lane;
-            bad |= (G[X + lane] ^ o) | (G[X + 64 + lane] ^ st) | (G[X + 128 + lane] ^ blk) | (q[0] ^ o) | (q[1] ^ st) | (q[2] ^ blk);
-            aux = o;
-        }
-        bad |= (G[Ab + 4288 + 64 * i + lane] ^ aux) | (G[Kf + 1600 + 64 * i + lane] ^ aux) | (G[Kf + KF_MID + 64 * i + lane] ^ aux);
-        const u64 last = G[Kf + KF_MID + 1600 * 24 + 64 * i + lane];
-        bad |= (G[Kf + 64 * i + lane] ^ last) | (G[Ab + 64 * i + lane] ^ last) | (G[sp.fs_b + (b + 1) * 1600 + 64 * i + lane] ^ last);
+    for (int y = 0; y < 5; y++) {
+        u64 m0[5], s[5], k[5];
+#pragma unroll
+        for (int x = 0; x < 5; x++) {
+            const int i = 5 * y + x;
+            m0[x] = mid[64 * i];
+            s[x] = b ? prev[64 * i] : 0;
+            k[x] = i < 17 ? blk[64 * i] : 0;
+        }
+#pragma unroll
+        for (int x = 0; x < 5; x++) bad |= m0[x] ^ s[x] ^ k[x];
     }
 #pragma unroll
     for (int o = 32; o > 0; o >>= 1) { bad |= ((u64)__shfl_xor((uint32_t)(bad >> 32), o, 64) << 32) | __shfl_xor((uint32_t)bad, o, 64); }
@@ -363,7 +341,7 @@
     const uint32_t Ab = sp.abs_b + A.perm_block[pi] * ABSORB_BITS;
     u64* G = A.bits + (uint64_t)y * A.group_stride;
     GenIO io; io.lane = lane;
-    const u64* mid = G + Ab + AB_KECCAKF + KF_MID + 1600 * r0;
+    const u64* mid = G + Ab + AB_MID + 1600 * r0;
 #pragma unroll
     for (int i = 0; i < 25; i++) io.s[i] = mid[64 * i + lane];
     io.st = G + Ab + AB_DIRECT + r0 * KR_BITS;
@@ -388,7 +366,7 @@
     const uint32_t Ab = sp.abs_b + (A).perm_block[pi] * ABSORB_BITS; \
     const u64* G = (A).bits + (uint64_t)(Y_) * (A).group_stride; \
     CheckIOT<NT, DP> io; io.lane = lane; io.bad = 0; \
-    const u64* mid = G + Ab + AB_KECCAKF + KF_MID + 1600 * r0; \
+    const u64* mid = G + Ab + AB_MID + 1600 * r0; \
     _Pragma("unroll") \
     for (int i = 0; i < 25; i++) io.s[i] = io.ldw(mid + 64 * i + lane); \
     io.st = G + Ab + AB_DIRECT + r0 * KR_BITS; \
@@ -444,7 +422,7 @@
     const SpongeDesc sp = A.sponges[A.perm_sponge[pi]];
     const uint32_t Ab = sp.abs_b + A.perm_block[pi] * ABSORB_BITS;
     u64* G = A.bits + (uint64_t)blockIdx.y * A.group_stride;
-    const u64* mid = G + Ab + AB_KECCAKF + KF_MID + 1600 * r0;
+    const u64* mid = G + Ab + AB_MID + 1600 * r0;
     GcIOT<DP, FAULT, NTM> io; io.lane = lane; io.bad = 0;
     if constexpr (FAULT) { io.fault = blockIdx.y == A.fault_group ? G + A.fault_word : nullptr; io.fault_mask = A.fault_mask; }
 #pragma unroll
@@ -469,20 +447,42 @@
     }
 }
 
-__device__ __forceinline__ u64 absorb_wire_word(const u64* A, uint32_t ab, uint32_t o, const uint16_t* tab, uint32_t* neg) {
+__device__ __forceinline__ u64 absorb_wire_word(const u64* A, const AbsorbRef B, uint32_t o, const uint16_t* tab, uint32_t* neg) {
     *neg = 0;
-    if (o < AB_DIRECT) return A[ab + o];
-    const uint32_t q = o - AB_DIRECT, r = q / KECCAKF_ROUND_WIRES, e = tab[q - r * KECCAKF_ROUND_WIRES];
+    const uint32_t ab = B.ab;
+    if (o < AB_ROUNDS_W) {
+        enum { M0, M24, S_, K_ };
+        uint32_t what, j;
+        if (o < 1600u) { what = M24; j = o; }
+        else if (o < 3200u) { what = S_; j = o - 1600u; }
+        else if (o < 4288u) { what = K_; j = o - 3200u; }
+        else if (o < ABSORB_OWN) { what = M0; j = o - 4288u; }
+        else if (o < AB_KECCAKF) {
+            const uint32_t q = o - ABSORB_OWN, i = q / 384u, t = q - 384u * i;
+            if (t < 192u) { what = t < 64u ? M0 : t < 128u ? S_ : K_; j = 64u * i + (t & 63u); }
+            else { const uint32_t u = t - 192u, c = u % 3u; what = c == 0 ? M0 : c == 1 ? S_ : K_; j = 64u * i + u / 3u; }
+        } else {
+            const uint32_t q = o - AB_KECCAKF;
+            if (q < 1600u) { what = M24; j = q; }
+            else if (q < KF_MID) { what = M0; j = q - 1600u; }
+            else return A[ab + AB_MID + (q - KF_MID)];
+        }
+        if (what == M0) return A[ab + AB_MID + j];
+        if (what == M24) return A[ab + AB_MID + 1600u * 24u + j];
+        if (what == S_) return B.prev == NO_RANK ? 0 : A[B.prev + j];
+        return A[B.src + j];
+    }
+    const uint32_t q = o - AB_ROUNDS_W, r = q / KECCAKF_ROUND_WIRES, e = tab[q - r * KECCAKF_ROUND_WIRES];
     const uint32_t slot = e >> 7, k = (e >> 1) & 63u;
     *neg = e & 1u;
-    if (slot < KS_ST) return A[ab + AB_KECCAKF + KF_MID + 1600 * r + 64 * slot + k];
+    if (slot < KS_ST) return A[ab + AB_MID + 1600 * r + 64 * slot + k];
     if (slot < KS_OUT) return A[ab + AB_DIRECT + r * KR_BITS + 64 * (slot - KS_ST) + k];
-    if (slot < KS_ZERO) return A[ab + AB_KECCAKF + KF_MID + 1600 * (r + 1) + 64 * (slot - KS_OUT) + k];
+    if (slot < KS_ZERO) return A[ab + AB_MID + 1600 * (r + 1) + 64 * (slot - KS_OUT) + k];
     if (slot == KS_ZERO) return 0;
     return ((KECCAK_RC_DEV[r] >> k) & 1) ? ~0ULL : 0ULL;
 }
 #ifdef POB_KECCAK_TU
-__global__ void __launch_bounds__(256) k_emit_absorb(const u64* G, uint8_t* out, uint32_t ab, uint32_t o0, uint32_t count, uint32_t sel, const uint16_t* tab) {
+__global__ void __launch_bounds__(256) k_emit_absorb(const u64* G, uint8_t* out, AbsorbRef ab, uint32_t o0, uint32_t count, uint32_t sel, const uint16_t* tab) {
     for (uint32_t t = blockIdx.x * blockDim.x + threadIdx.x; t < count; t += gridDim.x * blockDim.x) {
         uint32_t neg;
         const u64 word = absorb_wire_word(G, ab, o0 + t, tab, &neg);
@@ -491,7 +491,7 @@
         q[0] = make_uint4(v, 0, 0, 0); q[1] = make_uint4(0, 0, 0, 0);
     }
 }
-__global__ void __launch_bounds__(256) k_emit_absorb_red(const u64* G, uint8_t* out, uint32_t wire0, uint32_t ab, uint32_t o0, uint32_t count, uint32_t sel, const uint16_t* tab,
+__global__ void __launch_bounds__(256) k_emit_absorb_red(const u64* G, uint8_t* out, uint32_t wire0, AbsorbRef ab, uint32_t o0, uint32_t count, uint32_t sel, const uint16_t* tab,
                                                          const unsigned long long* rbits, const uint32_t* rpre, uint32_t k0, uint32_t kn) {
     for (uint32_t t = blockIdx.x * blockDim.x + threadIdx.x; t < count; t += gridDim.x * blockDim.x) {
         const uint32_t w = wire0 + t;
diff --git a/proof_of_burn_amd/csrc/kernels_common.hpp b/proof_of_burn_amd/csrc/kernels_common.hpp
--- a/proof_of_burn_amd/csrc/kernels_common.hpp
+++ b/proof_of_burn_amd/csrc/kernels_common.hpp
@@ -32,6 +32,8 @@
     uint32_t fault_group; uint64_t fault_word, fault_mask;
 };
 
+struct AbsorbRef { uint32_t ab, prev, src; };
+
 void launch_g_gen_light(const GArgs& A, uint32_t nunits, uint32_t ngroups, hipStream_t st);
 void launch_g_gen_sc(const GArgs& A, uint32_t nunits, uint32_t ngroups, hipStream_t st);
 void launch_pos_wide(const GArgs& A, uint32_t nunits, uint32_t ngroups, hipStream_t st, bool ride = false, bool fault = false);
@@ -62,7 +64,7 @@
 int pob_kgc_rounds();
 void launch_k_emit_bits(const u64* G, uint8_t* out, uint32_t wire_base, uint32_t bit_base, uint32_t count, uint32_t sel, hipStream_t st);
 void launch_k_emit_bits_red(const u64* G, uint8_t* out, uint32_t wire0, uint32_t bit_base, uint32_t count, uint32_t sel, const unsigned long long* rbits, const uint32_t* rpre, uint32_t k0, uint32_t kn, hipStream_t st);
-void launch_k_emit_absorb(const u64* G, uint8_t* out, uint32_t ab, uint32_t o0, uint32_t count, uint32_t sel, const uint16_t* tab, hipStream_t st);
-void launch_k_emit_absorb_red(const u64* G, uint8_t* out, uint32_t wire0, uint32_t ab, uint32_t o0, uint32_t count, uint32_t sel, const uint16_t* tab, const unsigned long long* rbits,
+void launch_k_emit_absorb(const u64* G, uint8_t* out, AbsorbRef B, uint32_t o0, uint32_t count, uint32_t sel, const uint16_t* tab, hipStream_t st);
+void launch_k_emit_absorb_red(const u64* G, uint8_t* out, uint32_t wire0, AbsorbRef B, uint32_t o0, uint32_t count, uint32_t sel, const uint16_t* tab, const unsigned long long* rbits,
                               const uint32_t* rpre, uint32_t k0, uint32_t kn, hipStream_t st);
 bool keccak_alias_table_host(uint16_t* tab);
diff --git a/proof_of_burn_amd/csrc/pob_host.hip b/proof_of_burn_amd/csrc/pob_host.hip
--- a/proof_of_burn_amd/csrc/pob_host.hip
+++ b/proof_of_burn_amd/csrc/pob_host.hip
@@ -300,7 +300,7 @@
         uint64_t pre_made_gen = 0;
         std::vector<uint32_t> status_host; uint64_t status_gen = 0;
         const uint32_t* pin_ptr = nullptr; uint64_t pin_n = 0, pin_id = 0;
-        struct Run { uint32_t w, b, n, absorb; };
+        struct Run { uint32_t w, b, n, absorb, o, prev, src; };
         std::vector<Run> runs;
         uint64_t probe_win = 0, probe_map = 0; uint32_t* d_order = nullptr; unsigned long long* d_probe = nullptr;
         struct WSeg { uint32_t cls, first, count; };
@@ -1173,13 +1173,13 @@
         const uint64_t lo = std::max<uint64_t>(r.w, wire_lo), hi = std::min<uint64_t>((uint64_t)r.w + r.n, wire_hi);
         if (lo >= hi) continue;
         if (!E.red) {
-            if (r.absorb) launch_k_emit_absorb(Gp, E.d_win[slot] + (lo - w0) * 32, r.b, (uint32_t)(lo - r.w), (uint32_t)(hi - lo), idx % 64, h->d_ktab, st);
+            if (r.absorb) launch_k_emit_absorb(Gp, E.d_win[slot] + (lo - w0) * 32, AbsorbRef{r.b, r.prev, r.src}, r.o + (uint32_t)(lo - r.w), (uint32_t)(hi - lo), idx % 64, h->d_ktab, st);
             else launch_k_emit_bits(Gp, E.d_win[slot] + (lo - w0) * 32, 0, (uint32_t)(r.b + (lo - r.w)), (uint32_t)(hi - lo), idx % 64, st);
         } else {
             const auto a = std::lower_bound(E.keep.begin() + w0, E.keep.begin() + w0 + wn, (uint32_t)lo), b = std::lower_bound(a, E.keep.begin() + w0 + wn, (uint32_t)hi);
             if (a == b) continue;
             const uint64_t lo2 = *a, hi2 = (uint64_t)*(b - 1) + 1;
-            if (r.absorb) launch_k_emit_absorb_red(Gp, E.d_win[slot], (uint32_t)lo2, r.b, (uint32_t)(lo2 - r.w), (uint32_t)(hi2 - lo2), idx % 64, h->d_ktab, E.d_rbits, E.d_rpre, (uint32_t)w0, (uint32_t)wn, st);
+            if (r.absorb) launch_k_emit_absorb_red(Gp, E.d_win[slot], (uint32_t)lo2, AbsorbRef{r.b, r.prev, r.src}, r.o + (uint32_t)(lo2 - r.w), (uint32_t)(hi2 - lo2), idx % 64, h->d_ktab, E.d_rbits, E.d_rpre, (uint32_t)w0, (uint32_t)wn, st);
             else launch_k_emit_bits_red(Gp, E.d_win[slot], (uint32_t)lo2, (uint32_t)(r.b + (lo2 - r.w)), (uint32_t)(hi2 - lo2), idx % 64, E.d_rbits, E.d_rpre, (uint32_t)w0, (uint32_t)wn, st);
         }
     }
@@ -1270,9 +1270,13 @@
             HIPC(hipEventCreateWithFlags(&E.ev_free[k], hipEventDisableTiming));
         }
         for (const SpongeDesc& sp : h->plan.sponges) {
-            E.runs.push_back({sp.kin_w, sp.kin_b, sp.n * 1088, 0}); E.runs.push_back({sp.fin_w, sp.fin_b, sp.n * 1088, 0});
-            E.runs.push_back({sp.fs_w, sp.fs_b, (sp.n + 1) * 1600, 0});
-            for (uint32_t b = 0; b < sp.n; b++) E.runs.push_back({sp.abs_w + b * ABSORB_WIRES, sp.abs_b + b * ABSORB_BITS, ABSORB_WIRES, 1});
+            E.runs.push_back({sp.kin_w, sp.src_b, sp.n * 1088, 0, 0, 0, 0}); E.runs.push_back({sp.fin_w, sp.src_b, sp.n * 1088, 0, 0, 0, 0});
+            E.runs.push_back({sp.fs_w, sp.abs_b, 1600, 1, 1600, NO_RANK, sp.src_b});
+            for (uint32_t b = 0; b < sp.n; b++) {
+                const uint32_t ab = sp.abs_b + b * ABSORB_BITS, m24 = ab + AB_MID + 24u * 1600u;
+                E.runs.push_back({sp.fs_w + (b + 1) * 1600, m24, 1600, 0, 0, 0, 0});
+                E.runs.push_back({sp.abs_w + b * ABSORB_WIRES, ab, ABSORB_WIRES, 1, 0, b ? m24 - ABSORB_BITS : NO_RANK, sp.src_b + b * 1088});
+            }
         }
         std::sort(E.runs.begin(), E.runs.end(), [](const pob_ctx::Emit::Run& a, const pob_ctx::Emit::Run& b) { return a.w < b.w; });
     }
@@ -1737,7 +1741,7 @@
             if (index < sp.abs_b || index >= sp.abs_b + (uint64_t)sp.n * ABSORB_BITS) continue;
             const uint32_t b = (uint32_t)((index - sp.abs_b) / ABSORB_BITS), o = (uint32_t)((index - sp.abs_b) % ABSORB_BITS);
             if (o < AB_DIRECT) break;
-            if (wire) *wire = sp.abs_w + b * ABSORB_WIRES + AB_DIRECT + (o - AB_DIRECT) / KR_BITS * KECCAKF_ROUND_WIRES;
+            if (wire) *wire = sp.abs_w + b * ABSORB_WIRES + AB_ROUNDS_W + (o - AB_DIRECT) / KR_BITS * KECCAKF_ROUND_WIRES;
             found = true; break;
         }
     } else if (cls == POB_CLASS_SM && h->circuit == POB_CIRCUIT_PROOF_OF_BURN) {
@@ -1840,6 +1844,11 @@
     }
     if (n == "commitment") { const FrRef r = h->circuit == POB_CIRCUIT_PROOF_OF_BURN ? L.pm.commitment : L.sm.commitment; return set(POB_CLASS_FR, r.i, r.w); }
     if (n == "kb.inLen") { if (k >= L.nkb) return POB_E_ARG; return set(POB_CLASS_SM, L.kbs[k].inLen.i, L.kbs[k].inLen.w); }
+    if (n == "kb.inBlocks" || n == "kb.absorb") {
+        if (k >= L.nkb) return POB_E_ARG;
+        const KBRefs& r = L.kbs[k];
+        return n == "kb.inBlocks" ? set(POB_CLASS_BIT, r.inBlocks.i, r.inBlocks.w) : set(POB_CLASS_BIT, r.abs_b + AB_MID, r.abs_w);
+    }
     if (n == "pad.div.out" || n == "pad.div.rem") {
         if (k >= L.nkb) return POB_E_ARG;
         const KBRefs& r = L.kbs[k];
```

New measurement: 1.224 million (median of 6 runs). 1.07x the previous value.
